# ntnu-yjyjames/nano-vectordb

Hardware: AMD Instinct MI355X
Metric: QPS + effective HBM GB/s, flat-scan top-10 d=768 (higher is better)
Workload: dtype f16

## Files before the change

include/nvdb_hip.h:

```cpp
#ifndef NVDB_HIP_H
#define NVDB_HIP_H

#include <stddef.h>
#include <stdint.h>

#ifdef __cplusplus
extern "C" {
#endif

#define NVDB_HIP_ABI_VERSION 3

enum { NVDB_DTYPE_F32 = 1, NVDB_DTYPE_F16 = 2, NVDB_DTYPE_I8 = 3 };

typedef enum nvdb_status {
  NVDB_OK = 0,
  NVDB_ERR_INVALID = 1,
  NVDB_ERR_HIP = 2,
  NVDB_ERR_UNSUPPORTED = 3,
  NVDB_ERR_NO_CORPUS = 4,
  NVDB_ERR_INTERNAL = 5
} nvdb_status;

#define NVDB_HIP_REFINE_KMAX 64

typedef struct nvdb_hip_ctx nvdb_hip_ctx;

typedef struct nvdb_hip_timing {
  float h2d_ms, kernel_ms, d2h_ms, total_ms;
  uint32_t threads;
  uint32_t nwarps;
  uint32_t K;
  uint32_t R;
  size_t shmem_bytes;
  uint32_t dbg_q;
  double dbg_dist_cycles_avg, dbg_write_cycles_avg, dbg_merge_cycles_avg;
  double dbg_dist_pct, dbg_write_pct, dbg_merge_pct;
} nvdb_hip_timing;

typedef struct nvdb_hip_scan_stats {
  uint32_t path;
  uint32_t chunks;
  uint64_t rows_scanned;
  uint64_t candidates;
  uint32_t overflow_queries;
  uint32_t bound_violations;
  float    filter_kernel_ms;
  float    other_kernel_ms;
  uint32_t i8_stage1_tiles;
  uint32_t i8_stage2_blocks;
  uint32_t sticky_overflow;
  uint32_t sticky_violations;
} nvdb_hip_scan_stats;

int nvdb_hip_abi_version(void);
int nvdb_hip_device_count(void);

nvdb_status nvdb_hip_create(int device_ordinal, nvdb_hip_ctx** out_ctx);
void nvdb_hip_destroy(nvdb_hip_ctx* ctx);
const char* nvdb_hip_last_error(const nvdb_hip_ctx* ctx);


nvdb_status nvdb_hip_upload_corpus(nvdb_hip_ctx* ctx, const void* rows, const float* scales,
                                   uint64_t n, uint32_t dim, uint32_t dtype, uint64_t global_row_base);

nvdb_status nvdb_hip_adopt_corpus(nvdb_hip_ctx* ctx, void* dev_rows, float* dev_scales,
                                  uint64_t n, uint32_t dim, uint32_t dtype, uint64_t global_row_base);

nvdb_status nvdb_hip_generate_corpus(nvdb_hip_ctx* ctx, uint64_t seed, uint64_t n, uint32_t dim,
                                     uint32_t dtype, uint64_t global_row_base);

nvdb_status nvdb_hip_corpus_info(const nvdb_hip_ctx* ctx, uint64_t* n, uint32_t* dim, uint32_t* dtype,
                                 uint64_t* global_row_base, float* max_row_norm);

nvdb_status nvdb_hip_download_rows(nvdb_hip_ctx* ctx, uint64_t row0, uint64_t nrows, void* rows_out,
                                   float* scales_out);


nvdb_status nvdb_hip_search_batch(nvdb_hip_ctx* ctx, const float* queries, uint32_t nq, uint32_t k,
                                  uint64_t* out_ids, float* out_scores, uint32_t* out_k_eff,
                                  nvdb_hip_timing* timing);

nvdb_status nvdb_hip_search_batch_dev(nvdb_hip_ctx* ctx, const float* dev_queries, uint32_t nq, uint32_t k,
                                      uint64_t* dev_out_ids, float* dev_out_scores, void* hip_stream);
nvdb_status nvdb_hip_search_check(nvdb_hip_ctx* ctx, nvdb_hip_scan_stats* stats);
nvdb_status nvdb_hip_get_stats(nvdb_hip_ctx* ctx, nvdb_hip_scan_stats* stats);


nvdb_status nvdb_hip_range_search(nvdb_hip_ctx* ctx, const float* queries, uint32_t nq,
                                  const float* radius , uint64_t* out_lims ,
                                  nvdb_hip_timing* timing );
nvdb_status nvdb_hip_range_results(nvdb_hip_ctx* ctx, uint64_t* out_ids, float* out_scores);

nvdb_status nvdb_hip_shadow_info(const nvdb_hip_ctx* ctx, uint64_t* out4);

nvdb_status nvdb_hip_merge_topk_dev(nvdb_hip_ctx* ctx, const uint64_t* dev_ids, const float* dev_scores,
                                    uint32_t nshards, uint32_t nq, uint32_t k, uint64_t* dev_out_ids,
                                    float* dev_out_scores, void* hip_stream);
nvdb_status nvdb_hip_merge_topk_strided_dev(nvdb_hip_ctx* ctx, const uint64_t* dev_ids, const float* dev_scores,
                                            size_t stride_ids_bytes, size_t stride_scores_bytes, uint32_t nshards,
                                            uint32_t nq, uint32_t k, uint64_t* dev_out_ids, float* dev_out_scores,
                                            void* hip_stream);
nvdb_status nvdb_merge_topk_host(const uint64_t* ids, const float* scores, uint32_t nshards, uint32_t nq,
                                 uint32_t k, uint64_t* out_ids, float* out_scores);

typedef struct nvdb_hip_group nvdb_hip_group;
typedef struct nvdb_hip_group_stats {
  uint32_t shards;
  uint32_t exchange;
  uint32_t host_merge_fallbacks;
  uint64_t bytes_per_rank;
} nvdb_hip_group_stats;

nvdb_status nvdb_hip_group_create(const int* devices, uint32_t n_devices, nvdb_hip_group** out_group);
void nvdb_hip_group_destroy(nvdb_hip_group* group);
const char* nvdb_hip_group_last_error(const nvdb_hip_group* group);
uint32_t nvdb_hip_group_size(const nvdb_hip_group* group);
nvdb_hip_ctx* nvdb_hip_group_ctx(nvdb_hip_group* group, uint32_t shard);
int nvdb_hip_group_exchange(const nvdb_hip_group* group, const char** why);
nvdb_status nvdb_hip_group_upload_corpus(nvdb_hip_group* group, const void* rows, const float* scales, uint64_t n,
                                         uint32_t dim, uint32_t dtype);
nvdb_status nvdb_hip_group_generate_corpus(nvdb_hip_group* group, uint64_t seed, uint64_t n, uint32_t dim, uint32_t dtype);
nvdb_status nvdb_hip_group_set_option(nvdb_hip_group* group, const char* key, int64_t value);
nvdb_status nvdb_hip_group_search_batch(nvdb_hip_group* group, const float* queries, uint32_t nq, uint32_t k,
                                        uint64_t* out_ids, float* out_scores, uint32_t* out_k_eff,
                                        nvdb_hip_group_stats* stats);


nvdb_status nvdb_hip_set_partitions(nvdb_hip_ctx* ctx, const uint64_t* offsets, uint32_t nparts);

nvdb_status nvdb_hip_set_centroids(nvdb_hip_ctx* ctx, const float* centroids);

nvdb_status nvdb_hip_search_partitions(nvdb_hip_ctx* ctx, const float* queries, uint32_t nq, uint32_t k,
                                       const uint32_t* probe, uint32_t nprobe,
                                       uint64_t* out_ids, float* out_scores, uint32_t* out_counts,
                                       nvdb_hip_timing* timing);

nvdb_status nvdb_hip_search_ivf(nvdb_hip_ctx* ctx, const float* queries, uint32_t nq, uint32_t k, uint32_t nprobe,
                                uint64_t* out_ids, float* out_scores, uint32_t* out_counts,
                                uint32_t* out_probe, nvdb_hip_timing* timing);


nvdb_status nvdb_hip_set_row_masks(nvdb_hip_ctx* ctx, const uint32_t* bits , uint32_t nmasks);

nvdb_status nvdb_hip_update_row_mask(nvdb_hip_ctx* ctx, uint32_t mask, const uint64_t* rows, uint64_t nrows, int live);

nvdb_status nvdb_hip_get_row_masks(nvdb_hip_ctx* ctx, uint32_t* nmasks, uint64_t* words_per_mask, uint32_t* bits_out );

nvdb_status nvdb_hip_search_partitions_masked(nvdb_hip_ctx* ctx, const float* queries, uint32_t nq, uint32_t k,
                                              const uint32_t* probe, uint32_t nprobe, const uint32_t* mask_of ,
                                              uint64_t* out_ids, float* out_scores, uint32_t* out_counts,
                                              nvdb_hip_timing* timing);
nvdb_status nvdb_hip_search_ivf_masked(nvdb_hip_ctx* ctx, const float* queries, uint32_t nq, uint32_t k, uint32_t nprobe,
                                       const uint32_t* mask_of ,
                                       uint64_t* out_ids, float* out_scores, uint32_t* out_counts,
                                       uint32_t* out_probe, nvdb_hip_timing* timing);
nvdb_status nvdb_hip_search_batch_masked(nvdb_hip_ctx* ctx, const float* queries, uint32_t nq, uint32_t k,
                                         const uint32_t* mask_of ,
                                         uint64_t* out_ids, float* out_scores, uint32_t* out_counts,
                                         nvdb_hip_timing* timing);


nvdb_status nvdb_hip_compact_rows(nvdb_hip_ctx* ctx, uint32_t mask, uint64_t* out_n ,
                                  uint32_t* out_old_rows );

struct nvdb_hip_ivf;
nvdb_status nvdb_hip_ivf_compact(struct nvdb_hip_ivf* ivf, uint32_t mask, uint64_t* out_n );


nvdb_status nvdb_hip_reserve_rows(nvdb_hip_ctx* ctx, uint64_t rows);

nvdb_status nvdb_hip_insert_rows(nvdb_hip_ctx* ctx, const void* rows, const float* scales , uint64_t m,
                                 const uint32_t* part_of ,
                                 uint64_t* out_new_rows , uint64_t* out_n );

nvdb_status nvdb_hip_ivf_add_rows(struct nvdb_hip_ivf* ivf, const void* rows, const float* scales , uint64_t m,
                                  uint64_t* out_first_id , uint32_t* out_assign );


nvdb_status nvdb_hip_range_search_partitions(nvdb_hip_ctx* ctx, const float* queries, uint32_t nq,
                                             const float* radius , const uint32_t* probe , uint32_t nprobe,
                                             const uint32_t* mask_of , int masked,
                                             uint64_t* out_lims , nvdb_hip_timing* timing );
nvdb_status nvdb_hip_range_search_ivf(nvdb_hip_ctx* ctx, const float* queries, uint32_t nq, const float* radius ,
                                      uint32_t nprobe, const uint32_t* mask_of , int masked,
                                      uint64_t* out_lims , uint32_t* out_probe ,
                                      nvdb_hip_timing* timing );
nvdb_status nvdb_hip_range_search_masked(nvdb_hip_ctx* ctx, const float* queries, uint32_t nq, const float* radius ,
                                         const uint32_t* mask_of , uint64_t* out_lims ,
                                         nvdb_hip_timing* timing );


nvdb_status nvdb_hip_search_partitions_anyk(nvdb_hip_ctx* ctx, const float* queries, uint32_t nq, uint32_t k,
                                            const uint32_t* probe , uint32_t nprobe,
                                            const uint32_t* mask_of , int masked,
                                            uint64_t* out_ids , float* out_scores ,
                                            uint32_t* out_counts , nvdb_hip_timing* timing );
nvdb_status nvdb_hip_search_ivf_anyk(nvdb_hip_ctx* ctx, const float* queries, uint32_t nq, uint32_t k, uint32_t nprobe,
                                     const uint32_t* mask_of , int masked,
                                     uint64_t* out_ids , float* out_scores ,
                                     uint32_t* out_counts , uint32_t* out_probe ,
                                     nvdb_hip_timing* timing );


nvdb_status nvdb_hip_assign_rows(nvdb_hip_ctx* ctx, const float* centroids, uint32_t nparts,
                                 uint64_t row0, uint64_t nrows, uint32_t* out_assign);

nvdb_status nvdb_hip_train_centroids(nvdb_hip_ctx* ctx, uint32_t nparts, uint32_t iters, uint64_t seed,
                                     uint64_t max_train_rows, const float* init, float* out_centroids);

nvdb_status nvdb_ivf_layout_host(const uint32_t* assign, uint64_t n, uint32_t nparts,
                                 uint64_t* out_offsets , uint32_t* out_perm );

typedef struct nvdb_hip_ivf nvdb_hip_ivf;
nvdb_status nvdb_hip_ivf_build(nvdb_hip_ctx* src, const float* centroids, uint32_t nparts, nvdb_hip_ivf** out);
void nvdb_hip_ivf_destroy(nvdb_hip_ivf* ivf);
const char* nvdb_hip_ivf_last_error(const nvdb_hip_ivf* ivf);
nvdb_hip_ctx* nvdb_hip_ivf_ctx(nvdb_hip_ivf* ivf);
nvdb_status nvdb_hip_ivf_info(const nvdb_hip_ivf* ivf, uint64_t* n, uint32_t* nparts,
                              uint64_t* offsets_out, uint32_t* perm_out);
nvdb_status nvdb_hip_ivf_search(nvdb_hip_ivf* ivf, const float* queries, uint32_t nq, uint32_t k, uint32_t nprobe,
                                uint64_t* out_ids, float* out_scores, uint32_t* out_counts,
                                uint32_t* out_probe, nvdb_hip_timing* timing);

nvdb_status nvdb_hip_ivf_set_row_masks(nvdb_hip_ivf* ivf, const uint32_t* bits, uint32_t nmasks);
nvdb_status nvdb_hip_ivf_update_row_mask(nvdb_hip_ivf* ivf, uint32_t mask, const uint64_t* rows, uint64_t nrows, int live);
nvdb_status nvdb_hip_ivf_search_masked(nvdb_hip_ivf* ivf, const float* queries, uint32_t nq, uint32_t k, uint32_t nprobe,
                                       const uint32_t* mask_of ,
                                       uint64_t* out_ids, float* out_scores, uint32_t* out_counts,
                                       uint32_t* out_probe, nvdb_hip_timing* timing);

nvdb_status nvdb_hip_ivf_search_anyk(nvdb_hip_ivf* ivf, const float* queries, uint32_t nq, uint32_t k, uint32_t nprobe,
                                     const uint32_t* mask_of , int masked,
                                     uint64_t* out_ids, float* out_scores, uint32_t* out_counts,
                                     uint32_t* out_probe, nvdb_hip_timing* timing);

nvdb_status nvdb_hip_ivf_range_search(nvdb_hip_ivf* ivf, const float* queries, uint32_t nq, const float* radius ,
                                      uint32_t nprobe, const uint32_t* mask_of , int masked,
                                      uint64_t* out_lims , uint32_t* out_probe ,
                                      nvdb_hip_timing* timing );
nvdb_status nvdb_hip_ivf_range_results(nvdb_hip_ivf* ivf, uint64_t* out_ids, float* out_scores);

nvdb_status nvdb_hip_set_option(nvdb_hip_ctx* ctx, const char* key, int64_t value);

nvdb_status nvdb_hip_collect_kernel_times(nvdb_hip_ctx* ctx, uint32_t* launches, double* total_ms,
                                          double* total_flops, double* total_bytes);


// ... 17 lines not shown
```

nano-vectordb_amd/csrc/kernels_corpus.h:

```cpp
#pragma once
#include <hip/hip_runtime.h>

#include "kernels_exact.h"
#include "nvdb_common.h"

namespace nvdbhip {

template <int DT>
__global__ __launch_bounds__(256) void gen_rows_kernel(uint64_t seed, uint64_t row_base, uint64_t n, uint32_t dim,
                                                       void* __restrict__ rows, float* __restrict__ scales) {
  const int lane = threadIdx.x & 63;
  const uint64_t r = static_cast<uint64_t>(blockIdx.x) * 4 + (threadIdx.x >> 6);
  if (r >= n) return;
  const uint32_t key = synth_row_key(seed, row_base + r);
  unsigned long long ss = 0;
  for (uint32_t c = lane; c < dim; c += 64) { const long long v = synth_raw(key, c); ss += static_cast<unsigned long long>(v * v); }
  for (int o = 32; o > 0; o >>= 1) ss += __shfl_xor(ss, o);
  const double inv = synth_inv_norm(ss);
  if constexpr (DT == DT_F32) {
    float* out = static_cast<float*>(rows) + r * dim;
    for (uint32_t c = lane; c < dim; c += 64) out[c] = synth_elem(synth_raw(key, c), inv);
  } else if constexpr (DT == DT_F16) {
    _Float16* out = static_cast<_Float16*>(rows) + r * dim;
    for (uint32_t c = lane; c < dim; c += 64) out[c] = static_cast<_Float16>(synth_elem(synth_raw(key, c), inv));
  } else {
    float mx = 0.f;
    for (uint32_t c = lane; c < dim; c += 64) mx = fmaxf(mx, fabsf(synth_elem(synth_raw(key, c), inv)));
    for (int o = 32; o > 0; o >>= 1) mx = fmaxf(mx, __shfl_xor(mx, o));
    const float scale = mx > 0.f ? mx / 127.f : 1.f;
    const float is = 1.0f / scale;
    signed char* out = static_cast<signed char*>(rows) + r * dim;
    for (uint32_t c = lane; c < dim; c += 64) {
      float qv = rintf(synth_elem(synth_raw(key, c), inv) * is);
      qv = fminf(fmaxf(qv, -127.f), 127.f);
      out[c] = static_cast<signed char>(static_cast<int>(qv));
    }
    if (lane == 0) scales[r] = scale;
  }
}

template <typename SrcT>
__global__ __launch_bounds__(256) void shadow_f16_kernel(const SrcT* __restrict__ src, _Float16* __restrict__ dst, size_t n,
                                                         uint32_t dim, uint32_t sdim, uint32_t* __restrict__ maxabs_bits) {
  float mx = 0.f;
  const size_t count = n * sdim;
  for (size_t i = static_cast<size_t>(blockIdx.x) * 256 + threadIdx.x; i < count; i += static_cast<size_t>(gridDim.x) * 256) {
    const size_t r = i / sdim;
    const uint32_t c = static_cast<uint32_t>(i - r * sdim);
    const float v = c < dim ? static_cast<float>(src[r * dim + c]) : 0.f;
    dst[i] = static_cast<_Float16>(v);
    mx = fmaxf(mx, fabsf(v));
  }
  for (int o = 32; o > 0; o >>= 1) mx = fmaxf(mx, __shfl_xor(mx, o));
  if ((threadIdx.x & 63) == 0 && mx > 0.f) atomicMax(maxabs_bits, __builtin_bit_cast(uint32_t, mx));
}

static __global__ __launch_bounds__(256) void shadow_i8_kernel(const signed char* __restrict__ src, signed char* __restrict__ dst, size_t n,
                                                        uint32_t dim, uint32_t sdim) {
  const size_t count = n * sdim;
  for (size_t i = static_cast<size_t>(blockIdx.x) * 256 + threadIdx.x; i < count; i += static_cast<size_t>(gridDim.x) * 256) {
    const size_t r = i / sdim;
    const uint32_t c = static_cast<uint32_t>(i - r * sdim);
    dst[i] = c < dim ? src[r * dim + c] : static_cast<signed char>(0);
  }
}

template <typename SrcT>
__global__ __launch_bounds__(256) void shadow_q8_kernel(const SrcT* __restrict__ src, signed char* __restrict__ dst, float* __restrict__ dst_scales,
                                                        uint64_t n, uint32_t dim, uint32_t sdim, uint32_t* __restrict__ out_bits) {
  const int lane = threadIdx.x & 63;
  float wres = 0.f;
  bool bad = false;
  for (uint64_t r = static_cast<uint64_t>(blockIdx.x) * 4 + (threadIdx.x >> 6); r < n; r += static_cast<uint64_t>(gridDim.x) * 4) {
    const SrcT* row = src + r * dim;
    float mx = 0.f;
    for (uint32_t c = lane; c < dim; c += 64) mx = fmaxf(mx, fabsf(static_cast<float>(row[c])));
    for (int o = 32; o > 0; o >>= 1) mx = fmaxf(mx, __shfl_xor(mx, o));
    if (!(mx < 3.0e38f)) bad = true;
    const float scale = mx > 0.f ? mx / 127.f : 1.f;
    const float inv = 1.0f / scale;
    float ss = 0.f;
    signed char* out = dst + r * sdim;
    for (uint32_t c = lane; c < sdim; c += 64) {
      float qv = 0.f, x = 0.f;
      if (c < dim) { x = static_cast<float>(row[c]); qv = fminf(fmaxf(rintf(x * inv), -127.f), 127.f); }
      out[c] = static_cast<signed char>(static_cast<int>(qv));
      const float d = x - qv * scale;
      ss = __builtin_fmaf(d, d, ss);
    }
    for (int o = 32; o > 0; o >>= 1) ss += __shfl_xor(ss, o);
    if (!(ss == ss)) bad = true;
    if (lane == 0) dst_scales[r] = scale;
    wres = fmaxf(wres, sqrtf(ss) * 1.0001f);
  }
  if (lane == 0 && wres > 0.f) atomicMax(out_bits, __builtin_bit_cast(uint32_t, wres));
  if (lane == 0 && (bad || !(wres < 3.0e38f))) out_bits[1] = 1u;
}

template <int DT>
__global__ __launch_bounds__(256) void row_norm_max_kernel(const void* __restrict__ rows, const float* __restrict__ scales,
                                                           uint64_t n, uint32_t dim, uint32_t* __restrict__ out_bits) {
  const int lane = threadIdx.x & 63;
  float wmax = 0.f;
  for (uint64_t r = static_cast<uint64_t>(blockIdx.x) * 4 + (threadIdx.x >> 6); r < n; r += static_cast<uint64_t>(gridDim.x) * 4) {
    const void* rp = row_ptr<DT>(rows, r, dim);
    float ss = 0.f;
    for (uint32_t c = lane; c < dim; c += 64) { const float v = load1<DT>(rp, c); ss = __builtin_fmaf(v, v, ss); }
    for (int o = 32; o > 0; o >>= 1) ss += __shfl_xor(ss, o);
    float nrm = sqrtf(ss) * 1.0001f;
    if constexpr (DT == DT_I8) {
      const float sc = scales[r];
      nrm *= fabsf(sc);
      if (!(sc >= 0.f && sc < 1e30f) && lane == 0) out_bits[1] = 1u;
    }
    wmax = fmaxf(wmax, nrm);
  }
  if (lane == 0 && wmax > 0.f) atomicMax(out_bits, __builtin_bit_cast(uint32_t, wmax));
}

}
```

nano-vectordb_amd/csrc/kernels_filter_i8s.h:

```cpp
#pragma once
#include "kernels_filter.h"

namespace nvdbhip {

typedef int intx4_t __attribute__((ext_vector_type(4)));

#define NVDB_MFMA_I8S_FROM(acc, a, b, c0) asm volatile("v_mfma_i32_16x16x64_i8 %0, %1, %2, %3" : "=&v"(acc) : "v"(a), "a"(b), "v"(c0))
#define NVDB_MFMA_I8S_ACC(acc, a, b) asm volatile("v_mfma_i32_16x16x64_i8 %0, %1, %2, %0" : "+v"(acc) : "v"(a), "a"(b))

template <int DIM, int WPB = 4> constexpr size_t filter_i8s_lds_bytes() { return static_cast<size_t>(3) * (2 * FILTER_ROWS * DIM + WPB * 256); }
template <int DIM, bool SYNC = false, bool STAMP = false, int RING = 6, int WPB = 4>
__global__ __launch_bounds__(64 * WPB, 1) void filter_i8s_kernel(
    const signed char* __restrict__ rows, const float* __restrict__ scales, uint32_t row_lo, uint32_t row_hi,
    const signed char* __restrict__ qhi, const signed char* __restrict__ qlo, uint32_t nq, uint32_t QT,
    const float* __restrict__ thr, const float* __restrict__ qscale, const float* __restrict__ qinv,
    const float* __restrict__ qdelta, Hit* __restrict__ hitlog, ScatterArgs sa, uint32_t* __restrict__ prog,
    uint32_t sync_mask, uint32_t sync_lead, uint32_t* __restrict__ stage_counts) {
  static_assert(WPB == 4 || WPB == 8, "4 waves x 64 queries or 8 waves x 32 queries");
  constexpr int NB = 16 / WPB, MB = 2;
  constexpr int NV = 8 * NB;
  constexpr int KS = DIM / 64;
  constexpr int ROW_BYTES = DIM;
  constexpr int TROWS = FILTER_ROWS * MB;
  constexpr int NSTAGE = 3;
  constexpr int DATA_BYTES = TROWS * ROW_BYTES;
  constexpr int STAGE_BYTES = DATA_BYTES + WPB * 256;
  constexpr int PIECES = DATA_BYTES / 1024, PPW = PIECES / WPB;
  constexpr int CHUNKS_PER_ROW = ROW_BYTES / 16;
  constexpr int NSLOT = 2 * NB * KS;
  constexpr int NFRAG = 2 * KS;
  static_assert(DIM % 128 == 0 && DIM <= 768, "row stride multiple of 128 bytes (swz_chunk); 64 queries x DIM bytes = 192 AGPRs at most");
  static_assert(PIECES % WPB == 0 && PPW % 2 == 0 && NSTAGE * STAGE_BYTES <= 160 * 1024 && PPW + 1 < 64 && NFRAG >= RING, "shape / LDS / vmcnt range");
  static_assert(NSTAGE * STAGE_BYTES == filter_i8s_lds_bytes<DIM, WPB>(), "the launchers size the dynamic LDS with filter_i8s_lds_bytes");

  extern __shared__ __attribute__((aligned(16))) char smem[];
  const int tid = threadIdx.x, lane = tid & 63, wave = __builtin_amdgcn_readfirstlane(tid >> 6);
  const int x15 = lane & 15, g4 = lane >> 4;
  const uint32_t wave_gid = blockIdx.x * WPB + wave;

  const uint32_t nwg = gridDim.x, b = blockIdx.x;
  const uint32_t S = nwg / QT;
  uint32_t stream, qt;
  if (xcd_aware_grid(QT, nwg)) { const uint32_t xcd = b & 7u, i = b >> 3; qt = i % QT; stream = (i / QT) * 8u + xcd; }
  else { qt = b % QT; stream = b / QT; }
  const uint32_t tiles_total = (row_hi - row_lo) / TROWS;
  const bool xcd_map = xcd_aware_grid(QT, nwg);
  uint32_t t_lo, t_hi;
  stream_tile_range(tiles_total, S, stream, xcd_map, sa.xcdw, t_lo, t_hi);
  const uint32_t NT = t_hi - t_lo;
  if (NT == 0) return;

  const uint32_t qbase = qt * 256u + wave * (16u * NB);
  float4_t bq[NB * KS];
#pragma unroll
  for (int f = 0; f < NB * KS; ++f) {
    const int nb = f / KS, s = f % KS;
    bq[f] = *reinterpret_cast<const float4_t*>(qhi + static_cast<uint64_t>(qbase + nb * 16 + x15) * DIM + 64 * s + 16 * g4);
  }
#pragma unroll
  for (int f = 0; f < NB * KS; ++f) asm volatile("" ::"a"(bq[f]));
  intx4_t bias0;
#pragma unroll
  for (int r = 0; r < 4; ++r) bias0[r] = I8_ACC_BIAS;
  asm volatile("" : "+v"(bias0));
  uint32_t qid[NB];
  float t1q[NB];
  const float lo_unit = __builtin_bit_cast(float, (127u - sa.lo_bits) << 23);
#pragma unroll
  for (int nb = 0; nb < NB; ++nb) {
    qid[nb] = qbase + nb * 16 + x15;
    const bool real = qid[nb] < nq;
    const float T = real ? thr[qid[nb]] * qscale[qid[nb]] : __builtin_huge_valf();
    t1q[nb] = real ? i8_stage1_bar(T, qdelta[qid[nb]], lo_unit) : __builtin_huge_valf();
    asm volatile("" ::"v"(t1q[nb]));
  }
  const bool wave_has_queries = qbase < nq;

  uint32_t src_off[PPW];
#pragma unroll
  for (int i = 0; i < PPW; ++i) {
    const uint32_t P = static_cast<uint32_t>((wave * PPW + i) * 64 + lane);
    const uint32_t r = P / CHUNKS_PER_ROW, cpos = P % CHUNKS_PER_ROW;
    src_off[i] = r * ROW_BYTES + (swz_chunk<ROW_BYTES>(cpos, r) << 4);
  }
  const uint32_t sc_off = (lane & (8 * MB - 1)) * 16;
  const uint32_t a16 = static_cast<uint32_t>(x15) * ROW_BYTES + (swz_chunk<ROW_BYTES>(static_cast<uint32_t>(g4), static_cast<uint32_t>(x15)) << 4);

  const char* gbase = reinterpret_cast<const char*>(rows);
  const uint32_t lds_base = static_cast<uint32_t>(reinterpret_cast<uintptr_t>(NVDB_LPTR(smem)));
  const uint32_t g_lo = row_lo / TROWS + t_lo;
  auto tile_row0 = [&](uint32_t t_rel) -> uint32_t { return perm_tile(g_lo + (t_rel < NT ? t_rel : NT - 1), sa) * TROWS; };
  auto issue_piece = [&](uint32_t row0, uint32_t buf, int i) {
    glds16(src_off[i], gbase + static_cast<uint64_t>(row0) * ROW_BYTES, lds_base + buf * STAGE_BYTES + (wave * PPW + i) * 1024);
  };
  auto issue_scales = [&](uint32_t row0, uint32_t buf) {
    if (lane < 8 * MB) glds16(sc_off, reinterpret_cast<const char*>(scales + row0), lds_base + buf * STAGE_BYTES + DATA_BYTES + wave * 256);
  };
#pragma unroll
  for (int st = 0; st < NSTAGE - 1; ++st) {
#pragma unroll
    for (int i = 0; i < PPW; ++i) issue_piece(tile_row0(st), st, i);
    issue_scales(tile_row0(st), st);
  }

  uint32_t wcnt = 0, n_stage1 = 0;
  Hit* mylog = hitlog + static_cast<uint64_t>(wave_gid) * FILTER_LOGCAP;

  intx4_t acc0[2][NB], acc1[2][NB];
  float scv[2][8], scc[2][8];
#pragma unroll
  for (int i = 0; i < 8; ++i) { scv[0][i] = scv[1][i] = 0.f; scc[0][i] = scc[1][i] = 0.f; }
#pragma unroll
  for (int h = 0; h < 2; ++h)
#pragma unroll
    for (int nb = 0; nb < NB; ++nb) acc1[h][nb] = bias0;
  float mx[NB][2];
  float4_t ar[RING];

  auto read_a = [&](const char* stage, int u, int mb) -> float4_t {
    const int s = u >> 1, h = u & 1;
    const uint32_t off = swz16<ROW_BYTES>() ? (a16 ^ ((s & 3) << 6)) + (s >> 2) * 256 : (a16 ^ ((s & 1) << 6)) + (s >> 1) * 128;
    return *reinterpret_cast<const float4_t*>(stage + off + (2 * mb + h) * 16 * ROW_BYTES);
  };
  constexpr int SW0 = NSLOT >= 64 ? 8 : 4;
  auto scale_step = [&](const char* stage, int mb, int set, int w) {
    if (w == 0) {
      const float* sc_lds = reinterpret_cast<const float*>(stage + DATA_BYTES + wave * 256);
#pragma unroll
      for (int h = 0; h < 2; ++h) {
        const float4 v = *reinterpret_cast<const float4*>(sc_lds + 32 * mb + 16 * h + 4 * g4);
        scv[set][4 * h] = v.x; scv[set][4 * h + 1] = v.y; scv[set][4 * h + 2] = v.z; scv[set][4 * h + 3] = v.w;
      }
    }
    const int i = w - SW0;
    if (i >= 0 && i < 8) scc[set][i] = scv[set][i] * -8388608.f;
  };
  float tm[NV];
  constexpr int W0 = SW0 + 10;
  constexpr int SPU = (NSLOT - W0 - 4) / NV >= 2 ? 2 : 1;
  static_assert(W0 + NV * SPU + 2 <= NSLOT, "the test ends before the half's last MFMA");
  auto test_step = [&](const intx4_t (&a)[2][NB], const float (&sc)[8], const float (&sccs)[8], int w) {
    const int rel = w - W0;
    if (rel < 0 || rel % SPU != 0) return;
    const int v = rel / SPU;
    if (v < NV) {
      const int nb = v >> 3, h = (v >> 2) & 1, j = v & 3;
      const int b0 = a[h][nb][j];
      tm[v] = __builtin_fmaf(__builtin_bit_cast(float, b0), sc[4 * h + j], sccs[4 * h + j]);
    }
    const int p = v - 1;
    if (p >= 0 && p < NV && (p & 1)) mx[p >> 3][(p >> 2) & 1] = vmax3(mx[p >> 3][(p >> 2) & 1], tm[p - 1], tm[p]);
  };
  auto reset_max = [&]() {
#pragma unroll
    for (int nb = 0; nb < NB; ++nb) { mx[nb][0] = -__builtin_huge_valf(); mx[nb][1] = -__builtin_huge_valf(); }
  };
  float flagv = -1.f;
  auto combine_flags = [&]() {
    float m[NB];
#pragma unroll
    for (int nb = 0; nb < NB; ++nb) m[nb] = vmax3(mx[nb][0], mx[nb][1], mx[nb][1]) - t1q[nb];
    flagv = NB == 4 ? vmax3(vmax3(m[0], m[1], m[NB / 2]), m[NB - 1], m[NB - 1]) : vmax3(m[0], m[NB - 1], m[NB - 1]);
  };
  auto any_flag = [&]() -> bool { return __builtin_amdgcn_ballot_w64(flagv >= 0.f) != 0; };
  auto rare_log = [&](const intx4_t (&a)[2][NB], const float (&sc)[8], uint32_t row0, int mb) {
    ++n_stage1;
#pragma unroll
    for (int nb = 0; nb < NB; ++nb)
#pragma unroll
      for (int h = 0; h < 2; ++h) {
        if (!__builtin_amdgcn_ballot_w64(mx[nb][h] >= t1q[nb])) continue;
#pragma unroll
        for (int j = 0; j < 4; ++j) {
          const int H = a[h][nb][j] - I8_ACC_BIAS;
          const bool hit = static_cast<float>(H) * sc[4 * h + j] >= t1q[nb];
          const unsigned long long m = __builtin_amdgcn_ballot_w64(hit);
          if (m) {
            const uint32_t idx = wcnt + static_cast<uint32_t>(__builtin_popcountll(m & ((1ull << lane) - 1ull)));
            if (hit && idx < FILTER_LOGCAP)
              mylog[idx] = Hit{sc[4 * h + j], row0 + 32u * mb + 16u * h + 4u * g4 + j, qid[nb], static_cast<uint32_t>(H)};
            wcnt += static_cast<uint32_t>(__builtin_popcountll(m));
          }
        }
      }
  };

  uint32_t sync_strikes = 0;
  uint64_t stamp_c = 0, stamp_r = 0;
  if constexpr (STAMP) { stamp_c = __builtin_amdgcn_s_memtime(); stamp_r = __builtin_amdgcn_s_memrealtime(); }
  const uint32_t xw_t0 = static_cast<uint32_t>(__builtin_amdgcn_s_memrealtime());
  constexpr int HP = PPW / 2, HP0 = HP < 3 ? HP : 3;
  constexpr int D1 = (HP - HP0) > 0 ? (HP - HP0) : 1;
  constexpr int EV1 = NFRAG / D1, EV2 = NFRAG / (PPW - HP);
  static_assert((HP == HP0 || NFRAG % (HP - HP0) == 0) && NFRAG % (PPW - HP) == 0, "pieces spread evenly over the A fragments of both halves");
  for (uint32_t t = 0; t < NT; ++t) {
    if constexpr (SYNC) {
      if (wave == 0 && (t & sync_mask) == 0) sibling_rendezvous(prog + static_cast<uint64_t>(stream) * 8, qt, t, sync_lead, sync_strikes, lane);
    }
    asm volatile("s_waitcnt vmcnt(%0)" ::"n"(PPW + 1) : "memory");
    __builtin_amdgcn_s_barrier();
    const uint32_t next_row0 = tile_row0(t + 2), next_buf = (t + 2) % NSTAGE;
    const char* stage = smem + (t % NSTAGE) * STAGE_BYTES;
    if (!wave_has_queries) {
#pragma unroll
      for (int i = 0; i < PPW; ++i) issue_piece(next_row0, next_buf, i);
      issue_scales(next_row0, next_buf);
      continue;
    }
    reset_max();
#pragma unroll
    for (int u = 0; u < RING - 1; ++u) ar[u] = read_a(stage, u, 0);
#pragma unroll
    for (int i = 0; i < HP0; ++i) issue_piece(next_row0, next_buf, i);
    __builtin_amdgcn_sched_barrier(0);
#pragma unroll
    for (int u = 0; u < NFRAG; ++u) {
      if (u + RING - 1 < NFRAG) ar[(u + RING - 1) % RING] = read_a(stage, u + RING - 1, 0);
      else ar[(u + RING - 1) % RING] = read_a(stage, u + RING - 1 - NFRAG, 1);
      const float4_t av = ar[u % RING];
      const int s = u >> 1, h = u & 1;
#pragma unroll
      for (int nb = 0; nb < NB; ++nb) {
        if (s == 0) NVDB_MFMA_I8S_FROM(acc0[h][nb], av, bq[nb * KS], bias0);
        else NVDB_MFMA_I8S_ACC(acc0[h][nb], av, bq[nb * KS + s]);
        const int w = NB * u + nb;
        scale_step(stage, 0, 0, w);
        test_step(acc1, scv[1], scc[1], w);
        if (w == NSLOT - 1) combine_flags();
        __builtin_amdgcn_sched_barrier(0);
      }
      if constexpr (HP > HP0) {
        if (u % EV1 == EV1 - 1) issue_piece(next_row0, next_buf, HP0 + u / EV1);
        __builtin_amdgcn_sched_barrier(0);
      }
    }
    if (t > 0 && any_flag()) rare_log(acc1, scv[1], tile_row0(t - 1), 1);
    reset_max();
    constexpr int R0 = NFRAG % RING;
#pragma unroll
    for (int u = 0; u < NFRAG; ++u) {
      if (u + RING - 1 < NFRAG) ar[(R0 + u + RING - 1) % RING] = read_a(stage, u + RING - 1, 1);
      const float4_t av = ar[(R0 + u) % RING];
      const int s = u >> 1, h = u & 1;
#pragma unroll
      for (int nb = 0; nb < NB; ++nb) {
        if (s == 0) NVDB_MFMA_I8S_FROM(acc1[h][nb], av, bq[nb * KS], bias0);
        else NVDB_MFMA_I8S_ACC(acc1[h][nb], av, bq[nb * KS + s]);
        const int w = NB * u + nb;
        scale_step(stage, 1, 1, w);
        test_step(acc0, scv[0], scc[0], w);
        if (w == NSLOT - 1) combine_flags();
        __builtin_amdgcn_sched_barrier(0);
      }
      if (u % EV2 == EV2 - 1) issue_piece(next_row0, next_buf, HP + u / EV2);
      if (u == 0) issue_scales(next_row0, next_buf);
      __builtin_amdgcn_sched_barrier(0);
    }
    if (any_flag()) rare_log(acc0, scv[0], tile_row0(t), 0);
  }
  if (wave_has_queries) {
    asm volatile("s_nop 15\n\ts_nop 15" ::: "memory");
    reset_max();
#pragma unroll
    for (int w = W0; w < W0 + (NV + 1) * SPU; ++w) test_step(acc1, scv[1], scc[1], w);
    combine_flags();
    if (any_flag()) rare_log(acc1, scv[1], tile_row0(NT - 1), 1);
  }
  if constexpr (STAMP) {
    const uint64_t dc = __builtin_amdgcn_s_memtime() - stamp_c, dr = __builtin_amdgcn_s_memrealtime() - stamp_r;
    if (wave == 0 && lane == 0) {
      uint64_t* out = reinterpret_cast<uint64_t*>(prog + static_cast<uint64_t>(gridDim.x) * 8) + static_cast<uint64_t>(blockIdx.x) * 2;
      out[0] = dc; out[1] = dr;
    }
  }
  if constexpr (SYNC) { if (wave == 0 && lane == 0) __hip_atomic_store(prog + static_cast<uint64_t>(stream) * 8 + qt, 0xFFFFFFFFu, __ATOMIC_RELAXED, __HIP_MEMORY_SCOPE_AGENT); }
  if (stage_counts && lane == 0 && n_stage1) atomicAdd(stage_counts, n_stage1);
  if (wave == 0 && lane == 0) record_xcd_speed(sa.xcdw, xcd_map, stream & 7u, NT, static_cast<uint32_t>(__builtin_amdgcn_s_memrealtime()) - xw_t0);
  verify_and_scatter_i8<DIM>(mylog, wcnt, sa, lane, rows, qlo, thr, qscale, qinv);
}

}
```

nano-vectordb_amd/csrc/nvdb_corpus.cpp:

```cpp
#include "nvdb_ctx.h"
#include "compact_plan.h"
#include "insert_plan.h"
#include "kernels_corpus.h"

namespace {

std::string g_create_err;

void free_corpus(nvdb_hip_ctx* c) {
  if (c->owned) {
    if (c->rows) (void)hipFree(c->rows);
    if (c->scales) (void)hipFree(c->scales);
  }
  if (c->shadow16) { (void)hipFree(c->shadow16); c->shadow16 = nullptr; }
  if (c->shadow8) { (void)hipFree(c->shadow8); c->shadow8 = nullptr; }
  if (c->shadow8_scales) { (void)hipFree(c->shadow8_scales); c->shadow8_scales = nullptr; }
  c->rows = nullptr; c->scales = nullptr; c->owned = false; c->n = 0; c->cap_rows = 0; c->dim = 0; c->fdim = 0; c->dtype = 0; c->max_norm = 0.f;
  c->cap_hint = 0;
  c->q8shadow = false; c->resid_max = 0.f; c->filter_max_norm = 0.f;
  c->shadow_demoted = false; c->last_filter_kind = FILTER_NONE;
  c->range_valid = false; c->range_total = 0;
  parts_drop(c);
  c->nmasks = 0;
}

nvdb_status compute_max_norm(nvdb_hip_ctx* c) {
  nvdb_status st = ensure(c, c->misc, 64);
  if (st) return st;
  if (c->cap_rows < c->n) c->cap_rows = c->n;
  const size_t cap = static_cast<size_t>(c->cap_rows);
  HIPCHK(c, hipMemsetAsync(c->misc.p, 0, 64, c->stream));
  uint32_t* bits = static_cast<uint32_t*>(c->misc.p) + 8;
  const unsigned grid = static_cast<unsigned>(std::min<uint64_t>((c->n + 3) / 4, 4096));
  if (c->dtype == NVDB_DTYPE_F32) row_norm_max_kernel<DT_F32><<<grid, 256, 0, c->stream>>>(c->rows, c->scales, c->n, c->dim, bits);
  else if (c->dtype == NVDB_DTYPE_F16) row_norm_max_kernel<DT_F16><<<grid, 256, 0, c->stream>>>(c->rows, c->scales, c->n, c->dim, bits);
  else row_norm_max_kernel<DT_I8><<<grid, 256, 0, c->stream>>>(c->rows, c->scales, c->n, c->dim, bits);
  HIPCHK(c, hipGetLastError());
  uint32_t h = 0, hb[2] = {0, 0};
  HIPCHK(c, hipMemcpyAsync(hb, bits, 8, hipMemcpyDeviceToHost, c->stream));
  HIPCHK(c, hipStreamSynchronize(c->stream));
  h = hb[0];
  std::memcpy(&c->max_norm, &h, 4);
  c->i8_scales_signed = hb[1] != 0;
  c->fdim = c->dim;
  c->filter_max_norm = c->max_norm;
  c->q8shadow = false; c->resid_max = 0.f;
  size_t free_hbm = 0, total_hbm = 0;
  const bool automatic = c->opt_q8_shadow < 0;
  if (automatic && hipMemGetInfo(&free_hbm, &total_hbm) != hipSuccess) { (void)hipGetLastError(); free_hbm = 0; }
  if (q8_shadow_wanted(c, free_hbm)) {
    const uint32_t sdim = c->dim;
    const size_t pad = static_cast<size_t>(PAD_ROWS) * sdim + 4096;
    const size_t cap_pad = (cap + PAD_ROWS - 1) / PAD_ROWS * PAD_ROWS + PAD_ROWS;
    hipError_t e = hipMalloc(reinterpret_cast<void**>(&c->shadow8), cap * sdim + pad);
    if (e == hipSuccess) e = hipMalloc(reinterpret_cast<void**>(&c->shadow8_scales), cap_pad * 4);
    if (e != hipSuccess) {
      if (c->shadow8) (void)hipFree(c->shadow8);
      c->shadow8 = nullptr; c->shadow8_scales = nullptr;
      (void)hipGetLastError();
      if (!automatic) return fail(c, NVDB_ERR_HIP, std::string("q8_shadow allocation: ") + hipGetErrorString(e));
    }
  }
  if (c->shadow8) {
    const uint32_t sdim = c->dim;
    const size_t count = static_cast<size_t>(c->n) * sdim, pad = static_cast<size_t>(PAD_ROWS) * sdim + 4096;
    const size_t n_pad = (static_cast<size_t>(c->n) + PAD_ROWS - 1) / PAD_ROWS * PAD_ROWS + PAD_ROWS;
    HIPCHK(c, hipMemsetAsync(c->shadow8 + count, 0, pad, c->stream));
    HIPCHK(c, hipMemsetAsync(c->shadow8_scales, 0, n_pad * 4, c->stream));
    HIPCHK(c, hipMemsetAsync(bits, 0, 8, c->stream));
    if (c->dtype == NVDB_DTYPE_F32) shadow_q8_kernel<float><<<grid, 256, 0, c->stream>>>(static_cast<const float*>(c->rows), c->shadow8, c->shadow8_scales, c->n, c->dim, sdim, bits);
    else shadow_q8_kernel<_Float16><<<grid, 256, 0, c->stream>>>(static_cast<const _Float16*>(c->rows), c->shadow8, c->shadow8_scales, c->n, c->dim, sdim, bits);
    HIPCHK(c, hipGetLastError());
    HIPCHK(c, hipMemcpyAsync(hb, bits, 8, hipMemcpyDeviceToHost, c->stream));
    HIPCHK(c, hipStreamSynchronize(c->stream));
    if (hb[1] == 0) {
      std::memcpy(&c->resid_max, &hb[0], 4);
      HIPCHK(c, hipMemsetAsync(bits, 0, 8, c->stream));
      row_norm_max_kernel<DT_I8><<<grid, 256, 0, c->stream>>>(c->shadow8, c->shadow8_scales, c->n, sdim, bits);
      HIPCHK(c, hipGetLastError());
      HIPCHK(c, hipMemcpyAsync(hb, bits, 8, hipMemcpyDeviceToHost, c->stream));
      HIPCHK(c, hipStreamSynchronize(c->stream));
      std::memcpy(&c->filter_max_norm, &hb[0], 4);
      c->q8shadow = true;
      c->i8_scales_signed = false;
      return NVDB_OK;
    }
    (void)hipFree(c->shadow8); c->shadow8 = nullptr;
    (void)hipFree(c->shadow8_scales); c->shadow8_scales = nullptr;
  }
  if (c->dtype != NVDB_DTYPE_I8 && c->dim <= F16_FILTER_MAX_DIM && !(c->dtype == NVDB_DTYPE_F16 && f16_filter_dim(c->dim)) && c->opt_f32_shadow) {
    uint32_t sdim = 128;
    while (!f16_filter_dim(sdim) || sdim < c->dim) sdim += 128;
    const size_t count = static_cast<size_t>(c->n) * sdim;
    const size_t pad = static_cast<size_t>(PAD_ROWS) * sdim * 2 + 4096;
    HIPCHK(c, hipMalloc(reinterpret_cast<void**>(&c->shadow16), cap * sdim * 2 + pad));
    HIPCHK(c, hipMemsetAsync(reinterpret_cast<char*>(c->shadow16) + count * 2, 0, pad, c->stream));
    HIPCHK(c, hipMemsetAsync(bits, 0, 4, c->stream));
    if (c->dtype == NVDB_DTYPE_F32) shadow_f16_kernel<float><<<4096, 256, 0, c->stream>>>(static_cast<const float*>(c->rows), c->shadow16, c->n, c->dim, sdim, bits);
    else shadow_f16_kernel<_Float16><<<4096, 256, 0, c->stream>>>(static_cast<const _Float16*>(c->rows), c->shadow16, c->n, c->dim, sdim, bits);
    HIPCHK(c, hipGetLastError());
    HIPCHK(c, hipMemcpyAsync(&h, bits, 4, hipMemcpyDeviceToHost, c->stream));
    HIPCHK(c, hipStreamSynchronize(c->stream));
    float maxabs; std::memcpy(&maxabs, &h, 4);
    if (!(maxabs < 60000.f)) { (void)hipFree(c->shadow16); c->shadow16 = nullptr; }
    else c->fdim = sdim;
  }
  if (c->dtype == NVDB_DTYPE_I8 && c->dim <= I8_FILTER_MAX_DIM && !i8_filter_dim(c->dim) && c->opt_f32_shadow) {
    uint32_t sdim = 256;
    while (!i8_filter_dim(sdim) || sdim < c->dim) sdim += 128;
    const size_t count = static_cast<size_t>(c->n) * sdim, pad = static_cast<size_t>(PAD_ROWS) * sdim + 4096;
    const size_t n_pad = (static_cast<size_t>(c->n) + PAD_ROWS - 1) / PAD_ROWS * PAD_ROWS + PAD_ROWS;
    const size_t cap_pad = (cap + PAD_ROWS - 1) / PAD_ROWS * PAD_ROWS + PAD_ROWS;
    HIPCHK(c, hipMalloc(reinterpret_cast<void**>(&c->shadow8), cap * sdim + pad));
    HIPCHK(c, hipMalloc(reinterpret_cast<void**>(&c->shadow8_scales), cap_pad * 4));
    HIPCHK(c, hipMemsetAsync(c->shadow8 + count, 0, pad, c->stream));
    HIPCHK(c, hipMemsetAsync(c->shadow8_scales, 0, n_pad * 4, c->stream));
    HIPCHK(c, hipMemcpyAsync(c->shadow8_scales, c->scales, static_cast<size_t>(c->n) * 4, hipMemcpyDeviceToDevice, c->stream));
    shadow_i8_kernel<<<4096, 256, 0, c->stream>>>(static_cast<const signed char*>(c->rows), c->shadow8, c->n, c->dim, sdim);
    HIPCHK(c, hipGetLastError());
    HIPCHK(c, hipStreamSynchronize(c->stream));
    c->fdim = sdim;
  }
  return NVDB_OK;
}

nvdb_status upload_rows(nvdb_hip_ctx* c, void* dst, const void* src, size_t bytes) {
  unsigned T = std::min(6u, std::max(2u, std::thread::hardware_concurrency() / 2));
  if (const char* e = std::getenv("NVDB_UPLOAD_THREADS")) T = static_cast<unsigned>(std::max(1, std::atoi(e)));
  constexpr size_t CH = size_t(8) << 20;
  const size_t nch = (bytes + CH - 1) / CH;
  if (T <= 1 || nch < 4 * static_cast<size_t>(T)) {
    const size_t chunk = size_t(256) << 20;
    for (size_t off = 0; off < bytes; off += chunk) {
      const size_t take = std::min(chunk, bytes - off);
      HIPCHK(c, hipMemcpy(static_cast<char*>(dst) + off, static_cast<const char*>(src) + off, take, hipMemcpyHostToDevice));
    }
    return NVDB_OK;
  }
  std::vector<std::string> errs(T);
  std::atomic<size_t> next{0};
  auto worker = [&](unsigned t) {
    hipStream_t st = nullptr;
    void* pin[2] = {nullptr, nullptr};
    hipEvent_t ev[2] = {nullptr, nullptr};
    bool used[2] = {false, false};
    auto chk = [&](hipError_t e, const char* what) { if (e != hipSuccess && errs[t].empty()) errs[t] = std::string(what) + ": " + hipGetErrorString(e); return e == hipSuccess; };
    bool ok = chk(hipSetDevice(c->device), "hipSetDevice") && chk(hipStreamCreateWithFlags(&st, hipStreamNonBlocking), "hipStreamCreate");
    const auto tp0 = std::chrono::steady_clock::now();
    for (int b = 0; b < 2 && ok; ++b)
      ok = chk(hipHostMalloc(&pin[b], CH, hipHostMallocDefault), "hipHostMalloc") && chk(hipEventCreateWithFlags(&ev[b], hipEventDisableTiming), "hipEventCreate");
    if (t == 0 && std::getenv("NVDB_UPLOAD_DEBUG")) std::fprintf(stderr, "[nvdb upload] thread 0: stream + 2 pinned buffers of %zu MB in %.1f ms\n", CH >> 20, std::chrono::duration<double, std::milli>(std::chrono::steady_clock::now() - tp0).count());
    for (int b = 0; ok; b ^= 1) {
      const size_t i = next.fetch_add(1);
      if (i >= nch) break;
      const size_t off = i * CH, take = std::min(CH, bytes - off);
      if (used[b]) ok = chk(hipEventSynchronize(ev[b]), "hipEventSynchronize");
      if (!ok) break;
      std::memcpy(pin[b], static_cast<const char*>(src) + off, take);
      ok = chk(hipMemcpyAsync(static_cast<char*>(dst) + off, pin[b], take, hipMemcpyHostToDevice, st), "hipMemcpyAsync") && chk(hipEventRecord(ev[b], st), "hipEventRecord");
      used[b] = true;
    }
    if (st) (void)hipStreamSynchronize(st);
    for (int b = 0; b < 2; ++b) { if (ev[b]) (void)hipEventDestroy(ev[b]); if (pin[b]) (void)hipHostFree(pin[b]); }
    if (st) (void)hipStreamDestroy(st);
  };
  std::vector<std::thread> th;
  for (unsigned t = 0; t < T; ++t) th.emplace_back(worker, t);
  for (auto& x : th) x.join();
  for (const auto& e : errs) if (!e.empty()) return fail(c, NVDB_ERR_HIP, "upload: " + e);
  return NVDB_OK;
}

nvdb_status check_corpus_args(nvdb_hip_ctx* c, uint64_t n, uint32_t dim, uint32_t dtype) {
  if (!c) return NVDB_ERR_INVALID;
  if (n == 0 || dim == 0) return fail(c, NVDB_ERR_INVALID, "corpus: count and dim must be > 0");
  if (bpe_of(dtype) == 0) return fail(c, NVDB_ERR_INVALID, "Unsupported base dtype (Float32/Float16/Int8 only)");
  if (n >= 0xFFFFFFF0ull) return fail(c, NVDB_ERR_UNSUPPORTED, "corpus shard must hold fewer than 2^32-16 rows (shard it)");
  return NVDB_OK;
}

}

namespace nvdbhip {

nvdb_status corpus_alloc_padded(nvdb_hip_ctx* c, uint64_t n, uint32_t dim, uint32_t dtype, void** rows, float** scales) {
  *rows = nullptr; *scales = nullptr;
  const size_t bytes = static_cast<size_t>(n) * dim * bpe_of(dtype);
  const size_t pad = static_cast<size_t>(PAD_ROWS) * dim * bpe_of(dtype) + 4096;
  HIPCHK(c, hipMalloc(rows, bytes + pad));
  hipError_t e = hipMemset(static_cast<char*>(*rows) + bytes, 0, pad);
  if (e == hipSuccess && dtype == NVDB_DTYPE_I8) {
    e = hipMalloc(reinterpret_cast<void**>(scales), (n + PAD_ROWS) * sizeof(float));
    if (e == hipSuccess) e = hipMemset(*scales + n, 0, PAD_ROWS * sizeof(float));
  }
  if (e != hipSuccess) {
    (void)hipFree(*rows); *rows = nullptr;
    if (*scales) { (void)hipFree(*scales); *scales = nullptr; }
    return fail(c, NVDB_ERR_HIP, std::string("corpus allocation: ") + hipGetErrorString(e));
  }
  return NVDB_OK;
}

nvdb_status corpus_take_ownership(nvdb_hip_ctx* c, void* dev_rows, float* dev_scales, uint64_t n, uint32_t dim, uint32_t dtype,
                                  uint64_t global_row_base) {
  free_corpus(c);
  c->rows = dev_rows; c->scales = dev_scales; c->owned = true;
  nvdb_status st = check_corpus_args(c, n, dim, dtype);
  if (!st && (!dev_rows || (dtype == NVDB_DTYPE_I8 && !dev_scales))) st = fail(c, NVDB_ERR_INVALID, "take_ownership: null buffer");
  if (st) { free_corpus(c); return st; }
  HIPCHK(c, hipSetDevice(c->device));
  c->n = n; c->dim = dim; c->dtype = dtype; c->row_base = global_row_base;
  return compute_max_norm(c);
}

void corpus_drop(nvdb_hip_ctx* c) { free_corpus(c); }

nvdb_status corpus_rederive(nvdb_hip_ctx* c) {
  if (c->shadow16) { (void)hipFree(c->shadow16); c->shadow16 = nullptr; }
  if (c->shadow8) { (void)hipFree(c->shadow8); c->shadow8 = nullptr; }
  if (c->shadow8_scales) { (void)hipFree(c->shadow8_scales); c->shadow8_scales = nullptr; }
  return compute_max_norm(c);
}

}

extern "C" {

int nvdb_hip_abi_version(void) { return NVDB_HIP_ABI_VERSION; }

// ... 6 lines not shown
nvdb_status nvdb_hip_create(int device_ordinal, nvdb_hip_ctx** out_ctx) {
  if (!out_ctx) return NVDB_ERR_INVALID;
  *out_ctx = nullptr;
  int ndev = 0;
  hipError_t e = hipGetDeviceCount(&ndev);
  if (e != hipSuccess || ndev <= 0) {
    g_create_err = std::string("no HIP device available: ") + (e != hipSuccess ? hipGetErrorString(e) : "device count is 0");
    return NVDB_ERR_HIP;
  }
  if (device_ordinal < 0 || device_ordinal >= ndev) { g_create_err = "device ordinal out of range"; return NVDB_ERR_INVALID; }
  if ((e = hipSetDevice(device_ordinal)) != hipSuccess) { g_create_err = hipGetErrorString(e); return NVDB_ERR_HIP; }
  auto* c = new nvdb_hip_ctx();
  c->device = device_ordinal;
  hipDeviceProp_t prop;
  if (hipGetDeviceProperties(&prop, device_ordinal) == hipSuccess) c->num_cu = prop.multiProcessorCount;
  if ((e = hipStreamCreateWithFlags(&c->stream, hipStreamNonBlocking)) != hipSuccess) {
    g_create_err = hipGetErrorString(e);
    delete c;
    return NVDB_ERR_HIP;
  }
  {
    float w0[24];
    for (int i = 0; i < 24; ++i) w0[i] = i < 8 ? 1.f : 0.f;
    if ((e = hipMalloc(&c->xcdw.p, sizeof(w0))) != hipSuccess || (e = hipMemcpy(c->xcdw.p, w0, sizeof(w0), hipMemcpyHostToDevice)) != hipSuccess) {
      g_create_err = hipGetErrorString(e);
      if (c->xcdw.p) (void)hipFree(c->xcdw.p);
      (void)hipStreamDestroy(c->stream);
      delete c;
      return NVDB_ERR_HIP;
    }
    c->xcdw.bytes = sizeof(w0);
  }
  *out_ctx = c;
  return NVDB_OK;
}

void nvdb_hip_destroy(nvdb_hip_ctx* c) {
  if (!c) return;
  (void)hipSetDevice(c->device);
  (void)hipStreamSynchronize(c->stream);
  free_corpus(c);
  parts_destroy(c);
  if (c->hostblock.p) c->misc.p = nullptr;
  for (DevBuf* b : {&c->q32, &c->q16, &c->qscale, &c->qinv, &c->ebound, &c->slack, &c->thr, &c->cnt, &c->overflow, &c->cand,
                    &c->out_ids, &c->out_scores, &c->misc, &c->hostblock, &c->hitlog, &c->prog, &c->qdelta, &c->rq, &c->rcand, &c->rout_ids, &c->rout_dist, &c->rdbg, &c->lk_scores, &c->lk_sel, &c->lk_hist, &c->lk_state, &c->xcdw, &c->tickets,
                    &c->rg_radius, &c->rg_kept, &c->rg_off, &c->rg_idx, &c->rg_q, &c->rg_desc, &c->rg_taken, &c->rg_slab, &c->rg_pcnt, &c->rg_maskof, &c->rg_ids, &c->rg_scores, &c->row_masks, &c->mask_rows,
                    &c->cp_rank, &c->cp_sums, &c->cp_bounce, &c->cp_map, &c->cp_live, &c->row_masks_alt, &c->ins_meta, &c->ins_pos})
    if (b->p) (void)hipFree(b->p);
  for (hipEvent_t e : c->ev_pool) (void)hipEventDestroy(e);
  for (auto& k : c->klaunch) { (void)hipEventDestroy(k.e0); (void)hipEventDestroy(k.e1); }
  for (hipEvent_t e : c->kl_pool) (void)hipEventDestroy(e);
  if (c->pinned) (void)hipHostFree(c->pinned);
  if (c->rpinned) (void)hipHostFree(c->rpinned);
  (void)hipStreamDestroy(c->stream);
  delete c;
}

const char* nvdb_hip_last_error(const nvdb_hip_ctx* c) { return c ? c->err.c_str() : g_create_err.c_str(); }

nvdb_status nvdb_hip_upload_corpus(nvdb_hip_ctx* c, const void* rows, const float* scales, uint64_t n, uint32_t dim,
                                   uint32_t dtype, uint64_t global_row_base) {
  nvdb_status st = check_corpus_args(c, n, dim, dtype);
  if (st) return st;
  if (!rows) return fail(c, NVDB_ERR_INVALID, "upload_corpus: null rows");
  if (dtype == NVDB_DTYPE_I8 && !scales) return fail(c, NVDB_ERR_INVALID, "upload_corpus: int8 corpus needs per-row scales");
  HIPCHK(c, hipSetDevice(c->device));
  free_corpus(c);
  const size_t bytes = static_cast<size_t>(n) * dim * bpe_of(dtype);
  const bool dbg = std::getenv("NVDB_UPLOAD_DEBUG") != nullptr;
  const auto t0 = std::chrono::steady_clock::now();
  auto since = [&]() { return std::chrono::duration<double, std::milli>(std::chrono::steady_clock::now() - t0).count(); };
  if ((st = corpus_alloc_padded(c, n, dim, dtype, &c->rows, &c->scales))) return st;
  c->owned = true;
  const double t_alloc = since();
  if ((st = upload_rows(c, c->rows, rows, bytes))) return st;
  const double t_rows = since();
  if (dtype == NVDB_DTYPE_I8) HIPCHK(c, hipMemcpy(c->scales, scales, n * sizeof(float), hipMemcpyHostToDevice));
  c->n = n; c->dim = dim; c->dtype = dtype; c->row_base = global_row_base;
  st = compute_max_norm(c);
  if (dbg) std::fprintf(stderr, "[nvdb upload] %.2f GB: device allocation %.1f ms, rows %.1f ms (%.1f GB/s), scales + row-norm pass (+ shadow copy) %.1f ms\n",
                        bytes / 1e9, t_alloc, t_rows - t_alloc, bytes / 1e6 / (t_rows - t_alloc), since() - t_rows);
  return st;
}

nvdb_status nvdb_hip_adopt_corpus(nvdb_hip_ctx* c, void* dev_rows, float* dev_scales, uint64_t n, uint32_t dim, uint32_t dtype,
                                  uint64_t global_row_base) {
  nvdb_status st = check_corpus_args(c, n, dim, dtype);
  if (st) return st;
  if (!dev_rows) return fail(c, NVDB_ERR_INVALID, "adopt_corpus: null rows");
  if (dtype == NVDB_DTYPE_I8 && !dev_scales) return fail(c, NVDB_ERR_INVALID, "adopt_corpus: int8 corpus needs per-row scales");
  HIPCHK(c, hipSetDevice(c->device));
  free_corpus(c);
  c->rows = dev_rows; c->scales = dev_scales; c->owned = false;
  c->n = n; c->dim = dim; c->dtype = dtype; c->row_base = global_row_base;
  return compute_max_norm(c);
}

nvdb_status nvdb_hip_generate_corpus(nvdb_hip_ctx* c, uint64_t seed, uint64_t n, uint32_t dim, uint32_t dtype,
                                     uint64_t global_row_base) {
  nvdb_status st = check_corpus_args(c, n, dim, dtype);
  if (st) return st;
  HIPCHK(c, hipSetDevice(c->device));
  free_corpus(c);
  if ((st = corpus_alloc_padded(c, n, dim, dtype, &c->rows, &c->scales))) return st;
  c->owned = true;
  c->n = n; c->dim = dim; c->dtype = dtype; c->row_base = global_row_base;
  const uint64_t slab = 1ull << 24;
  for (uint64_t r0 = 0; r0 < n; r0 += slab) {
    const uint64_t cntr = std::min(slab, n - r0);
    const unsigned grid = static_cast<unsigned>((cntr + 3) / 4);
    char* rp = static_cast<char*>(c->rows) + r0 * dim * bpe_of(dtype);
    if (dtype == NVDB_DTYPE_F32) gen_rows_kernel<DT_F32><<<grid, 256, 0, c->stream>>>(seed, global_row_base + r0, cntr, dim, rp, nullptr);
    else if (dtype == NVDB_DTYPE_F16) gen_rows_kernel<DT_F16><<<grid, 256, 0, c->stream>>>(seed, global_row_base + r0, cntr, dim, rp, nullptr);
    else gen_rows_kernel<DT_I8><<<grid, 256, 0, c->stream>>>(seed, global_row_base + r0, cntr, dim, rp, c->scales + r0);
    HIPCHK(c, hipGetLastError());
  }
  return compute_max_norm(c);
}

nvdb_status nvdb_hip_corpus_info(const nvdb_hip_ctx* c, uint64_t* n, uint32_t* dim, uint32_t* dtype, uint64_t* base, float* mx) {
  if (!c) return NVDB_ERR_INVALID;
  if (n) *n = c->n;
  if (dim) *dim = c->dim;
  if (dtype) *dtype = c->dtype;
  if (base) *base = c->row_base;
  if (mx) *mx = c->max_norm;
  return c->rows ? NVDB_OK : NVDB_ERR_NO_CORPUS;
}

nvdb_status nvdb_hip_download_rows(nvdb_hip_ctx* c, uint64_t row0, uint64_t nrows, void* rows_out, float* scales_out) {
  if (!c) return NVDB_ERR_INVALID;
  if (!c->rows) return fail(c, NVDB_ERR_NO_CORPUS, "Empty base");
  if (row0 + nrows > c->n || !rows_out) return fail(c, NVDB_ERR_INVALID, "download_rows: range out of bounds");
  HIPCHK(c, hipSetDevice(c->device));
  HIPCHK(c, hipStreamSynchronize(c->stream));
  const size_t rb = static_cast<size_t>(c->dim) * bpe_of(c->dtype);
  HIPCHK(c, hipMemcpy(rows_out, static_cast<const char*>(c->rows) + row0 * rb, nrows * rb, hipMemcpyDeviceToHost));
  if (scales_out && c->scales) HIPCHK(c, hipMemcpy(scales_out, c->scales + row0, nrows * sizeof(float), hipMemcpyDeviceToHost));
  return NVDB_OK;
}

nvdb_status nvdb_hip_set_option(nvdb_hip_ctx* c, const char* key, int64_t value) {
  if (!c || !key) return NVDB_ERR_INVALID;
  const std::string k(key);
  if (k == "path") { if (value < 0 || value > 2) return fail(c, NVDB_ERR_INVALID, "path must be 0,1,2"); c->opt_path = value; }
  else if (k == "chunk0_rows") { if (value < 256) return fail(c, NVDB_ERR_INVALID, "chunk0_rows must be >= 256"); c->opt_chunk0 = value; }
  else if (k == "cand_cap") { if (value < 0 || value > SELECT_MAX_CAP) return fail(c, NVDB_ERR_INVALID, "cand_cap out of range"); c->opt_cap = value; }
  else if (k == "time_kernels") { c->opt_time_kernels = value ? 1 : 0; }
  else if (k == "sync_every") { if (value < 1 || (value & (value - 1))) return fail(c, NVDB_ERR_INVALID, "sync_every must be a power of two"); c->opt_sync_every = value; }
  else if (k == "sync_lead") { if (value < 1) return fail(c, NVDB_ERR_INVALID, "sync_lead must be >= 1"); c->opt_sync_lead = value; }
  else if (k == "sibling_sync") { c->opt_sibling_sync = value ? 1 : 0; }
  else if (k == "f32_shadow") { c->opt_f32_shadow = value ? 1 : 0; }
  else if (k == "q8_shadow") { c->opt_q8_shadow = value < 0 ? -1 : value ? 1 : 0; }
  else if (k == "q8_auto_min_rows") { if (value < 1) return fail(c, NVDB_ERR_INVALID, "q8_auto_min_rows must be >= 1"); c->opt_q8_auto_min_rows = value; }
  else if (k == "q8_auto_max_mb") { if (value < 0 || value > (int64_t(1) << 30)) return fail(c, NVDB_ERR_INVALID, "q8_auto_max_mb out of range"); c->opt_q8_auto_max_mb = value; }
#ifdef NVDB_HIP_DEV
  else if (k == "mfma16") { c->opt_mfma16 = value ? 1 : 0; }
  else if (k == "i8_wide") { c->opt_i8_wide = value ? 1 : 0; }
  else if (k == "i8_pipe") { c->opt_i8_pipe = value ? 1 : 0; }
  else if (k == "i8_waves8") { c->opt_i8_waves8 = value ? 1 : 0; }
  else if (k == "i8_mfma16") { c->opt_i8_mfma16 = value ? 1 : 0; }
  else if (k == "i8_small8") { c->opt_i8_small8 = value ? 1 : 0; }
#else
  else if (k == "mfma16" || k == "i8_wide" || k == "i8_pipe" || k == "i8_mfma16" || k == "i8_small8") { if (!value) return fail(c, NVDB_ERR_UNSUPPORTED, k + " = 0 selects a developer-build kernel variant (libnvdb_hip_dev.so)"); }
  else if (k == "i8_waves8") { if (value) return fail(c, NVDB_ERR_UNSUPPORTED, "i8_waves8 = 1 selects a developer-build kernel variant (libnvdb_hip_dev.so)"); }
#endif

  else if (k == "i8_dense8") { c->opt_i8_dense8 = value ? 1 : 0; }
  else if (k == "i8_defer") { c->opt_i8_defer = value ? 1 : 0; }
  else if (k == "xcd_balance") { c->opt_xcd_balance = value ? 1 : 0; }
  else if (k == "i8_lo_bits") { if (value < 2 || value > 7) return fail(c, NVDB_ERR_INVALID, "i8_lo_bits must be in [2,7]"); c->opt_i8_lo_bits = value; }
  else if (k == "boot_tiles") { if (value < 0 || value > SELECT_MAX_CAP) return fail(c, NVDB_ERR_INVALID, "boot_tiles out of range"); c->opt_boot_tiles = value; }
#ifdef NVDB_HIP_DEV
  else if (k == "debug_rows") { c->dbg_rows = value < 0 ? 0 : value; }
  else if (k == "debug_bound_pct") { if (value < 1 || value > 100) return fail(c, NVDB_ERR_INVALID, "debug_bound_pct must be in [1,100]"); c->dbg_bound_pct = value; }
#endif
  else if (k == "waves8") { c->opt_waves8 = value ? 1 : 0; }
  else if (k == "fuse") { c->opt_fuse = value ? 1 : 0; }
  else if (k == "zero_copy") { c->opt_zero_copy = value ? 1 : 0; }
  else if (k == "shadow_exact_thr") { c->opt_shadow_exact_thr = value ? 1 : 0; }
  else if (k == "exact_mfma") { c->opt_exact_mfma = value ? 1 : 0; }
  else if (k == "exact_img") { c->opt_exact_img = value ? 1 : 0; }
  else if (k == "exact_prescan") { c->opt_exact_prescan = value ? 1 : 0; }
  else if (k == "exact_wgs") { if (value < 1 || value > 16) return fail(c, NVDB_ERR_INVALID, "exact_wgs must be in [1,16]"); c->opt_exact_wgs = value; }
  else if (k == "exact_lds") { if (value < 0 || value > 2) return fail(c, NVDB_ERR_INVALID, "exact_lds must be 0, 1 or 2"); c->opt_exact_lds = value; }
  else if (k == "time_launches") { c->opt_time_launches = value ? 1 : 0; }
  else if (k == "tile_permute") { c->opt_tile_permute = value ? 1 : 0; }
  else if (k == "rescore8") { c->opt_rescore8 = value < 0 ? 0 : (value > 2 ? 2 : value); }
  else if (k == "mfma_boot") { c->opt_mfma_boot = value ? 1 : 0; }
  else if (k == "refine_v2") { c->opt_refine_v2 = value < 0 ? 0 : (value > 2 ? 2 : value); }
  else if (k == "refine_pinned") { c->opt_refine_pinned = value ? 1 : 0; }
  else if (k == "refine_dbg_q") { if (value < 0) return fail(c, NVDB_ERR_INVALID, "refine_dbg_q must be >= 0"); c->opt_refine_dbg_q = value; }
  else if (k == "largek_budget_mb") { if (value < 1) return fail(c, NVDB_ERR_INVALID, "largek_budget_mb must be >= 1"); c->opt_largek_budget_mb = value; }
  else if (k == "range_max_mb") { if (value < 1) return fail(c, NVDB_ERR_INVALID, "range_max_mb must be >= 1"); c->opt_range_max_mb = value; }
  else if (k == "compact_slab_rows") { if (!cp_slab_rows_valid(value)) return fail(c, NVDB_ERR_INVALID, "compact_slab_rows must be a multiple of 64 in [64, 2^24]"); c->opt_compact_slab_rows = value; }
  else if (k == "insert_growth_pct") { if (!ins_growth_pct_valid(value)) return fail(c, NVDB_ERR_INVALID, "insert_growth_pct must be in [0, 400]"); c->opt_insert_growth_pct = value; }
  else if (k == "chunk_growth") { if (value != 0 && (value < 2 || value > 64)) return fail(c, NVDB_ERR_INVALID, "chunk_growth must be 0 (automatic) or in [2,64]"); c->opt_growth = value; }
  else if (k == "min_filter_batch") { if (value < 1) return fail(c, NVDB_ERR_INVALID, "min_filter_batch must be >= 1"); c->opt_min_filter_batch = value; }
  else return fail(c, NVDB_ERR_INVALID, "unknown option: " + k);
  return NVDB_OK;
}

nvdb_status nvdb_hip_shadow_info(const nvdb_hip_ctx* c, uint64_t* out4) {
  if (!c || !out4) return NVDB_ERR_INVALID;
  out4[0] = c->q8shadow ? 1u : 0u;
  out4[1] = c->q8shadow ? q8_shadow_bytes(c->n, c->dim) : 0u;
  out4[2] = c->shadow_demoted ? 1u : 0u;
  out4[3] = c->last_filter_kind;
  return NVDB_OK;
}

nvdb_status nvdb_hip_get_stats(nvdb_hip_ctx* c, nvdb_hip_scan_stats* stats) {
  if (!c || !stats) return NVDB_ERR_INVALID;
  if (c->stats_lazy) {
    c->stats_lazy = false;
    unsigned long long tot = 0;
    HIPCHK(c, hipSetDevice(c->device));
    if (nvdb_status st = sum_candidates(c, &tot)) return st;
    c->stats.candidates = tot;
  }
  *stats = c->stats;
  return NVDB_OK;
}

#ifdef NVDB_HIP_DEV
uint32_t nvdb_permuted_tile(uint32_t g, uint32_t n_tiles) {
  uint32_t mul, mask;
  perm_params(n_tiles, mul, mask);
  return perm_tile_raw(g, mul, mask, n_tiles);
}
#endif

void nvdb_synth_rows_f32(uint64_t seed, uint64_t row0, uint64_t nrows, uint32_t dim, float* out) {
  std::vector<int32_t> raw(dim);
  for (uint64_t r = 0; r < nrows; ++r) {
    const uint32_t key = synth_row_key(seed, row0 + r);
    uint64_t ss = 0;
    for (uint32_t c = 0; c < dim; ++c) { raw[c] = synth_raw(key, c); ss += static_cast<uint64_t>(static_cast<int64_t>(raw[c]) * raw[c]); }
    const double inv = synth_inv_norm(ss);
    for (uint32_t c = 0; c < dim; ++c) out[r * dim + c] = synth_elem(raw[c], inv);
  }
}

void nvdb_f32_to_f16(const float* src, uint16_t* dst, uint64_t n) {
  for (uint64_t i = 0; i < n; ++i) dst[i] = f32_to_f16_rne(src[i]);
}

void nvdb_quantize_i8_rows(const float* rows, uint64_t nrows, uint32_t dim, int8_t* out, float* scales) {
  for (uint64_t r = 0; r < nrows; ++r) scales[r] = quantize_i8_row(rows + r * dim, dim, out + r * dim);
}

}
```

nano-vectordb_amd/csrc/nvdb_ctx.h:

```cpp
#pragma once
#pragma GCC visibility push(default)
#include "../../include/nvdb_hip.h"
#ifdef NVDB_HIP_DEV
#include "../../include/nvdb_hip_dev.h"
#endif
#pragma GCC visibility pop

#include <hip/hip_runtime.h>
#include <hip/hip_ext.h>

#include <algorithm>
#include <atomic>
#include <chrono>
#include <cmath>
#include <cstdio>
#include <cstdlib>
#include <cstring>
#include <set>
#include <string>
#include <thread>
#include <type_traits>
#include <vector>

#include "kernels_exact.h"
#include "kernels_filter.h"
#include "nvdb_common.h"

using namespace nvdbhip;

namespace nvdbhip {

constexpr uint32_t SELECT_MAX_CAP = 8192;
constexpr uint32_t WAVE_KMAX = 64;
constexpr uint32_t FILTER_KMAX = 1024;
constexpr float FILTER_REL_F16 = 7.5e-4f;
constexpr uint32_t PROG_SLOTS = 16;
constexpr uint32_t F16_FILTER_MAX_DIM = 3072;
constexpr uint32_t I8W_TILE_ROWS = 64;
constexpr uint32_t PAD_ROWS = 64;
constexpr uint32_t I8_FILTER_MAX_DIM = 1536;

enum FilterKind : uint32_t { FILTER_NONE = 0, FILTER_F16 = 1, FILTER_SHADOW8 = 2, FILTER_I8 = 3 };
struct DevBuf {
  void* p = nullptr;
  size_t bytes = 0;
};

struct PartState;

}

struct nvdb_hip_ctx {
  int device = 0;
  int num_cu = 256;
  hipStream_t stream = nullptr;
  std::string err;

  void* rows = nullptr;
  float* scales = nullptr;
  bool owned = false;
  uint64_t n = 0;
  uint64_t cap_rows = 0;
  uint32_t dim = 0, dtype = 0;
  uint64_t row_base = 0;
  float max_norm = 0.f;
  bool i8_scales_signed = false;
  signed char* shadow8 = nullptr;
  bool q8shadow = false;
  bool shadow_demoted = false;
  float filter_max_norm = 0.f;
  float resid_max = 0.f;
  int64_t opt_q8_shadow = -1;
  int64_t opt_q8_auto_min_rows = 1 << 20;
  int64_t opt_q8_auto_max_mb = 16384;
  float* shadow8_scales = nullptr;
  _Float16* shadow16 = nullptr;
  uint32_t fdim = 0;
  DevBuf qdelta;
  int64_t opt_i8_wide = 1;
  int64_t opt_i8_waves8 = 0;
  int64_t opt_i8_dense8 = 1;
  int64_t opt_i8_defer = 0;
  int64_t opt_i8_mfma16 = 1;
  int64_t opt_i8_pipe = 1;
  int64_t opt_waves8 = 1;
  void* pinned = nullptr;
  void* pinned_dev = nullptr;
  size_t pinned_bytes = 0;
  int64_t opt_tile_permute = 1;
  uint32_t cap_hint = 0;
  bool stats_lazy = false;
  std::vector<hipEvent_t> kl_pool;
  int64_t opt_time_launches = 0;
  int64_t opt_exact_lds = 1;
  int64_t opt_exact_img = 1;
  int64_t opt_exact_wgs = 1;
  int64_t opt_exact_prescan = 1;
  int64_t opt_exact_mfma = 1;
  int64_t opt_rescore8 = 2;

  DevBuf q32, q16, qscale, qinv, ebound, slack, thr, cnt, overflow, cand, out_ids, out_scores, misc, hitlog, prog;
  DevBuf hostblock;
  DevBuf tickets;
  int64_t opt_fuse = 1;
  int64_t opt_shadow_exact_thr = 1;
  int64_t opt_zero_copy = 1;
  bool status_by_kernel = false;
  size_t q32_dirty = 0;
  DevBuf rq, rcand, rout_ids, rout_dist;
  DevBuf rdbg;
  DevBuf xcdw;
  int64_t opt_xcd_balance = 1;
  int64_t opt_i8_lo_bits = 7;
  int64_t opt_boot_tiles = 0;
  int64_t opt_i8_small8 = 1;
  int64_t dbg_rows = 0;
  int64_t dbg_bound_pct = 100;
  DevBuf lk_scores, lk_sel, lk_hist, lk_state;
  int64_t opt_refine_pinned = 0;
  int64_t opt_refine_dbg_q = 0;
  void* rpinned = nullptr;
  size_t rpinned_bytes = 0;
  int64_t opt_largek_budget_mb = 8192;
  DevBuf rg_radius, rg_kept, rg_off, rg_idx, rg_q, rg_desc, rg_taken, rg_slab;
  DevBuf rg_pcnt, rg_maskof;
  DevBuf rg_ids, rg_scores;
  uint64_t range_total = 0;
  bool range_valid = false;
  int64_t opt_range_max_mb = 4096;

  int64_t opt_path = 0, opt_chunk0 = 512, opt_cap = 0, opt_min_filter_batch = 1, opt_growth = 0;

  nvdb_hip_scan_stats stats{};
  uint32_t last_nq = 0, last_cap = 0;
  bool last_filter = false;
  FilterKind last_filter_kind = FILTER_NONE;
  bool last_perm = false;
  std::vector<hipEvent_t> ev_pool;
  std::vector<std::pair<int, int>> ev_filter;
  struct KLaunch { hipEvent_t e0, e1; double flops, bytes; };
  std::vector<KLaunch> klaunch;
  int64_t opt_time_kernels = 0;
  int64_t opt_sync_every = 4, opt_sync_lead = 4;
  int64_t opt_sibling_sync = 1;
  int64_t opt_f32_shadow = 1;
  int64_t opt_mfma_boot = 1;
  int64_t opt_refine_v2 = 2;
  int64_t opt_mfma16 = 1;
  std::set<const void*> lds_attr_set;
  nvdbhip::PartState* parts = nullptr;
  DevBuf row_masks, mask_rows;
  uint32_t nmasks = 0;
  std::vector<uint64_t> mask_live;
  DevBuf cp_rank, cp_sums, cp_bounce, cp_map, cp_live, row_masks_alt;
  int64_t opt_compact_slab_rows = 65536;
  DevBuf ins_meta, ins_pos;
  int64_t opt_insert_growth_pct = 50;
};

#define HIPCHK(ctx, call)                                                                        \
  do {                                                                                           \
    hipError_t e_ = (call);                                                                      \
    if (e_ != hipSuccess) {                                                                      \
      (ctx)->err = std::string(#call) + ": " + hipGetErrorString(e_);                            \
      return NVDB_ERR_HIP;                                                                       \
    }                                                                                            \
  } while (0)

namespace nvdbhip {

inline nvdb_status fail(nvdb_hip_ctx* c, nvdb_status s, const std::string& msg) {
  c->err = msg;
  return s;
}

inline nvdb_status ensure(nvdb_hip_ctx* c, DevBuf& b, size_t bytes) {
  if (b.bytes >= bytes && b.p) return NVDB_OK;
  if (b.p) { HIPCHK(c, hipFree(b.p)); b.p = nullptr; b.bytes = 0; }
  size_t want = std::max<size_t>(bytes, 256);
  HIPCHK(c, hipMalloc(&b.p, want));
  b.bytes = want;
  return NVDB_OK;
}

inline size_t bpe_of(uint32_t dtype) { return dtype == NVDB_DTYPE_F32 ? 4 : (dtype == NVDB_DTYPE_F16 ? 2 : (dtype == NVDB_DTYPE_I8 ? 1 : 0)); }

inline bool aligned_rows(uint32_t dtype, uint32_t dim) {
  if (dtype == NVDB_DTYPE_F32) return dim % 4 == 0;
  return dim % 8 == 0;
}

template <int... D> struct DimList {};
using F16Dims = DimList<768, 640, 512, 384, 256, 128>;
using F16Dims16 = DimList<896, 1024, 1152, 1280, 1408, 1536>;
using F16DimsK2 = DimList<2048, 2560, 3072>;
using I8Dims = DimList<768, 640, 512, 384, 256>;
using I8DimsBig = DimList<896, 1024, 1152, 1280, 1408, 1536>;
using ExactMfmaDims = DimList<768, 640, 512, 384, 256, 128>;
using Refine3Dims = DimList<768, 512, 384, 256>;

template <int... D, typename F>
bool dispatch_dim(DimList<D...>, uint32_t dim, nvdb_status& st, F&& f) {
  return ((dim == static_cast<uint32_t>(D) && ((st = f(std::integral_constant<int, D>{})), true)) || ...);
}
template <int... D> bool has_dim(DimList<D...>, uint32_t dim) { return ((dim == static_cast<uint32_t>(D)) || ...); }
template <typename F>
void dispatch_dtype(uint32_t dtype, nvdb_status& st, F&& f) {
  if (dtype == NVDB_DTYPE_F32) st = f(std::integral_constant<int, DT_F32>{});
  else if (dtype == NVDB_DTYPE_F16) st = f(std::integral_constant<int, DT_F16>{});
  else st = f(std::integral_constant<int, DT_I8>{});
}

inline bool f16_filter_dim(uint32_t dim) { return has_dim(F16Dims{}, dim) || has_dim(F16Dims16{}, dim) || has_dim(F16DimsK2{}, dim); }
inline bool i8_filter_dim(uint32_t dim) { return has_dim(I8Dims{}, dim) || has_dim(I8DimsBig{}, dim); }

inline const signed char* filter_rows_i8(const nvdb_hip_ctx* c) { return c->shadow8 ? c->shadow8 : static_cast<const signed char*>(c->rows); }
inline const float* filter_scales_i8(const nvdb_hip_ctx* c) { return c->shadow8 ? c->shadow8_scales : c->scales; }
inline const _Float16* filter_rows_f16(const nvdb_hip_ctx* c) {
  return c->shadow16 ? c->shadow16 : static_cast<const _Float16*>(c->rows);
}

inline bool f16_beside_shadow(const nvdb_hip_ctx* c) { return c->q8shadow && c->dtype == NVDB_DTYPE_F16 && f16_filter_dim(c->dim); }
inline bool shadow_preferred(const nvdb_hip_ctx* c) { return c->q8shadow && !(f16_beside_shadow(c) && (c->opt_q8_shadow == 0 || c->shadow_demoted)); }
inline FilterKind filter_kind(const nvdb_hip_ctx* c) { return c->dtype == NVDB_DTYPE_I8 ? FILTER_I8 : shadow_preferred(c) ? FILTER_SHADOW8 : FILTER_F16; }
// ... 161 lines not shown
```

nano-vectordb_amd/csrc/nvdb_insert.cpp:

```cpp
#include "nvdb_insert.h"
#include "nvdb_parts.h"
#include "insert_plan.h"
#include "kernels_corpus.h"
#include "kernels_insert.h"

namespace nvdbhip {
namespace {

enum ArrKind { ARR_ROWS, ARR_SCALES, ARR_SH8, ARR_SH8S, ARR_SH16 };

struct InsArray { ArrKind kind; void* p; size_t row_bytes; const void* staged; void* fresh; };

inline size_t pad_rows_up(size_t n) { return (n + PAD_ROWS - 1) / PAD_ROWS * PAD_ROWS + PAD_ROWS; }

size_t arr_bytes(const InsArray& a, size_t cap) {
  if (a.kind == ARR_SCALES) return (cap + PAD_ROWS) * 4;
  if (a.kind == ARR_SH8S) return pad_rows_up(cap) * 4;
  return cap * a.row_bytes + static_cast<size_t>(PAD_ROWS) * a.row_bytes + 4096;
}
size_t arr_tail(const InsArray& a, size_t n) {
  if (a.kind == ARR_SCALES) return static_cast<size_t>(PAD_ROWS) * 4;
  if (a.kind == ARR_SH8S) return (pad_rows_up(n) - n) * 4;
  return static_cast<size_t>(PAD_ROWS) * a.row_bytes + 4096;
}
// ... 32 lines not shown
    (void)hipFree(a.p);
    switch (a.kind) {
      case ARR_ROWS: c->rows = a.fresh; break;
      case ARR_SCALES: c->scales = static_cast<float*>(a.fresh); break;
      case ARR_SH8: c->shadow8 = static_cast<signed char*>(a.fresh); break;
      case ARR_SH8S: c->shadow8_scales = static_cast<float*>(a.fresh); break;
      case ARR_SH16: c->shadow16 = static_cast<_Float16*>(a.fresh); break;
    }
    a.p = a.fresh; a.fresh = nullptr;
  }
  c->cap_rows = cap;
}

template <class F>
void with_lane(size_t row_bytes, F&& f) {
  if (row_bytes % 16 == 0) f(CompactLane16{});
  else if (row_bytes % 8 == 0) f(CompactLane8{});
  else if (row_bytes % 4 == 0) f(uint32_t{});
  else if (row_bytes % 2 == 0) f(uint16_t{});
  else f(uint8_t{});
}

struct PlanImage { const uint64_t *off_old, *shift, *off_new; uint32_t nparts; };

nvdb_status launch_spread(nvdb_hip_ctx* c, hipStream_t s, const InsArray& a, const void* src, uint64_t src_row0, void* dst, const PlanImage& im, const InsSlab& sl) {
  const uint32_t nt = static_cast<uint32_t>((sl.s1 - sl.s0 + INS_TILE_ROWS - 1) / INS_TILE_ROWS);
  with_lane(a.row_bytes, [&](auto lane) {
    using LaneT = decltype(lane);
    insert_spread_kernel<LaneT><<<nt, INSERT_MOVE_THREADS, 0, s>>>(static_cast<const LaneT*>(src), src_row0, static_cast<LaneT*>(dst), im.off_old, im.shift, im.nparts,
                                                                    sl.s0, sl.s1, static_cast<uint32_t>(a.row_bytes / sizeof(LaneT)));
  });
  HIPCHK(c, hipGetLastError());
  return NVDB_OK;
}

nvdb_status launch_scatter(nvdb_hip_ctx* c, hipStream_t s, const InsArray& a, void* dst, const uint32_t* pos, uint64_t m) {
  const uint32_t nt = static_cast<uint32_t>((m + INS_TILE_ROWS - 1) / INS_TILE_ROWS);
  with_lane(a.row_bytes, [&](auto lane) {
    using LaneT = decltype(lane);
    insert_scatter_kernel<LaneT><<<nt, INSERT_MOVE_THREADS, 0, s>>>(static_cast<const LaneT*>(a.staged), static_cast<LaneT*>(dst), pos, m,
                                                                     static_cast<uint32_t>(a.row_bytes / sizeof(LaneT)));
  });
  HIPCHK(c, hipGetLastError());
  return NVDB_OK;
}

nvdb_status move_array(nvdb_hip_ctx* c, hipStream_t s, const InsArray& a, bool grow, const InsPlan& pl, const std::vector<InsSlab>& slabs, const PlanImage& im,
                       const uint32_t* pos) {
  char* dst = static_cast<char*>(grow ? a.fresh : a.p);
  if (grow && pl.lo) HIPCHK(c, hipMemcpyAsync(dst, a.p, pl.lo * a.row_bytes, hipMemcpyDeviceToDevice, s));
  for (const InsSlab& sl : slabs) {
    if (grow || sl.direct) {
      if (nvdb_status st = launch_spread(c, s, a, a.p, 0, dst, im, sl)) return st;
      continue;
    }
    HIPCHK(c, hipMemcpyAsync(c->cp_bounce.p, static_cast<const char*>(a.p) + sl.s0 * a.row_bytes, (sl.s1 - sl.s0) * a.row_bytes, hipMemcpyDeviceToDevice, s));
    if (nvdb_status st = launch_spread(c, s, a, c->cp_bounce.p, sl.s0, dst, im, sl)) return st;
  }
  if (nvdb_status st = launch_scatter(c, s, a, dst, pos, pl.m)) return st;
  const size_t n_new = static_cast<size_t>(pl.n + pl.m);
  HIPCHK(c, hipMemsetAsync(dst + n_new * a.row_bytes, 0, arr_tail(a, n_new), s));
  return NVDB_OK;
}

struct DevTmp {
  void* p = nullptr;
  DevTmp() = default;
  DevTmp(const DevTmp&) = delete;
  DevTmp& operator=(const DevTmp&) = delete;
  ~DevTmp() { if (p) (void)hipFree(p); }
};
nvdb_status tmp_alloc(nvdb_hip_ctx* c, DevTmp& t, size_t bytes) {
  HIPCHK(c, hipMalloc(&t.p, std::max<size_t>(bytes, 256)));
  return NVDB_OK;
}

nvdb_status read_bits(nvdb_hip_ctx* c, hipStream_t s, const uint32_t* bits, uint32_t hb[2]) {
  HIPCHK(c, hipMemcpyAsync(hb, bits, 8, hipMemcpyDeviceToHost, s));
  HIPCHK(c, hipStreamSynchronize(s));
  return NVDB_OK;
}
inline float as_float(uint32_t b) { float f; std::memcpy(&f, &b, 4); return f; }

template <int DT>
nvdb_status launch_norm(nvdb_hip_ctx* c, hipStream_t s, const void* rows, const float* scales, uint64_t m, uint32_t dim, uint32_t* bits) {
  HIPCHK(c, hipMemsetAsync(bits, 0, 8, s));
  const unsigned grid = static_cast<unsigned>(std::min<uint64_t>((m + 3) / 4, 4096));
  row_norm_max_kernel<DT><<<grid, 256, 0, s>>>(rows, scales, m, dim, bits);
  HIPCHK(c, hipGetLastError());
  return NVDB_OK;
}

}

nvdb_status insert_stage(nvdb_hip_ctx* c, const char* who, const void* rows, const float* scales, uint64_t m, bool needs_table, const uint32_t* part_of,
                         InsertStage& stage, bool* done) {
  *done = true;
  const std::string w(who);
  if (!c->rows || c->n == 0) return fail(c, NVDB_ERR_NO_CORPUS, "Empty base");
  if (!c->owned) return fail(c, NVDB_ERR_UNSUPPORTED, w + ": an adopted corpus is the caller's memory (unpadded, not moved)");
  if (m == 0) return NVDB_OK;
  if (!rows) return fail(c, NVDB_ERR_INVALID, w + ": null rows");
  if (c->dtype == NVDB_DTYPE_I8 && !scales) return fail(c, NVDB_ERR_INVALID, w + ": int8 corpus needs per-row scales");
  const bool table = c->parts && !c->parts->offsets.empty();
  if ((needs_table || part_of) && !table) return fail(c, NVDB_ERR_INVALID, w + ": part_of without a partition table (nvdb_hip_set_partitions)");
  if (part_of) {
    const uint64_t nparts = c->parts->offsets.size() - 1;
    for (uint64_t i = 0; i < m; ++i)
      if (part_of[i] >= nparts) return fail(c, NVDB_ERR_INVALID, w + ": an entry of part_of is >= the number of partitions");
  }
  if (m >= 0xFFFFFFF0ull - c->n) return fail(c, NVDB_ERR_UNSUPPORTED, w + ": corpus shard must hold fewer than 2^32-16 rows (shard it)");
  if ((table || c->nmasks) && c->n + m > ROW_MASK_MAX_ROWS) return fail(c, NVDB_ERR_UNSUPPORTED, w + ": too many rows for the resident partition table / row masks");
  HIPCHK(c, hipSetDevice(c->device));
  const size_t rb = static_cast<size_t>(c->dim) * bpe_of(c->dtype);
  HIPCHK(c, hipMalloc(&stage.rows, std::max<size_t>(m * rb, 256)));
  if (c->dtype == NVDB_DTYPE_I8) HIPCHK(c, hipMalloc(reinterpret_cast<void**>(&stage.scales), std::max<size_t>(m * 4, 256)));
  HIPCHK(c, hipMemcpyAsync(stage.rows, rows, m * rb, hipMemcpyHostToDevice, c->stream));
  if (stage.scales) HIPCHK(c, hipMemcpyAsync(stage.scales, scales, m * 4, hipMemcpyHostToDevice, c->stream));
  HIPCHK(c, hipStreamSynchronize(c->stream));
  *done = false;
  return NVDB_OK;
}

nvdb_status insert_staged(nvdb_hip_ctx* c, const char* who, const InsertStage& stage, uint64_t m, const uint32_t* part_of, uint64_t* out_new_rows, uint64_t* out_n,
                          InsPlan* out_plan) {
  const std::string w(who);
  hipStream_t s = c->stream;
  nvdb_status st;
  const uint64_t n = c->n, n_new = n + m;
  const bool table = c->parts && !c->parts->offsets.empty();

  const uint64_t whole[2] = {0, n};
  const uint64_t* offsets = table ? c->parts->offsets.data() : whole;
  const uint32_t nparts = table ? static_cast<uint32_t>(c->parts->offsets.size() - 1) : 1u;
  InsPlan pl;
  std::vector<uint64_t> new_rows(m);
  if (!ins_plan(offsets, nparts, part_of, m, pl, new_rows.data())) return fail(c, NVDB_ERR_INVALID, w + ": an entry of part_of is >= the number of partitions");
  const bool grow = n_new > c->cap_rows;
  const uint64_t new_cap = grow ? ins_capacity(n, m, c->cap_rows, static_cast<uint64_t>(c->opt_insert_growth_pct)) : c->cap_rows;

  HIPCHK(c, hipSetDevice(c->device));
  if ((st = ensure(c, c->misc, 64))) return st;
  uint32_t* bits = static_cast<uint32_t*>(c->misc.p) + 8;
  uint32_t hb[2] = {0, 0};
  if (c->dtype == NVDB_DTYPE_F32) st = launch_norm<DT_F32>(c, s, stage.rows, stage.scales, m, c->dim, bits);
  else if (c->dtype == NVDB_DTYPE_F16) st = launch_norm<DT_F16>(c, s, stage.rows, stage.scales, m, c->dim, bits);
  else st = launch_norm<DT_I8>(c, s, stage.rows, stage.scales, m, c->dim, bits);
  if (st || (st = read_bits(c, s, bits, hb))) return st;
  const float new_max_norm = as_float(hb[0]);
  const bool new_signed = hb[1] != 0;
  float new_filter_norm = 0.f, new_resid = 0.f;
  bool shadow_bad = false;
  DevTmp sh8, sh8s, sh16;
  const void* staged_sh8s = nullptr;
  if (c->q8shadow) {
    if ((st = tmp_alloc(c, sh8, m * c->dim)) || (st = tmp_alloc(c, sh8s, m * 4))) return st;
    HIPCHK(c, hipMemsetAsync(bits, 0, 8, s));
    const unsigned grid = static_cast<unsigned>(std::min<uint64_t>((m + 3) / 4, 4096));
    if (c->dtype == NVDB_DTYPE_F32) shadow_q8_kernel<float><<<grid, 256, 0, s>>>(static_cast<const float*>(stage.rows), static_cast<signed char*>(sh8.p), static_cast<float*>(sh8s.p), m, c->dim, c->dim, bits);
    else shadow_q8_kernel<_Float16><<<grid, 256, 0, s>>>(static_cast<const _Float16*>(stage.rows), static_cast<signed char*>(sh8.p), static_cast<float*>(sh8s.p), m, c->dim, c->dim, bits);
    HIPCHK(c, hipGetLastError());
    if ((st = read_bits(c, s, bits, hb))) return st;
    new_resid = as_float(hb[0]);
    shadow_bad = hb[1] != 0;
    if (!shadow_bad) {
      if ((st = launch_norm<DT_I8>(c, s, sh8.p, static_cast<const float*>(sh8s.p), m, c->dim, bits)) || (st = read_bits(c, s, bits, hb))) return st;
      new_filter_norm = as_float(hb[0]);
    }
    staged_sh8s = sh8s.p;
  } else if (c->shadow8) {
    if ((st = tmp_alloc(c, sh8, m * c->fdim))) return st;
    const unsigned grid = static_cast<unsigned>(std::min<uint64_t>((m * c->fdim + 255) / 256, 4096));
    shadow_i8_kernel<<<grid, 256, 0, s>>>(static_cast<const signed char*>(stage.rows), static_cast<signed char*>(sh8.p), m, c->dim, c->fdim);
    HIPCHK(c, hipGetLastError());
    staged_sh8s = stage.scales;
  }
  if (c->shadow16) {
    if ((st = tmp_alloc(c, sh16, m * c->fdim * 2))) return st;
    HIPCHK(c, hipMemsetAsync(bits, 0, 8, s));
    const unsigned grid = static_cast<unsigned>(std::min<uint64_t>((m * c->fdim + 255) / 256, 4096));
    if (c->dtype == NVDB_DTYPE_F32) shadow_f16_kernel<float><<<grid, 256, 0, s>>>(static_cast<const float*>(stage.rows), static_cast<_Float16*>(sh16.p), m, c->dim, c->fdim, bits);
    else shadow_f16_kernel<_Float16><<<grid, 256, 0, s>>>(static_cast<const _Float16*>(stage.rows), static_cast<_Float16*>(sh16.p), m, c->dim, c->fdim, bits);
    HIPCHK(c, hipGetLastError());
    if ((st = read_bits(c, s, bits, hb))) return st;
    if (!(as_float(hb[0]) < 60000.f)) shadow_bad = true;
  }

  std::vector<InsArray> arrays = corpus_arrays(c, !shadow_bad);
  for (InsArray& a : arrays)
    a.staged = a.kind == ARR_ROWS ? stage.rows : a.kind == ARR_SCALES ? static_cast<const void*>(stage.scales) : a.kind == ARR_SH8 ? sh8.p : a.kind == ARR_SH8S ? staged_sh8s : sh16.p;
  std::vector<uint64_t> meta;
  meta.insert(meta.end(), pl.off_old.begin(), pl.off_old.end());
  meta.insert(meta.end(), pl.shift.begin(), pl.shift.end());
  meta.insert(meta.end(), pl.off_new.begin(), pl.off_new.end());
  std::vector<uint32_t> pos32(new_rows.begin(), new_rows.end());
  if ((st = ensure(c, c->ins_meta, meta.size() * 8)) || (st = ensure(c, c->ins_pos, m * 4))) return st;
  HIPCHK(c, hipMemcpyAsync(c->ins_meta.p, meta.data(), meta.size() * 8, hipMemcpyHostToDevice, s));
  HIPCHK(c, hipMemcpyAsync(c->ins_pos.p, pos32.data(), m * 4, hipMemcpyHostToDevice, s));
  const uint64_t* d_meta = static_cast<const uint64_t*>(c->ins_meta.p);
  const PlanImage im{d_meta, d_meta + nparts + 1, d_meta + 2 * static_cast<size_t>(nparts) + 1, nparts};
  std::vector<InsSlab> slabs;
  ins_slabs(pl, static_cast<uint64_t>(c->opt_compact_slab_rows), slabs);
  if (!grow) {
    size_t bounce = 0;
    for (const InsSlab& sl : slabs)
      if (!sl.direct)
        for (const InsArray& a : arrays) bounce = std::max(bounce, static_cast<size_t>(sl.s1 - sl.s0) * a.row_bytes);
    if (bounce && (st = ensure(c, c->cp_bounce, bounce))) return st;
  }

  const uint32_t W = static_cast<uint32_t>(rm_words(n)), W2 = static_cast<uint32_t>(rm_words(n_new));
  if (c->nmasks) {
    if ((st = ensure(c, c->row_masks_alt, static_cast<size_t>(c->nmasks) * W2 * 4))) return st;
    insert_planes_kernel<<<dim3((W2 + 255) / 256, c->nmasks), 256, 0, s>>>(static_cast<const uint32_t*>(c->row_masks.p), W, static_cast<uint32_t*>(c->row_masks_alt.p), W2,
                                                                           im.off_old, im.off_new, nparts, n_new);
    HIPCHK(c, hipGetLastError());
  }
  if (grow && (st = alloc_fresh(c, arrays, new_cap, who))) return st;
  if (hipStreamSynchronize(s) != hipSuccess) {
    free_fresh(arrays);
    return fail(c, NVDB_ERR_HIP, w + ": staging failed on the device");
  }

  for (const InsArray& a : arrays)
    if ((st = move_array(c, s, a, grow, pl, slabs, im, static_cast<const uint32_t*>(c->ins_pos.p)))) break;
  if (!st && hipStreamSynchronize(s) != hipSuccess) st = fail(c, NVDB_ERR_HIP, w + ": the move failed on the device");
  if (!st) {
    if (grow) adopt_fresh(c, arrays, new_cap);
    c->n = n_new;
    if (shadow_bad) st = corpus_rederive(c);
  }
  if (st) {
    const std::string why = c->err;
    (void)hipGetLastError();
    free_fresh(arrays);
    corpus_drop(c);
    return fail(c, NVDB_ERR_HIP, why + " (the corpus was dropped: load it again)");
  }
  if (!shadow_bad) {
    c->max_norm = std::max(c->max_norm, new_max_norm);
    if (c->q8shadow) {
      c->filter_max_norm = std::max(c->filter_max_norm, new_filter_norm);
      c->resid_max = std::max(c->resid_max, new_resid);
    } else {
      c->filter_max_norm = c->max_norm;
      c->i8_scales_signed = c->i8_scales_signed || new_signed;
    }
  }
  if (table) c->parts->offsets = pl.off_new;
  if (c->nmasks) {
    std::swap(c->row_masks, c->row_masks_alt);
    for (uint64_t& live : c->mask_live) live += m;
  }
  c->range_valid = false; c->range_total = 0;
  if (out_new_rows) std::copy(new_rows.begin(), new_rows.end(), out_new_rows);
  if (out_n) *out_n = n_new;
  if (out_plan) *out_plan = std::move(pl);
  return NVDB_OK;
}

}

extern "C" {

nvdb_status nvdb_hip_reserve_rows(nvdb_hip_ctx* c, uint64_t rows) {
  if (!c) return NVDB_ERR_INVALID;
  if (!c->rows || c->n == 0) return fail(c, NVDB_ERR_NO_CORPUS, "Empty base");
  if (!c->owned) return fail(c, NVDB_ERR_UNSUPPORTED, "reserve_rows: an adopted corpus is the caller's memory");
  if (rows <= c->cap_rows) return NVDB_OK;
  if (rows >= 0xFFFFFFF0ull) return fail(c, NVDB_ERR_UNSUPPORTED, "reserve_rows: corpus shard must hold fewer than 2^32-16 rows (shard it)");
  HIPCHK(c, hipSetDevice(c->device));
  hipStream_t s = c->stream;
  std::vector<InsArray> arrays = corpus_arrays(c, true);
  if (nvdb_status st = alloc_fresh(c, arrays, rows, "reserve_rows")) return st;
  hipError_t e = hipSuccess;
  for (const InsArray& a : arrays) {
    const size_t used = static_cast<size_t>(c->n) * a.row_bytes;
    if (e == hipSuccess) e = hipMemcpyAsync(a.fresh, a.p, used, hipMemcpyDeviceToDevice, s);
    if (e == hipSuccess) e = hipMemsetAsync(static_cast<char*>(a.fresh) + used, 0, arr_tail(a, c->n), s);
  }
  if (e == hipSuccess) e = hipStreamSynchronize(s);
  if (e != hipSuccess) {
    free_fresh(arrays);
    (void)hipGetLastError();
    return fail(c, NVDB_ERR_HIP, std::string("reserve_rows: ") + hipGetErrorString(e));
  }
  adopt_fresh(c, arrays, rows);
  return NVDB_OK;
}

nvdb_status nvdb_hip_insert_rows(nvdb_hip_ctx* c, const void* rows, const float* scales, uint64_t m, const uint32_t* part_of, uint64_t* out_new_rows, uint64_t* out_n) {
  if (!c) return NVDB_ERR_INVALID;
  InsertStage stage;
  bool done = false;
  if (nvdb_status st = insert_stage(c, "insert_rows", rows, scales, m, false, part_of, stage, &done)) return st;
  if (done) {
    if (out_n) *out_n = c->n;
    return NVDB_OK;
  }
  return insert_staged(c, "insert_rows", stage, m, part_of, out_new_rows, out_n);
}

}
```

nano-vectordb_amd/csrc/nvdb_ivf.cpp:

```cpp
#include "nvdb_ctx.h"
#include "compact_plan.h"
#include "insert_plan.h"
#include "nvdb_insert.h"
#include "nvdb_parts.h"
#include "ivf_layout.h"
#include "row_mask.h"
#include "kernels_ivf.h"

namespace nvdbhip {
namespace {

constexpr uint32_t ASSIGN_BATCH = 1024;

std::string g_ivf_build_err;

struct DevMem {
  void* p = nullptr;
  DevMem() = default;
  DevMem(const DevMem&) = delete;
  DevMem& operator=(const DevMem&) = delete;
  ~DevMem() { if (p) (void)hipFree(p); }
  template <typename T> T* as() const { return static_cast<T*>(p); }
};
nvdb_status dev_alloc(nvdb_hip_ctx* c, DevMem& m, size_t bytes) {
// ... 170 lines not shown

nvdb_status nvdb_hip_assign_rows(nvdb_hip_ctx* c, const float* centroids, uint32_t nparts, uint64_t row0, uint64_t nrows, uint32_t* out_assign) {
  nvdb_status st = ivf_args(c, nparts, "assign_rows");
  if (st) return st;
  if (!centroids) return fail(c, NVDB_ERR_INVALID, "assign_rows: null centroids");
  if (row0 > c->n || nrows > c->n - row0) return fail(c, NVDB_ERR_INVALID, "assign_rows: row range out of bounds");
  if (nrows == 0) return NVDB_OK;
  if (!out_assign) return fail(c, NVDB_ERR_INVALID, "assign_rows: null output");
  Coarse co;
  if ((st = coarse_load(c, co, centroids, nparts, "assign_rows"))) return st;
  return assign_core(c, co.ctx, nparts, RowSel{row0, nullptr, nrows}, out_assign, "assign_rows");
}

nvdb_status nvdb_hip_train_centroids(nvdb_hip_ctx* c, uint32_t nparts, uint32_t iters, uint64_t seed, uint64_t max_train_rows,
                                     const float* init, float* out_centroids) {
  nvdb_status st = ivf_args(c, nparts, "train_centroids");
  if (st) return st;
  if (!out_centroids) return fail(c, NVDB_ERR_INVALID, "train_centroids: null output");
  const uint64_t n = c->n, m = (max_train_rows == 0 || max_train_rows >= n) ? n : max_train_rows;
  if (nparts > m) return fail(c, NVDB_ERR_INVALID, "train_centroids: more centroids than training rows");
  if (m > IVF_MAX_ROWS) return fail(c, NVDB_ERR_UNSUPPORTED, "train_centroids: training set too large (max_train_rows)");
  HIPCHK(c, hipSetDevice(c->device));
  hipStream_t s = c->stream;
  const uint32_t dim = c->dim;
  const size_t cen_count = static_cast<size_t>(nparts) * dim;

  std::vector<uint32_t> train_rows;
  DevMem d_train;
  if (m < n) {
    train_rows.resize(m);
    for (uint64_t i = 0; i < m; ++i) train_rows[i] = static_cast<uint32_t>(i * n / m);
    if ((st = dev_alloc(c, d_train, m * 4))) return st;
    HIPCHK(c, hipMemcpy(d_train.p, train_rows.data(), m * 4, hipMemcpyHostToDevice));
  }
  const RowSel train{0, m < n ? d_train.as<uint32_t>() : nullptr, m};
  auto corpus_row = [&](uint64_t t) { return m < n ? train_rows[t] : static_cast<uint32_t>(t); };

  std::vector<float> cen(cen_count);
  DevMem d_cen;
  if ((st = dev_alloc(c, d_cen, cen_count * 4))) return st;
  if (init) std::memcpy(cen.data(), init, cen_count * 4);
  else {
    std::vector<bool> taken(m, false);
    std::vector<uint32_t> pick(nparts);
    for (uint32_t j = 0; j < nparts; ++j) {
      uint64_t t = train_draw(seed, j, 0, m);
      for (uint32_t a = 1; taken[t] && a < 64; ++a) t = train_draw(seed, j, a, m);
      while (taken[t]) t = t + 1 < m ? t + 1 : 0;
      taken[t] = true;
      pick[j] = corpus_row(t);
    }
    DevMem d_pick;
    if ((st = dev_alloc(c, d_pick, static_cast<size_t>(nparts) * 4))) return st;
    HIPCHK(c, hipMemcpyAsync(d_pick.p, pick.data(), static_cast<size_t>(nparts) * 4, hipMemcpyHostToDevice, s));
    if ((st = launch_rows_to_f32(c, s, RowSel{0, d_pick.as<uint32_t>(), nparts}, 0, nparts, d_cen.as<float>()))) return st;
    HIPCHK(c, hipMemcpyAsync(cen.data(), d_cen.p, cen_count * 4, hipMemcpyDeviceToHost, s));
    HIPCHK(c, hipStreamSynchronize(s));
    for (uint32_t j = 0; j < nparts; ++j) {
      float* v = cen.data() + static_cast<size_t>(j) * dim;
      double ss = 0.0;
      for (uint32_t k = 0; k < dim; ++k) ss += static_cast<double>(v[k]) * v[k];
      const double norm = std::sqrt(ss);
      if (!(norm > 0.0) || !std::isfinite(norm)) continue;
      for (uint32_t k = 0; k < dim; ++k) v[k] = static_cast<float>(static_cast<double>(v[k]) / norm);
    }
  }

  if (iters) {
    Coarse co;
    std::vector<uint32_t> assign(m), perm(m), members, chunk_first(static_cast<size_t>(nparts) + 1);
    std::vector<uint64_t> offsets(static_cast<size_t>(nparts) + 1);
    std::vector<uint2> chunks;
    const size_t max_chunks = m / IVF_SUM_CHUNK_ROWS + nparts;
    DevMem d_members, d_chunks, d_first, d_partial;
    if ((st = dev_alloc(c, d_members, m * 4))) return st;
    if ((st = dev_alloc(c, d_chunks, max_chunks * sizeof(uint2)))) return st;
    if ((st = dev_alloc(c, d_first, chunk_first.size() * 4))) return st;
    if ((st = dev_alloc(c, d_partial, max_chunks * dim * sizeof(double)))) return st;
    const bool dbg = ivf_debug();
    StreamTimer t_assign(dbg, s), t_update(dbg, s);
    float ms_assign = 0.f, ms_update = 0.f;
    for (uint32_t it = 0; it < iters; ++it) {
      if ((st = coarse_load(c, co, cen.data(), nparts, "train_centroids"))) return st;
      t_assign.start();
      if ((st = assign_core(c, co.ctx, nparts, train, assign.data(), "train_centroids"))) return st;
      ms_assign += t_assign.stop();
      if (!ivf_layout(assign.data(), m, nparts, offsets.data(), perm.data())) return fail(c, NVDB_ERR_INTERNAL, "train_centroids: assignment out of range");
      const uint32_t* mem = perm.data();
      if (m < n) {
        members.resize(m);
        for (uint64_t j = 0; j < m; ++j) members[j] = train_rows[perm[j]];
        mem = members.data();
      }
      chunks.clear();
      for (uint32_t p = 0; p < nparts; ++p) {
        chunk_first[p] = static_cast<uint32_t>(chunks.size());
        for (uint64_t b = offsets[p]; b < offsets[p + 1]; b += IVF_SUM_CHUNK_ROWS)
          chunks.push_back(make_uint2(static_cast<uint32_t>(b), static_cast<uint32_t>(std::min<uint64_t>(b + IVF_SUM_CHUNK_ROWS, offsets[p + 1]))));
      }
      chunk_first[nparts] = static_cast<uint32_t>(chunks.size());
      HIPCHK(c, hipMemcpyAsync(d_members.p, mem, m * 4, hipMemcpyHostToDevice, s));
      HIPCHK(c, hipMemcpyAsync(d_chunks.p, chunks.data(), chunks.size() * sizeof(uint2), hipMemcpyHostToDevice, s));
      HIPCHK(c, hipMemcpyAsync(d_first.p, chunk_first.data(), chunk_first.size() * 4, hipMemcpyHostToDevice, s));
      HIPCHK(c, hipMemcpyAsync(d_cen.p, cen.data(), cen_count * 4, hipMemcpyHostToDevice, s));
      t_update.start();
      if ((st = launch_centroid_sum(c, s, d_members.as<uint32_t>(), d_chunks.as<uint2>(), static_cast<uint32_t>(chunks.size()), d_partial.as<double>()))) return st;
      centroid_finish_kernel<<<nparts, 256, 0, s>>>(d_partial.as<double>(), d_first.as<uint32_t>(), dim, d_cen.as<float>());
      HIPCHK(c, hipGetLastError());
      ms_update += t_update.stop();
      HIPCHK(c, hipMemcpyAsync(cen.data(), d_cen.p, cen_count * 4, hipMemcpyDeviceToHost, s));
      HIPCHK(c, hipStreamSynchronize(s));
    }
    if (dbg) std::fprintf(stderr, "[nvdb ivf] train: %u iterations over %llu rows, %u centroids: assignment %.1f ms, member sums + normalisation %.2f ms (hipEvents)\n",
                          iters, static_cast<unsigned long long>(m), nparts, ms_assign, ms_update);
  }
  std::memcpy(out_centroids, cen.data(), cen_count * 4);
  return NVDB_OK;
}

nvdb_status nvdb_hip_ivf_build(nvdb_hip_ctx* src, const float* centroids, uint32_t nparts, nvdb_hip_ivf** out) {
  if (!out) return NVDB_ERR_INVALID;
  *out = nullptr;
  if (!src) { g_ivf_build_err = "ivf_build: null source context"; return NVDB_ERR_INVALID; }
  auto src_fail = [&](nvdb_status st) { g_ivf_build_err = src->err; return st; };
  nvdb_status st = ivf_args(src, nparts, "ivf_build");
  if (st) return src_fail(st);
  if (!centroids) return src_fail(fail(src, NVDB_ERR_INVALID, "ivf_build: null centroids"));
  if (src->n > IVF_MAX_ROWS) return src_fail(fail(src, NVDB_ERR_UNSUPPORTED, "ivf_build: corpus shard too large"));
  const uint64_t n = src->n;
  const bool dbg = ivf_debug();

  auto ix = new nvdb_hip_ivf();
  auto bail = [&](nvdb_status s_, const std::string& msg) { g_ivf_build_err = msg; nvdb_hip_ivf_destroy(ix); return s_; };
  std::vector<uint32_t> assign(n);
  float ms_assign = 0.f, ms_gather = 0.f;
  {
    Coarse co;
    if ((st = coarse_load(src, co, centroids, nparts, "ivf_build"))) return bail(st, src->err);
    StreamTimer t(dbg, src->stream);
    t.start();
    if ((st = assign_core(src, co.ctx, nparts, RowSel{0, nullptr, n}, assign.data(), "ivf_build"))) return bail(st, src->err);
    ms_assign = t.stop();
  }
  ix->perm.resize(n);
  ix->offsets.resize(static_cast<size_t>(nparts) + 1);
  ix->src_row_base = src->row_base;
  ix->src_n = n;
  if (!ivf_layout(assign.data(), n, nparts, ix->offsets.data(), ix->perm.data())) return bail(NVDB_ERR_INTERNAL, "ivf_build: assignment out of range");

  if ((st = nvdb_hip_create(src->device, &ix->ctx))) return bail(st, std::string("ivf_build: ") + nvdb_hip_last_error(nullptr));
  nvdb_hip_ctx* c = ix->ctx;
  auto ctx_fail = [&](nvdb_status s_) { return bail(s_, "ivf_build: " + c->err); };
  c->opt_f32_shadow = src->opt_f32_shadow;
  c->opt_q8_shadow = src->opt_q8_shadow > 0 ? 1 : 0;
  void* rows = nullptr;
  float* scales = nullptr;
  {
    DevMem d_perm;
    if ((st = dev_alloc(c, d_perm, n * 4))) return ctx_fail(st);
    if ((st = corpus_alloc_padded(c, n, src->dim, src->dtype, &rows, &scales))) return ctx_fail(st);
    auto gather = [&]() -> nvdb_status {
      HIPCHK(c, hipStreamSynchronize(src->stream));
      HIPCHK(c, hipMemcpyAsync(d_perm.p, ix->perm.data(), n * 4, hipMemcpyHostToDevice, c->stream));
      StreamTimer t(dbg, c->stream);
      t.start();
      if (nvdb_status g = launch_gather_rows(c, c->stream, src, d_perm.as<uint32_t>(), rows, scales)) return g;
      ms_gather = t.stop();
      HIPCHK(c, hipStreamSynchronize(c->stream));
      return NVDB_OK;
    };
    if ((st = gather())) { (void)hipFree(rows); if (scales) (void)hipFree(scales); return ctx_fail(st); }
  }
  if ((st = corpus_take_ownership(c, rows, scales, n, src->dim, src->dtype, 0))) return ctx_fail(st);
  if ((st = nvdb_hip_set_partitions(c, ix->offsets.data(), nparts))) return ctx_fail(st);
  if ((st = nvdb_hip_set_centroids(c, centroids))) return ctx_fail(st);
  if (dbg) {
    const double bytes = 2.0 * static_cast<double>(n) * src->dim * bpe_of(src->dtype);
    std::fprintf(stderr, "[nvdb ivf] build: %llu rows, %u lists: assignment %.1f ms, gather %.3f ms (%.2f TB/s read + written) (hipEvents)\n",
                 static_cast<unsigned long long>(n), nparts, ms_assign, ms_gather, ms_gather > 0.f ? bytes / (ms_gather * 1e9) : 0.0);
  }
  *out = ix;
  return NVDB_OK;
}

void nvdb_hip_ivf_destroy(nvdb_hip_ivf* ix) {
  if (!ix) return;
  if (ix->ctx) nvdb_hip_destroy(ix->ctx);
  delete ix;
}

const char* nvdb_hip_ivf_last_error(const nvdb_hip_ivf* ix) { return ix ? ix->err.c_str() : g_ivf_build_err.c_str(); }

nvdb_hip_ctx* nvdb_hip_ivf_ctx(nvdb_hip_ivf* ix) { return ix ? ix->ctx : nullptr; }

nvdb_status nvdb_hip_ivf_info(const nvdb_hip_ivf* ix, uint64_t* n, uint32_t* nparts, uint64_t* offsets_out, uint32_t* perm_out) {
  if (!ix) return NVDB_ERR_INVALID;
  if (n) *n = ix->perm.size();
  if (nparts) *nparts = static_cast<uint32_t>(ix->offsets.size() - 1);
  if (offsets_out) std::memcpy(offsets_out, ix->offsets.data(), ix->offsets.size() * sizeof(uint64_t));
  if (perm_out && !ix->perm.empty()) std::memcpy(perm_out, ix->perm.data(), ix->perm.size() * sizeof(uint32_t));
  return NVDB_OK;
}

nvdb_status nvdb_hip_ivf_search(nvdb_hip_ivf* ix, const float* queries, uint32_t nq, uint32_t k, uint32_t nprobe, uint64_t* out_ids,
                                float* out_scores, uint32_t* out_counts, uint32_t* out_probe, nvdb_hip_timing* timing) {
  if (!ix) return NVDB_ERR_INVALID;
  if (nvdb_status st = ivf_forward(ix, nvdb_hip_search_ivf(ix->ctx, queries, nq, k, nprobe, out_ids, out_scores, out_counts, out_probe, timing))) return st;
  if (nq && k) ivf_map_ids(ix, out_ids, static_cast<uint64_t>(nq) * k);
  return NVDB_OK;
}

nvdb_status nvdb_hip_ivf_set_row_masks(nvdb_hip_ivf* ix, const uint32_t* bits, uint32_t nmasks) {
  if (!ix) return NVDB_ERR_INVALID;
  nvdb_status st;
  if (!bits || nmasks == 0 || nmasks == 0xFFFFFFFFu) st = nvdb_hip_set_row_masks(ix->ctx, nullptr, nmasks);
  else {
    const uint64_t n = ix->perm.size(), W = rm_words(n), Wsrc = rm_words(ix->src_n);
    std::vector<uint32_t> planes(static_cast<size_t>(nmasks) * W);
    for (uint32_t m = 0; m < nmasks; ++m) rm_permute(bits + static_cast<size_t>(m) * Wsrc, ix->perm.data(), n, planes.data() + static_cast<size_t>(m) * W);
    st = nvdb_hip_set_row_masks(ix->ctx, planes.data(), nmasks);
  }
  if (st) ix->err = nvdb_hip_last_error(ix->ctx);
  return st;
}

nvdb_status nvdb_hip_ivf_update_row_mask(nvdb_hip_ivf* ix, uint32_t mask, const uint64_t* rows, uint64_t nrows, int live) {
  if (!ix) return NVDB_ERR_INVALID;
  const uint64_t n = ix->src_n;
  if (nrows && !rows) { ix->err = "ivf_update_row_mask: null row list"; return NVDB_ERR_INVALID; }
  if (!rm_rows_valid(rows, nrows, n)) { ix->err = "ivf_update_row_mask: a listed row is >= the row count"; return NVDB_ERR_INVALID; }
  if (ix->inv.empty() && nrows) {
    ix->inv.resize(n);
    if (!cp_inverse(ix->perm.data(), ix->perm.size(), n, ix->inv.data())) { ix->inv.clear(); ix->err = "ivf_update_row_mask: the index's permutation is damaged"; return NVDB_ERR_INTERNAL; }
  }
  std::vector<uint64_t> pos;
  pos.reserve(nrows);
  for (uint64_t i = 0; i < nrows; ++i)
    if (ix->inv[rows[i]] != 0xFFFFFFFFu) pos.push_back(ix->inv[rows[i]]);
  const nvdb_status st = nvdb_hip_update_row_mask(ix->ctx, mask, pos.data(), pos.size(), live);
  if (st) ix->err = nvdb_hip_last_error(ix->ctx);
  return st;
}

nvdb_status nvdb_hip_ivf_compact(nvdb_hip_ivf* ix, uint32_t mask, uint64_t* out_n) {
  if (!ix) return NVDB_ERR_INVALID;
  std::vector<uint32_t> old_rows(ix->perm.size());
  uint64_t n_new = 0;
  const nvdb_status st = nvdb_hip_compact_rows(ix->ctx, mask, &n_new, old_rows.data());
  if (st) {
    ix->err = nvdb_hip_last_error(ix->ctx);
    if (!ix->ctx->rows) {
      ix->perm.clear(); ix->inv.clear();
      std::fill(ix->offsets.begin(), ix->offsets.end(), 0);
    }
    return st;
  }
  if (n_new == ix->perm.size()) {
    if (out_n) *out_n = n_new;
    return NVDB_OK;
  }
  cp_offsets_from_map(old_rows.data(), n_new, ix->offsets.data(), ix->offsets.size(), ix->offsets.data());
  cp_perm(ix->perm.data(), old_rows.data(), n_new);
  ix->perm.resize(n_new);
  ix->inv.clear();
  if (out_n) *out_n = n_new;
  return NVDB_OK;
}

nvdb_status nvdb_hip_ivf_add_rows(nvdb_hip_ivf* ix, const void* rows, const float* scales, uint64_t m, uint64_t* out_first_id, uint32_t* out_assign) {
  if (!ix) return NVDB_ERR_INVALID;
  nvdb_hip_ctx* c = ix->ctx;
  auto ctx_fail = [&](nvdb_status st) {
    ix->err = c->err;
    if (!c->rows) {
      ix->perm.clear(); ix->inv.clear();
      std::fill(ix->offsets.begin(), ix->offsets.end(), 0);
    }
    return st;
  };
  if (m > IVF_MAX_ROWS || ix->src_n + m > IVF_MAX_ROWS) { ix->err = "ivf_add_rows: too many rows for one index"; return NVDB_ERR_UNSUPPORTED; }
  InsertStage stage;
  bool done = false;
  nvdb_status st = insert_stage(c, "ivf_add_rows", rows, scales, m, true, nullptr, stage, &done);
  if (st) return ctx_fail(st);
  if (done) {
    if (out_first_id) *out_first_id = ix->src_n;
    return NVDB_OK;
  }
  PartState* ps = c->parts;
  if (!ps || !ps->have_centroids || !ps->coarse) return ctx_fail(fail(c, NVDB_ERR_INVALID, "ivf_add_rows: the index has no centroids"));
  const uint32_t nparts = static_cast<uint32_t>(ix->offsets.size() - 1);
  std::vector<uint32_t> assign(m);
  if ((st = assign_core(c, ps->coarse, nparts, RowSel{0, nullptr, m, stage.rows, stage.scales}, assign.data(), "ivf_add_rows"))) return ctx_fail(st);
  InsPlan pl;
  std::vector<uint64_t> new_rows(m);
  if ((st = insert_staged(c, "ivf_add_rows", stage, m, assign.data(), new_rows.data(), nullptr, &pl))) return ctx_fail(st);
  ins_perm(ix->perm, ix->inv, pl, new_rows.data(), ix->src_n);
  ix->offsets = pl.off_new;
  if (out_first_id) *out_first_id = ix->src_n;
  if (out_assign) std::copy(assign.begin(), assign.end(), out_assign);
  ix->src_n += m;
  return NVDB_OK;
}

nvdb_status nvdb_hip_ivf_search_masked(nvdb_hip_ivf* ix, const float* queries, uint32_t nq, uint32_t k, uint32_t nprobe, const uint32_t* mask_of,
                                       uint64_t* out_ids, float* out_scores, uint32_t* out_counts, uint32_t* out_probe, nvdb_hip_timing* timing) {
// ... 29 lines not shown
```

nano-vectordb_amd/csrc/nvdb_launch_i8.cpp:

```cpp
#include "nvdb_ctx.h"
#include "kernels_filter_i8s.h"

namespace nvdbhip {

nvdb_status launch_prep_q8(nvdb_hip_ctx* c, hipStream_t s, const float* dev_q, uint32_t nq, uint32_t nq_pad, const PrepInit& pinit) {
  prep_q8_kernel<<<nq_pad, 256, 0, s>>>(dev_q, nq, c->dim, c->fdim, prep_norm(c, c->filter_max_norm), c->q8shadow ? prep_norm(c, c->resid_max) : 0.f, static_cast<signed char*>(c->q16.p),
                                        static_cast<signed char*>(c->q16.p) + static_cast<size_t>(nq_pad) * c->fdim,
                                        static_cast<float*>(c->qscale.p), static_cast<float*>(c->qinv.p),
                                        static_cast<float*>(c->ebound.p), static_cast<float*>(c->slack.p), static_cast<float*>(c->qdelta.p),
                                        static_cast<uint32_t*>(c->overflow.p), static_cast<uint32_t>(c->opt_i8_lo_bits), pinit);
  HIPCHK(c, hipGetLastError());
  return NVDB_OK;
}

#ifdef NVDB_HIP_DEV
template <int DIM>
nvdb_status launch_filter_i8_dim(nvdb_hip_ctx* c, FilterRun& run, RowRange rows) {
  const uint32_t nwg = filter_grid(c, run.QT);
  nvdb_status st;
  SyncArgs sy;
  if ((st = sibling_sync_args(c, run, nwg, sy))) return st;
  return launch_filter_i8_kernel(c, run, rows, run.QT, sy.prog ? filter_i8_kernel<DIM, false, 6, true> : filter_i8_kernel<DIM>, nwg, FilterGeom{256, filter_i8_lds_bytes<DIM>(), 4, true},
                                 static_cast<size_t>(run.nq_pad) * DIM, &c->hitlog, scatter_args(c, run, FILTER_ROWS), 0u, sy.prog, sy.mask, sy.lead);
}
#endif

template <int DIM, int NB, int MB> auto i8w_build(bool sync) { return sync ? filter_i8w_kernel<DIM, NB, 6, true, MB> : filter_i8w_kernel<DIM, NB, 6, false, MB>; }
template <int DIM, int WPB, bool DEFER> auto i8p_build(bool sync) { return sync ? filter_i8p_kernel<DIM, true, false, 6, WPB, DEFER> : filter_i8p_kernel<DIM, false, false, 6, WPB, DEFER>; }
template <int DIM, int WPB> auto i8s_build(bool sync) { return sync ? filter_i8s_kernel<DIM, true, false, 6, WPB> : filter_i8s_kernel<DIM, false, false, 6, WPB>; }

template <int DIM, int NB>
nvdb_status launch_filter_i8w_dim(nvdb_hip_ctx* c, FilterRun& run, RowRange rows) {
  constexpr uint32_t TROWS = i8w_tile_rows(DIM);
  static_assert(TROWS == I8W_TILE_ROWS, "the builds of dims <= 768 stream two 32-row blocks per tile");
  if ((rows.hi - rows.lo) % TROWS) return fail(c, NVDB_ERR_INTERNAL, "int8 two-stage kernel: row range is not a multiple of its 64-row tile");
  const bool pipe = i8_pipelined(c, run.kind, NB);
  const bool defer = i8_stage2_in_loop(c), logs = i8_logs_survivors(c, run.kind, NB);
#ifdef NVDB_HIP_DEV
  const bool w8 = pipe && c->opt_i8_waves8 && DIM != 384;
  constexpr bool HAS_I8W = true, HAS_I8P32 = true, DEV_I8S8_512 = true;
#else
  constexpr bool DEV_I8S8_512 = false;
  constexpr bool w8 = false;
  constexpr bool HAS_I8W = (NB == 1);
  constexpr bool HAS_I8P32 = (DIM < 384);
#endif
  const uint32_t nwg = filter_grid(c, run.QT);
  nvdb_status st;
  SyncArgs sy;
  if ((st = sibling_sync_args(c, run, nwg, sy))) return st;
  const bool sync = sy.prog != nullptr;
  auto launch = [&](auto kern, uint32_t waves, size_t lds) {
    return launch_filter_i8w_kernel(c, run, rows, kern, nwg, FilterGeom{64 * waves, lds, 8, true}, static_cast<size_t>(run.nq_pad) * DIM, TROWS, sy);
  };
  if constexpr (NB == 1 && (DIM == 768 || DIM == 512))
    if (c->opt_i8_small8 && !defer && run.QT == 1 && run.nq > 8)
      return launch(filter_i8s_kernel<DIM, false, false, 6, 8>, 8, filter_i8s_lds_bytes<DIM, 8>());
  if constexpr (NB == 1 && DIM == 384)
    if (c->opt_i8_small8 && !defer && run.QT == 1 && run.nq > 64)
      return launch(filter_i8s_kernel<DIM, false, false, 6, 4>, 4, filter_i8s_lds_bytes<DIM, 4>());
  if (logs && c->opt_i8_mfma16) {
    if constexpr (DIM == 768 || (DEV_I8S8_512 && DIM == 512))
      if ((w8 || c->opt_i8_dense8) && DIM == 768) return launch(i8s_build<DIM, 8>(sync), 8, filter_i8s_lds_bytes<DIM, 8>());
    if constexpr (DIM >= 384)
      if (!w8) return launch(i8s_build<DIM, 4>(sync), 4, filter_i8s_lds_bytes<DIM, 4>());
  }
#ifdef NVDB_HIP_DEV
  if constexpr (DIM != 384)
    if (w8) return launch(i8p_build<DIM, 8, true>(sync), 8, filter_i8p_lds_bytes<DIM, 8, true>());
#endif
  if (pipe && defer) return launch(i8p_build<DIM, 4, true>(sync), 4, filter_i8p_lds_bytes<DIM, 4, true>());
  if constexpr (HAS_I8P32)
    if (pipe) return launch(i8p_build<DIM, 4, false>(sync), 4, filter_i8p_lds_bytes<DIM, 4, false>());
  if constexpr (HAS_I8W)
    if (!pipe) return launch(i8w_build<DIM, NB, 2>(sync), 4, filter_i8w_lds_bytes<DIM, 2>());
  return fail(c, NVDB_ERR_INTERNAL, "int8 two-stage kernel: no build for this batch");
}

template <int DIM>
nvdb_status launch_filter_i8w_big_dim(nvdb_hip_ctx* c, FilterRun& run, RowRange rows) {
  constexpr uint32_t TROWS = i8w_tile_rows(DIM);
  static_assert(TROWS == FILTER_ROWS, "the builds of dims > 768 stream one 32-row block per tile");
  if ((rows.hi - rows.lo) % TROWS) return fail(c, NVDB_ERR_INTERNAL, "int8 kernel: row range is not a multiple of its 32-row tile");
  const uint32_t nwg = filter_grid(c, run.QT);
  nvdb_status st;
  SyncArgs sy;
  if ((st = sibling_sync_args(c, run, nwg, sy))) return st;
  return launch_filter_i8w_kernel(c, run, rows, i8w_build<DIM, 1, 1>(sy.prog != nullptr), nwg, FilterGeom{256, filter_i8w_lds_bytes<DIM, 1>(), 4, true},
                                  static_cast<size_t>(run.nq_pad) * DIM, TROWS, sy);
}

template <int DIM>
nvdb_status launch_boot_i8_dim(nvdb_hip_ctx* c, FilterRun& run, RowRange rows) {
  const uint32_t QT = run.nq_pad / 128u;
  return launch_filter_i8_kernel(c, run, rows, QT, filter_i8_kernel<DIM, true>, filter_grid(c, QT), FilterGeom{256, filter_i8_lds_bytes<DIM>(), 0, false},
                                 static_cast<size_t>(run.nq_pad) * DIM, &c->cand, scatter_args(c, run, FILTER_ROWS), run.cap, static_cast<uint32_t*>(nullptr), 0u, 0u);
}

nvdb_status launch_boot_i8(nvdb_hip_ctx* c, FilterRun& run, uint32_t n0) {
  nvdb_status st;
  if (dispatch_dim(I8Dims{}, c->fdim, st, [&](auto D) { return launch_boot_i8_dim<decltype(D)::value>(c, run, RowRange{0, n0}); })) return st;
  return fail(c, NVDB_ERR_UNSUPPORTED, "int8 boot kernel: unsupported dim");
}

nvdb_status launch_filter_i8(nvdb_hip_ctx* c, FilterRun& run, RowRange rows) {
  const uint32_t nb = filter_nb(c, run.kind, run.nq);
  nvdb_status st;
  if (dispatch_dim(I8DimsBig{}, c->fdim, st, [&](auto D) { return launch_filter_i8w_big_dim<decltype(D)::value>(c, run, rows); })) return st;
  if (i8_two_stage(c, run.kind) && dispatch_dim(I8Dims{}, c->fdim, st, [&](auto D) {
        return nb == 2 ? launch_filter_i8w_dim<decltype(D)::value, 2>(c, run, rows) : launch_filter_i8w_dim<decltype(D)::value, 1>(c, run, rows);
      })) return st;
#ifdef NVDB_HIP_DEV
  if (dispatch_dim(I8Dims{}, c->fdim, st, [&](auto D) { return launch_filter_i8_dim<decltype(D)::value>(c, run, rows); })) return st;
#endif
  return fail(c, NVDB_ERR_UNSUPPORTED, "int8 filter kernel: unsupported dim");
}

}
```

nano-vectordb_amd/nvdb_amd/__init__.py:

```python
import ctypes as C
import os

import numpy as np

_HERE = os.path.dirname(os.path.abspath(__file__))
LIB_PATH = os.path.join(os.path.dirname(_HERE), "lib", "libnvdb_hip.so")
DEV_LIB_PATH = os.path.join(os.path.dirname(_HERE), "lib", "libnvdb_hip_dev.so")

DT_F32, DT_F16, DT_I8 = 1, 2, 3
REFINE_KMAX = 64
_NP_OF = {DT_F32: np.float32, DT_F16: np.uint16, DT_I8: np.int8}

EXPORTS = [
    "nvdb_hip_abi_version", "nvdb_hip_device_count", "nvdb_hip_create", "nvdb_hip_destroy", "nvdb_hip_last_error",
    "nvdb_hip_upload_corpus", "nvdb_hip_adopt_corpus", "nvdb_hip_generate_corpus", "nvdb_hip_corpus_info",
    "nvdb_hip_download_rows", "nvdb_hip_search_batch", "nvdb_hip_search_batch_dev", "nvdb_hip_search_check",
    "nvdb_hip_get_stats", "nvdb_hip_range_search", "nvdb_hip_range_results", "nvdb_hip_shadow_info", "nvdb_hip_collect_kernel_times", "nvdb_hip_merge_topk_dev", "nvdb_hip_merge_topk_strided_dev", "nvdb_merge_topk_host", "nvdb_hip_set_option",
    "nvdb_hip_refine_l2_topk", "nvdb_hip_refine_l2_topk_dev", "nvdb_synth_rows_f32", "nvdb_f32_to_f16",
    "nvdb_quantize_i8_rows",
    "nvdb_hip_group_create", "nvdb_hip_group_destroy", "nvdb_hip_group_last_error", "nvdb_hip_group_size", "nvdb_hip_group_ctx",
    "nvdb_hip_group_exchange", "nvdb_hip_group_upload_corpus", "nvdb_hip_group_generate_corpus", "nvdb_hip_group_set_option",
    "nvdb_hip_group_search_batch",
    "nvdb_hip_set_partitions", "nvdb_hip_set_centroids", "nvdb_hip_search_partitions", "nvdb_hip_search_ivf",
    "nvdb_hip_assign_rows", "nvdb_hip_train_centroids", "nvdb_ivf_layout_host",
    "nvdb_hip_ivf_build", "nvdb_hip_ivf_destroy", "nvdb_hip_ivf_last_error", "nvdb_hip_ivf_ctx", "nvdb_hip_ivf_info", "nvdb_hip_ivf_search",
    "nvdb_hip_set_row_masks", "nvdb_hip_update_row_mask", "nvdb_hip_get_row_masks", "nvdb_hip_search_partitions_masked",
    "nvdb_hip_search_ivf_masked", "nvdb_hip_search_batch_masked",
    "nvdb_hip_ivf_set_row_masks", "nvdb_hip_ivf_update_row_mask", "nvdb_hip_ivf_search_masked",
    "nvdb_hip_range_search_partitions", "nvdb_hip_range_search_ivf", "nvdb_hip_range_search_masked",
    "nvdb_hip_ivf_range_search", "nvdb_hip_ivf_range_results",
    "nvdb_hip_search_partitions_anyk", "nvdb_hip_search_ivf_anyk", "nvdb_hip_ivf_search_anyk",
    "nvdb_hip_compact_rows", "nvdb_hip_ivf_compact",
    "nvdb_hip_reserve_rows", "nvdb_hip_insert_rows", "nvdb_hip_ivf_add_rows",
]
DEV_EXPORTS = ["nvdb_hip_debug_clock", "nvdb_hip_debug_clock_i8", "nvdb_permuted_tile", "nvdb_hip_debug_tile_ranges",
               "nvdb_hip_debug_plan"]


class NvdbError(RuntimeError):
    def __init__(self, status, msg):
        super().__init__(f"nvdb_hip status {status}: {msg}")
        self.status = status


class Timing(C.Structure):
    _fields_ = [("h2d_ms", C.c_float), ("kernel_ms", C.c_float), ("d2h_ms", C.c_float), ("total_ms", C.c_float),
                ("threads", C.c_uint32), ("nwarps", C.c_uint32), ("K", C.c_uint32), ("R", C.c_uint32),
                ("shmem_bytes", C.c_size_t), ("dbg_q", C.c_uint32),
                ("dbg_dist_cycles_avg", C.c_double), ("dbg_write_cycles_avg", C.c_double),
                ("dbg_merge_cycles_avg", C.c_double), ("dbg_dist_pct", C.c_double), ("dbg_write_pct", C.c_double),
                ("dbg_merge_pct", C.c_double)]


class ScanStats(C.Structure):
    _fields_ = [("path", C.c_uint32), ("chunks", C.c_uint32), ("rows_scanned", C.c_uint64), ("candidates", C.c_uint64),
                ("overflow_queries", C.c_uint32), ("bound_violations", C.c_uint32), ("filter_kernel_ms", C.c_float),
                ("other_kernel_ms", C.c_float), ("i8_stage1_tiles", C.c_uint32), ("i8_stage2_blocks", C.c_uint32),
                ("sticky_overflow", C.c_uint32), ("sticky_violations", C.c_uint32)]

    def as_dict(self):
        return {f: getattr(self, f) for f, _ in self._fields_}


class PlanShape(C.Structure):
    _fields_ = [("n", C.c_uint64), ("dim", C.c_uint32), ("fdim", C.c_uint32), ("dtype", C.c_uint32), ("owned", C.c_uint32),
                ("has_shadow16", C.c_uint32), ("has_shadow8", C.c_uint32), ("q8shadow", C.c_uint32), ("i8_scales_signed", C.c_uint32),
                ("num_cu", C.c_uint32), ("cap_hint", C.c_uint32), ("shadow_demoted", C.c_uint32), ("load_rule", C.c_uint32),
                ("free_hbm", C.c_uint64)]


class PlanOption(C.Structure):
    _fields_ = [("key", C.c_char_p), ("value", C.c_int64)]


PLAN_MAX_CHUNKS = 64


class Plan(C.Structure):
    _fields_ = [(f, C.c_uint32) for f in ("route", "prep", "prep_inits", "k_wide", "k_eff", "cap", "QPB", "QT", "nq_pad", "prog_words", "head",
                                          "padded", "perm_on", "boot", "tile_rows", "n_al", "growth", "boot_tiles", "boot_rows", "r0",
                                          "tail_exact", "helper_tile_rows", "n_chunks")] + \
               [("chunk_lo", C.c_uint32 * PLAN_MAX_CHUNKS), ("chunk_hi", C.c_uint32 * PLAN_MAX_CHUNKS), ("stat_chunks", C.c_uint32),
                ("stat_rows_scanned", C.c_uint64), ("filter_shadow", C.c_uint32)]


class GroupStats(C.Structure):
    _fields_ = [("shards", C.c_uint32), ("exchange", C.c_uint32), ("host_merge_fallbacks", C.c_uint32), ("bytes_per_rank", C.c_uint64)]

    def as_dict(self):
        return {f: getattr(self, f) for f, _ in self._fields_}


_lib = None
_dev_lib = None


def _share_hip_runtime_with_torch():
    import importlib.util
    spec = importlib.util.find_spec("torch")
    if spec is None or not spec.submodule_search_locations:
        return
    cand = os.path.join(list(spec.submodule_search_locations)[0], "lib", "libamdhip64.so")
    if os.path.exists(cand):
        C.CDLL(cand, mode=C.RTLD_GLOBAL)


def _share_rccl_with_torch():
    import importlib.util
    if importlib.util.find_spec("torch") is None:
        return
    import torch


def _bind(L, dev):
    vp, u32, u64, i64, f32p = C.c_void_p, C.c_uint32, C.c_uint64, C.c_int64, C.POINTER(C.c_float)
    L.nvdb_hip_abi_version.restype = C.c_int
    L.nvdb_hip_device_count.restype = C.c_int
    L.nvdb_hip_create.argtypes = [C.c_int, C.POINTER(vp)]
    L.nvdb_hip_destroy.argtypes = [vp]
    L.nvdb_hip_destroy.restype = None
    L.nvdb_hip_last_error.argtypes = [vp]
    L.nvdb_hip_last_error.restype = C.c_char_p
    L.nvdb_hip_upload_corpus.argtypes = [vp, vp, vp, u64, u32, u32, u64]
    L.nvdb_hip_adopt_corpus.argtypes = [vp, vp, vp, u64, u32, u32, u64]
    L.nvdb_hip_generate_corpus.argtypes = [vp, u64, u64, u32, u32, u64]
    L.nvdb_hip_corpus_info.argtypes = [vp, C.POINTER(u64), C.POINTER(u32), C.POINTER(u32), C.POINTER(u64), f32p]
    L.nvdb_hip_download_rows.argtypes = [vp, u64, u64, vp, vp]
    L.nvdb_hip_search_batch.argtypes = [vp, vp, u32, u32, vp, vp, C.POINTER(u32), C.POINTER(Timing)]
    L.nvdb_hip_search_batch_dev.argtypes = [vp, vp, u32, u32, vp, vp, vp]
    L.nvdb_hip_search_check.argtypes = [vp, C.POINTER(ScanStats)]
    L.nvdb_hip_get_stats.argtypes = [vp, C.POINTER(ScanStats)]
    L.nvdb_hip_range_search.argtypes = [vp, vp, u32, vp, vp, C.POINTER(Timing)]
    L.nvdb_hip_range_results.argtypes = [vp, vp, vp]
    L.nvdb_hip_shadow_info.argtypes = [vp, C.POINTER(u64)]
    L.nvdb_hip_collect_kernel_times.argtypes = [vp, C.POINTER(u32), C.POINTER(C.c_double), C.POINTER(C.c_double),
                                                C.POINTER(C.c_double)]
    L.nvdb_hip_merge_topk_dev.argtypes = [vp, vp, vp, u32, u32, u32, vp, vp, vp]
    L.nvdb_hip_merge_topk_strided_dev.argtypes = [vp, vp, vp, C.c_size_t, C.c_size_t, u32, u32, u32, vp, vp, vp]
    L.nvdb_merge_topk_host.argtypes = [vp, vp, u32, u32, u32, vp, vp]
    L.nvdb_hip_set_option.argtypes = [vp, C.c_char_p, i64]
    L.nvdb_hip_refine_l2_topk.argtypes = [vp, vp, vp, u32, u32, u32, vp, vp, C.POINTER(Timing)]
    L.nvdb_hip_refine_l2_topk_dev.argtypes = [vp, vp, vp, u32, u32, u32, vp, vp, vp]
    L.nvdb_synth_rows_f32.argtypes = [u64, u64, u64, u32, vp]
    L.nvdb_synth_rows_f32.restype = None
    L.nvdb_f32_to_f16.argtypes = [vp, vp, u64]
    L.nvdb_f32_to_f16.restype = None
    L.nvdb_quantize_i8_rows.argtypes = [vp, u64, u32, vp, vp]
    L.nvdb_quantize_i8_rows.restype = None
    L.nvdb_hip_group_create.argtypes = [C.POINTER(C.c_int), u32, C.POINTER(vp)]
    L.nvdb_hip_group_destroy.argtypes = [vp]
    L.nvdb_hip_group_destroy.restype = None
    L.nvdb_hip_group_last_error.argtypes = [vp]
    L.nvdb_hip_group_last_error.restype = C.c_char_p
    L.nvdb_hip_group_size.argtypes = [vp]
    L.nvdb_hip_group_size.restype = u32
    L.nvdb_hip_group_ctx.argtypes = [vp, u32]
    L.nvdb_hip_group_ctx.restype = vp
    L.nvdb_hip_group_exchange.argtypes = [vp, C.POINTER(C.c_char_p)]
    L.nvdb_hip_group_exchange.restype = C.c_int
    L.nvdb_hip_group_upload_corpus.argtypes = [vp, vp, vp, u64, u32, u32]
    L.nvdb_hip_group_generate_corpus.argtypes = [vp, u64, u64, u32, u32]
    L.nvdb_hip_group_set_option.argtypes = [vp, C.c_char_p, i64]
    L.nvdb_hip_group_search_batch.argtypes = [vp, vp, u32, u32, vp, vp, C.POINTER(u32), C.POINTER(GroupStats)]
    L.nvdb_hip_set_partitions.argtypes = [vp, vp, u32]
    L.nvdb_hip_set_centroids.argtypes = [vp, vp]
    L.nvdb_hip_search_partitions.argtypes = [vp, vp, u32, u32, vp, u32, vp, vp, vp, C.POINTER(Timing)]
    L.nvdb_hip_search_ivf.argtypes = [vp, vp, u32, u32, u32, vp, vp, vp, vp, C.POINTER(Timing)]
    L.nvdb_hip_assign_rows.argtypes = [vp, vp, u32, u64, u64, vp]
    L.nvdb_hip_train_centroids.argtypes = [vp, u32, u32, u64, u64, vp, vp]
    L.nvdb_ivf_layout_host.argtypes = [vp, u64, u32, vp, vp]
    L.nvdb_hip_ivf_build.argtypes = [vp, vp, u32, C.POINTER(vp)]
    L.nvdb_hip_ivf_destroy.argtypes = [vp]
    L.nvdb_hip_ivf_destroy.restype = None
    L.nvdb_hip_ivf_last_error.argtypes = [vp]
    L.nvdb_hip_ivf_last_error.restype = C.c_char_p
    L.nvdb_hip_ivf_ctx.argtypes = [vp]
    L.nvdb_hip_ivf_ctx.restype = vp
    L.nvdb_hip_ivf_info.argtypes = [vp, C.POINTER(u64), C.POINTER(u32), vp, vp]
    L.nvdb_hip_ivf_search.argtypes = [vp, vp, u32, u32, u32, vp, vp, vp, vp, C.POINTER(Timing)]
    L.nvdb_hip_set_row_masks.argtypes = [vp, vp, u32]
    L.nvdb_hip_update_row_mask.argtypes = [vp, u32, vp, u64, C.c_int]
    L.nvdb_hip_get_row_masks.argtypes = [vp, C.POINTER(u32), C.POINTER(u64), vp]
    L.nvdb_hip_search_partitions_masked.argtypes = [vp, vp, u32, u32, vp, u32, vp, vp, vp, vp, C.POINTER(Timing)]
    L.nvdb_hip_search_ivf_masked.argtypes = [vp, vp, u32, u32, u32, vp, vp, vp, vp, vp, C.POINTER(Timing)]
    L.nvdb_hip_search_batch_masked.argtypes = [vp, vp, u32, u32, vp, vp, vp, vp, C.POINTER(Timing)]
    L.nvdb_hip_ivf_set_row_masks.argtypes = [vp, vp, u32]
    L.nvdb_hip_ivf_update_row_mask.argtypes = [vp, u32, vp, u64, C.c_int]
    L.nvdb_hip_ivf_search_masked.argtypes = [vp, vp, u32, u32, u32, vp, vp, vp, vp, vp, C.POINTER(Timing)]
    L.nvdb_hip_range_search_partitions.argtypes = [vp, vp, u32, vp, vp, u32, vp, C.c_int, vp, C.POINTER(Timing)]
    L.nvdb_hip_range_search_ivf.argtypes = [vp, vp, u32, vp, u32, vp, C.c_int, vp, vp, C.POINTER(Timing)]
    L.nvdb_hip_range_search_masked.argtypes = [vp, vp, u32, vp, vp, vp, C.POINTER(Timing)]
    L.nvdb_hip_ivf_range_search.argtypes = [vp, vp, u32, vp, u32, vp, C.c_int, vp, vp, C.POINTER(Timing)]
    L.nvdb_hip_ivf_range_results.argtypes = [vp, vp, vp]
    L.nvdb_hip_search_partitions_anyk.argtypes = [vp, vp, u32, u32, vp, u32, vp, C.c_int, vp, vp, vp, C.POINTER(Timing)]
    L.nvdb_hip_search_ivf_anyk.argtypes = [vp, vp, u32, u32, u32, vp, C.c_int, vp, vp, vp, vp, C.POINTER(Timing)]
    L.nvdb_hip_ivf_search_anyk.argtypes = [vp, vp, u32, u32, u32, vp, C.c_int, vp, vp, vp, vp, C.POINTER(Timing)]
    L.nvdb_hip_compact_rows.argtypes = [vp, u32, C.POINTER(u64), vp]
    L.nvdb_hip_ivf_compact.argtypes = [vp, u32, C.POINTER(u64)]
    L.nvdb_hip_reserve_rows.argtypes = [vp, u64]
    L.nvdb_hip_insert_rows.argtypes = [vp, vp, vp, u64, vp, vp, C.POINTER(u64)]
    L.nvdb_hip_ivf_add_rows.argtypes = [vp, vp, vp, u64, C.POINTER(u64), vp]
    for name in EXPORTS:
        getattr(L, name)
    if dev:
        L.nvdb_hip_debug_clock.argtypes = [vp, C.c_int, u32, C.c_float, f32p]
        L.nvdb_hip_debug_clock_i8.argtypes = [vp, C.c_int, u32, C.c_float, f32p]
        L.nvdb_permuted_tile.argtypes = [u32, u32]
        L.nvdb_hip_debug_tile_ranges.argtypes = [vp, u32, u32, f32p, C.POINTER(u32), C.POINTER(u32), f32p]
        L.nvdb_permuted_tile.restype = u32
        L.nvdb_hip_debug_plan.argtypes = [C.POINTER(PlanShape), C.POINTER(PlanOption), u32, u32, u32, C.c_int, u32, C.POINTER(Plan), C.c_char_p, C.c_size_t]
    return L


def load_library():
    global _lib
    if _lib is not None:
        return _lib
    if not os.path.exists(LIB_PATH):
        raise ImportError(f"{LIB_PATH} is missing: build it with `make -C nano-vectordb_amd` "
                          "(python -c 'import __graft_entry__ as g; g.build()')")
    _share_hip_runtime_with_torch()
    _lib = _bind(C.CDLL(LIB_PATH), dev=False)
    return _lib


def load_dev_library():
    global _dev_lib
    if _dev_lib is not None:
        return _dev_lib
    if not os.path.exists(DEV_LIB_PATH):
        raise ImportError(f"{DEV_LIB_PATH} is missing: build it with `make -C nano-vectordb_amd`")
    _share_hip_runtime_with_torch()
    _dev_lib = _bind(C.CDLL(DEV_LIB_PATH), dev=True)
    return _dev_lib


def synth_rows_f32(seed, row0, nrows, dim):
    out = np.empty((nrows, dim), dtype=np.float32)
    load_library().nvdb_synth_rows_f32(seed, row0, nrows, dim, out.ctypes.data)
    return out


def f32_to_f16(x):
    x = np.ascontiguousarray(x, dtype=np.float32)
    out = np.empty(x.shape, dtype=np.uint16)
    load_library().nvdb_f32_to_f16(x.ctypes.data, out.ctypes.data, x.size)
    return out


def quantize_i8(rows):
    rows = np.ascontiguousarray(rows, dtype=np.float32)
    out = np.empty(rows.shape, dtype=np.int8)
    scales = np.empty(rows.shape[0], dtype=np.float32)
    load_library().nvdb_quantize_i8_rows(rows.ctypes.data, rows.shape[0], rows.shape[1], out.ctypes.data,
                                         scales.ctypes.data)
    return out, scales


def synth_corpus(seed, row0, nrows, dim, dtype):
    f = synth_rows_f32(seed, row0, nrows, dim)
    if dtype == DT_F32:
        return f, None
    if dtype == DT_F16:
        return f32_to_f16(f), None
    return quantize_i8(f)


def debug_plan(shape, nq, k, options=None, force_path=0, cap_override=0):
    sh = PlanShape(**{"fdim": shape["dim"], **shape})
    items = list((options or {}).items())
    opts = (PlanOption * max(len(items), 1))(*[PlanOption(key.encode(), int(v)) for key, v in items])
    out, err = Plan(), C.create_string_buffer(256)
    st = load_dev_library().nvdb_hip_debug_plan(C.byref(sh), opts, len(items), nq, k, force_path, cap_override, C.byref(out), err, len(err))
    if st:
        raise NvdbError(st, err.value.decode())
    p = {f: getattr(out, f) for f, _ in Plan._fields_}
    p["chunk_lo"], p["chunk_hi"] = list(out.chunk_lo[:out.n_chunks]), list(out.chunk_hi[:out.n_chunks])
    return p


def merge_topk_host(ids, scores):
    ids = np.ascontiguousarray(ids, dtype=np.uint64)
    scores = np.ascontiguousarray(scores, dtype=np.float32)
    s, nq, k = ids.shape
    oi = np.empty((nq, k), dtype=np.uint64)
    os_ = np.empty((nq, k), dtype=np.float32)
    st = load_library().nvdb_merge_topk_host(ids.ctypes.data, scores.ctypes.data, s, nq, k, oi.ctypes.data,
# ... 19 lines not shown
    words = (n + 31) // 32
    if masks.dtype == np.uint32:
        return np.ascontiguousarray(masks).reshape(-1, words)
    if masks.dtype != np.bool_:
        raise TypeError("row masks are bool [nmasks, n] or packed uint32 [nmasks, ceil(n / 32)]")
    masks = masks.reshape(-1, n)
    packed = np.zeros((masks.shape[0], words * 4), dtype=np.uint8)
    packed[:, :(n + 7) // 8] = np.packbits(masks, axis=1, bitorder="little")
    return np.ascontiguousarray(packed).view("<u4")


def unpack_row_masks(packed, n):
    packed = np.ascontiguousarray(packed, dtype="<u4")
    return np.unpackbits(packed.view(np.uint8), axis=1, bitorder="little")[:, :n].astype(bool)


def _mask_of_arg(mask_of, nq):
    if mask_of is None:
        return None
    return np.ascontiguousarray(np.broadcast_to(np.asarray(mask_of, dtype=np.uint32), (nq,)))


def _range_call(owner, last_error, results, call, queries, radius, mask_of, masked):
    queries = np.ascontiguousarray(queries, dtype=np.float32)
    if queries.ndim == 1:
        queries = queries[None, :]
    nq = queries.shape[0]
    radius = np.ascontiguousarray(np.broadcast_to(np.asarray(radius, dtype=np.float32), (nq,)))
    mo = _mask_of_arg(mask_of, nq)
    masked = (mo is not None) if masked is None else bool(masked)
    lims = np.zeros(nq + 1, dtype=np.uint64)
    st = call(queries, nq, radius, mo.ctypes.data if mo is not None else None, 1 if masked else 0, lims)
    if st:
        err = NvdbError(st, last_error())
        err.lims = lims
        raise err
    total = int(lims[nq])
    ids = np.empty(max(total, 1), dtype=np.uint64)
    scores = np.empty(max(total, 1), dtype=np.float32)
    owner._chk(results(ids.ctypes.data, scores.ctypes.data))
    return lims, ids[:total], scores[:total]


class HipContext:

    def __init__(self, device=0, dev=False):
        self.lib = load_dev_library() if dev else load_library()
        h = C.c_void_p()
        st = self.lib.nvdb_hip_create(device, C.byref(h))
        if st:
            raise NvdbError(st, self.lib.nvdb_hip_last_error(None).decode())
        self.h = h
        self.device = device

    def close(self):
        if getattr(self, "h", None):
            self.lib.nvdb_hip_destroy(self.h)
            self.h = None

    def __del__(self):
        try:
            self.close()
        except Exception:
            pass

    def _chk(self, st):
        if st:
            raise NvdbError(st, self.lib.nvdb_hip_last_error(self.h).decode())

    def upload_corpus(self, rows, dtype, scales=None, row_base=0):
        if dtype == DT_F16 and getattr(rows, "dtype", None) == np.float16:
            rows = rows.view(np.uint16)
        rows = np.ascontiguousarray(rows, dtype=_NP_OF[dtype])
        sc = np.ascontiguousarray(scales, dtype=np.float32) if scales is not None else None
        self._chk(self.lib.nvdb_hip_upload_corpus(self.h, rows.ctypes.data, sc.ctypes.data if sc is not None else None,
                                                  rows.shape[0], rows.shape[1], dtype, row_base))

    def adopt_corpus(self, dev_ptr, n, dim, dtype, dev_scales_ptr=None, row_base=0):
        self._chk(self.lib.nvdb_hip_adopt_corpus(self.h, dev_ptr, dev_scales_ptr, n, dim, dtype, row_base))

    def generate_corpus(self, seed, n, dim, dtype, row_base=0):
        self._chk(self.lib.nvdb_hip_generate_corpus(self.h, seed, n, dim, dtype, row_base))

    def corpus_info(self):
        n, dim, dt, base, mx = C.c_uint64(), C.c_uint32(), C.c_uint32(), C.c_uint64(), C.c_float()
        self._chk(self.lib.nvdb_hip_corpus_info(self.h, C.byref(n), C.byref(dim), C.byref(dt), C.byref(base), C.byref(mx)))
        return dict(n=n.value, dim=dim.value, dtype=dt.value, row_base=base.value, max_row_norm=mx.value)

    def download_rows(self, row0, nrows):
        info = self.corpus_info()
        out = np.empty((nrows, info["dim"]), dtype=_NP_OF[info["dtype"]])
        sc = np.empty(nrows, dtype=np.float32) if info["dtype"] == DT_I8 else None
        self._chk(self.lib.nvdb_hip_download_rows(self.h, row0, nrows, out.ctypes.data,
                                                  sc.ctypes.data if sc is not None else None))
        return out, sc

    def set_option(self, key, value):
        self._chk(self.lib.nvdb_hip_set_option(self.h, key.encode(), int(value)))

    def search_batch(self, queries, k, want_timing=False):
        queries = np.ascontiguousarray(queries, dtype=np.float32)
        if queries.ndim == 1:
            queries = queries[None, :]
        nq = queries.shape[0]
        ids = np.full((nq, max(k, 1)), np.iinfo(np.uint64).max, dtype=np.uint64)
        scores = np.full((nq, max(k, 1)), -np.inf, dtype=np.float32)
        keff = C.c_uint32(0)
        t = Timing()
        self._chk(self.lib.nvdb_hip_search_batch(self.h, queries.ctypes.data, nq, k, ids.ctypes.data, scores.ctypes.data,
                                                 C.byref(keff), C.byref(t) if want_timing else None))
        ke = keff.value if k > 0 else 0
        if want_timing:
            return ids[:, :ke], scores[:, :ke], t
        return ids[:, :ke], scores[:, :ke]

    def search_batch_dev(self, dev_q, nq, k, dev_out_ids, dev_out_scores, stream=None):
        self._chk(self.lib.nvdb_hip_search_batch_dev(self.h, dev_q, nq, k, dev_out_ids, dev_out_scores, stream))

    def search_check(self):
        s = ScanStats()
        self._chk(self.lib.nvdb_hip_search_check(self.h, C.byref(s)))
        return s.as_dict()

    def stats(self):
        s = ScanStats()
        self._chk(self.lib.nvdb_hip_get_stats(self.h, C.byref(s)))
        return s.as_dict()

    def range_search(self, queries, radius, want_timing=False):
        queries = np.ascontiguousarray(queries, dtype=np.float32)
        if queries.ndim == 1:
            queries = queries[None, :]
        nq = queries.shape[0]
        radius = np.ascontiguousarray(np.broadcast_to(np.asarray(radius, dtype=np.float32), (nq,)))
        lims = np.zeros(nq + 1, dtype=np.uint64)
        t = Timing()
        st = self.lib.nvdb_hip_range_search(self.h, queries.ctypes.data, nq, radius.ctypes.data, lims.ctypes.data,
                                            C.byref(t) if want_timing else None)
        if st:
            err = NvdbError(st, self.lib.nvdb_hip_last_error(self.h).decode())
            err.lims = lims
            raise err
        total = int(lims[nq])
        ids = np.empty(max(total, 1), dtype=np.uint64)
        scores = np.empty(max(total, 1), dtype=np.float32)
        self._chk(self.lib.nvdb_hip_range_results(self.h, ids.ctypes.data, scores.ctypes.data))
        return (lims, ids[:total], scores[:total], t) if want_timing else (lims, ids[:total], scores[:total])

    def shadow_info(self):
        out = (C.c_uint64 * 4)()
        self._chk(self.lib.nvdb_hip_shadow_info(self.h, out))
        return dict(resident=bool(out[0]), bytes=int(out[1]), demoted=bool(out[2]), last_filter=(None, "f16", "shadow", "i8")[out[3]])

    def collect_kernel_times(self):
        n, ms, fl, by = C.c_uint32(), C.c_double(), C.c_double(), C.c_double()
        self._chk(self.lib.nvdb_hip_collect_kernel_times(self.h, C.byref(n), C.byref(ms), C.byref(fl), C.byref(by)))
        return dict(launches=n.value, ms=ms.value, flops=fl.value, bytes=by.value)

    def merge_topk_dev(self, dev_ids, dev_scores, nshards, nq, k, dev_out_ids, dev_out_scores, stream=None):
        self._chk(self.lib.nvdb_hip_merge_topk_dev(self.h, dev_ids, dev_scores, nshards, nq, k, dev_out_ids,
                                                   dev_out_scores, stream))

    def merge_topk_strided_dev(self, dev_ids, dev_scores, stride_ids, stride_scores, nshards, nq, k, dev_out_ids, dev_out_scores,
                               stream=None):
        self._chk(self.lib.nvdb_hip_merge_topk_strided_dev(self.h, dev_ids, dev_scores, stride_ids, stride_scores, nshards, nq, k,
                                                           dev_out_ids, dev_out_scores, stream))

    def set_partitions(self, offsets):
        offsets = np.ascontiguousarray(offsets, dtype=np.uint64)
        self._chk(self.lib.nvdb_hip_set_partitions(self.h, offsets.ctypes.data, max(offsets.size, 1) - 1))

    def set_centroids(self, centroids):
        centroids = np.ascontiguousarray(centroids, dtype=np.float32)
        self._chk(self.lib.nvdb_hip_set_centroids(self.h, centroids.ctypes.data))

    def _probe_outputs(self, queries, k):
        queries = np.ascontiguousarray(queries, dtype=np.float32)
        if queries.ndim == 1:
            queries = queries[None, :]
        nq = queries.shape[0]
        ids = np.full((nq, k), np.iinfo(np.uint64).max, dtype=np.uint64)
        scores = np.full((nq, k), -np.inf, dtype=np.float32)
        return queries, nq, ids, scores, np.zeros(nq, dtype=np.uint32)

    def search_partitions(self, queries, k, probe, want_timing=False):
        queries, nq, ids, scores, counts = self._probe_outputs(queries, k)
        probe = np.ascontiguousarray(probe, dtype=np.uint32).reshape(nq, -1)
        t = Timing()
        self._chk(self.lib.nvdb_hip_search_partitions(self.h, queries.ctypes.data, nq, k, probe.ctypes.data, probe.shape[1],
                                                      ids.ctypes.data, scores.ctypes.data, counts.ctypes.data,
                                                      C.byref(t) if want_timing else None))
        return (ids, scores, counts, t) if want_timing else (ids, scores, counts)

    def search_ivf(self, queries, k, nprobe, want_probe=False):
        queries, nq, ids, scores, counts = self._probe_outputs(queries, k)
        probe = np.full((nq, nprobe), 0xFFFFFFFF, dtype=np.uint32)
        self._chk(self.lib.nvdb_hip_search_ivf(self.h, queries.ctypes.data, nq, k, nprobe, ids.ctypes.data, scores.ctypes.data,
                                               counts.ctypes.data, probe.ctypes.data if want_probe else None, None))
        return (ids, scores, counts, probe) if want_probe else (ids, scores, counts)

    def set_row_masks(self, masks):
        if masks is None or (isinstance(masks, (int, np.integer)) and not isinstance(masks, (bool, np.bool_))):
            self._chk(self.lib.nvdb_hip_set_row_masks(self.h, None, int(masks or 0)))
            return
        packed = pack_row_masks(masks, self.corpus_info()["n"])
        self._chk(self.lib.nvdb_hip_set_row_masks(self.h, packed.ctypes.data, packed.shape[0]))

    def update_row_mask(self, mask, rows, live):
        rows = np.ascontiguousarray(rows, dtype=np.uint64).ravel()
        self._chk(self.lib.nvdb_hip_update_row_mask(self.h, mask, rows.ctypes.data if rows.size else None, rows.size, 1 if live else 0))

    def get_row_masks(self):
        nm, w = C.c_uint32(), C.c_uint64()
        self._chk(self.lib.nvdb_hip_get_row_masks(self.h, C.byref(nm), C.byref(w), None))
        out = np.zeros((nm.value, w.value), dtype=np.uint32)
        if out.size:
            self._chk(self.lib.nvdb_hip_get_row_masks(self.h, None, None, out.ctypes.data))
        return out

    def compact_rows(self, mask=0):
        n_old = self.corpus_info()["n"]
        old = np.zeros(max(n_old, 1), dtype=np.uint32)
        n_new = C.c_uint64(0)
        self._chk(self.lib.nvdb_hip_compact_rows(self.h, mask, C.byref(n_new), old.ctypes.data))
        return n_new.value, old[:n_new.value].copy()

    def reserve_rows(self, rows):
        self._chk(self.lib.nvdb_hip_reserve_rows(self.h, int(rows)))

    def insert_rows(self, rows, scales=None, part_of=None):
        info = self.corpus_info()
        if info["dtype"] == DT_F16 and getattr(rows, "dtype", None) == np.float16:
            rows = rows.view(np.uint16)
        rows = np.ascontiguousarray(rows, dtype=_NP_OF[info["dtype"]]).reshape(-1, info["dim"])
        m = rows.shape[0]
        sc = np.ascontiguousarray(scales, dtype=np.float32) if scales is not None else None
        po = np.ascontiguousarray(part_of, dtype=np.uint32).ravel() if part_of is not None else None
        if po is not None and po.size != m:
            raise ValueError("part_of must have one entry per row")
        new_rows = np.zeros(max(m, 1), dtype=np.uint64)
        n_new = C.c_uint64(0)
        self._chk(self.lib.nvdb_hip_insert_rows(self.h, rows.ctypes.data if m else None, sc.ctypes.data if sc is not None else None, m,
                                                po.ctypes.data if po is not None else None, new_rows.ctypes.data, C.byref(n_new)))
        return n_new.value, new_rows[:m].copy()

    def search_partitions_masked(self, queries, k, probe, mask_of=None, want_timing=False):
        queries, nq, ids, scores, counts = self._probe_outputs(queries, k)
        probe = np.ascontiguousarray(probe, dtype=np.uint32).reshape(nq, -1)
        mo = _mask_of_arg(mask_of, nq)
        t = Timing()
        self._chk(self.lib.nvdb_hip_search_partitions_masked(self.h, queries.ctypes.data, nq, k, probe.ctypes.data, probe.shape[1],
                                                             mo.ctypes.data if mo is not None else None, ids.ctypes.data,
                                                             scores.ctypes.data, counts.ctypes.data, C.byref(t) if want_timing else None))
        return (ids, scores, counts, t) if want_timing else (ids, scores, counts)

    def search_ivf_masked(self, queries, k, nprobe, mask_of=None, want_probe=False):
        queries, nq, ids, scores, counts = self._probe_outputs(queries, k)
        probe = np.full((nq, nprobe), 0xFFFFFFFF, dtype=np.uint32)
        mo = _mask_of_arg(mask_of, nq)
        self._chk(self.lib.nvdb_hip_search_ivf_masked(self.h, queries.ctypes.data, nq, k, nprobe, mo.ctypes.data if mo is not None else None,
                                                      ids.ctypes.data, scores.ctypes.data, counts.ctypes.data,
                                                      probe.ctypes.data if want_probe else None, None))
        return (ids, scores, counts, probe) if want_probe else (ids, scores, counts)

    def search_masked(self, queries, k, mask_of=None, want_timing=False):
        queries, nq, ids, scores, counts = self._probe_outputs(queries, k)
        mo = _mask_of_arg(mask_of, nq)
        t = Timing()
        self._chk(self.lib.nvdb_hip_search_batch_masked(self.h, queries.ctypes.data, nq, k, mo.ctypes.data if mo is not None else None,
                                                        ids.ctypes.data, scores.ctypes.data, counts.ctypes.data,
                                                        C.byref(t) if want_timing else None))
        return (ids, scores, counts, t) if want_timing else (ids, scores, counts)

    def search_partitions_anyk(self, queries, k, probe, mask_of=None, masked=None, want_timing=False):
        queries, nq, ids, scores, counts = self._probe_outputs(queries, k)
        probe = np.ascontiguousarray(probe, dtype=np.uint32).reshape(nq, -1)
        mo = _mask_of_arg(mask_of, nq)
        masked = (mo is not None) if masked is None else bool(masked)
        t = Timing()
        self._chk(self.lib.nvdb_hip_search_partitions_anyk(self.h, queries.ctypes.data, nq, k, probe.ctypes.data, probe.shape[1],
                                                           mo.ctypes.data if mo is not None else None, 1 if masked else 0, ids.ctypes.data,
                                                           scores.ctypes.data, counts.ctypes.data, C.byref(t) if want_timing else None))
        return (ids, scores, counts, t) if want_timing else (ids, scores, counts)

    def search_ivf_anyk(self, queries, k, nprobe, mask_of=None, masked=None, want_probe=False):
        queries, nq, ids, scores, counts = self._probe_outputs(queries, k)
        probe = np.full((nq, nprobe), 0xFFFFFFFF, dtype=np.uint32)
        mo = _mask_of_arg(mask_of, nq)
        masked = (mo is not None) if masked is None else bool(masked)
        self._chk(self.lib.nvdb_hip_search_ivf_anyk(self.h, queries.ctypes.data, nq, k, nprobe, mo.ctypes.data if mo is not None else None,
                                                    1 if masked else 0, ids.ctypes.data, scores.ctypes.data, counts.ctypes.data,
                                                    probe.ctypes.data if want_probe else None, None))
        return (ids, scores, counts, probe) if want_probe else (ids, scores, counts)

    def _range(self, call, queries, radius, mask_of, masked):
        return _range_call(self, lambda: self.lib.nvdb_hip_last_error(self.h).decode(),
                           lambda i, s: self.lib.nvdb_hip_range_results(self.h, i, s), call, queries, radius, mask_of, masked)

    def range_search_partitions(self, queries, radius, probe, mask_of=None, masked=None):
        def call(q, nq, r, mo, masked_, lims):
            pr = np.ascontiguousarray(probe, dtype=np.uint32).reshape(nq, -1)
            return self.lib.nvdb_hip_range_search_partitions(self.h, q.ctypes.data, nq, r.ctypes.data, pr.ctypes.data, pr.shape[1], mo, masked_,
                                                             lims.ctypes.data, None)
        return self._range(call, queries, radius, mask_of, masked)

    def range_search_ivf(self, queries, radius, nprobe, mask_of=None, masked=None, want_probe=False):
# ... 279 lines not shown
```

Before: 161,100.

## Quantise i8 shadow with one common scale and use a scalar-threshold filter kernel

```diff
diff --git a/include/nvdb_hip.h b/include/nvdb_hip.h
--- a/include/nvdb_hip.h
+++ b/include/nvdb_hip.h
@@ -93,6 +93,8 @@
 
 nvdb_status nvdb_hip_shadow_info(const nvdb_hip_ctx* ctx, uint64_t* out4);
 
+nvdb_status nvdb_hip_shadow_scale_info(const nvdb_hip_ctx* ctx, double* out4);
+
 nvdb_status nvdb_hip_merge_topk_dev(nvdb_hip_ctx* ctx, const uint64_t* dev_ids, const float* dev_scores,
                                     uint32_t nshards, uint32_t nq, uint32_t k, uint64_t* dev_out_ids,
                                     float* dev_out_scores, void* hip_stream);
diff --git a/nano-vectordb_amd/csrc/kernels_corpus.h b/nano-vectordb_amd/csrc/kernels_corpus.h
--- a/nano-vectordb_amd/csrc/kernels_corpus.h
+++ b/nano-vectordb_amd/csrc/kernels_corpus.h
@@ -67,9 +67,9 @@
 
 template <typename SrcT>
 __global__ __launch_bounds__(256) void shadow_q8_kernel(const SrcT* __restrict__ src, signed char* __restrict__ dst, float* __restrict__ dst_scales,
-                                                        uint64_t n, uint32_t dim, uint32_t sdim, uint32_t* __restrict__ out_bits) {
+                                                        uint64_t n, uint32_t dim, uint32_t sdim, float common_scale, uint32_t* __restrict__ out_bits) {
   const int lane = threadIdx.x & 63;
-  float wres = 0.f;
+  float wres = 0.f, wscale = 0.f;
   bool bad = false;
   for (uint64_t r = static_cast<uint64_t>(blockIdx.x) * 4 + (threadIdx.x >> 6); r < n; r += static_cast<uint64_t>(gridDim.x) * 4) {
     const SrcT* row = src + r * dim;
@@ -77,23 +77,24 @@
     for (uint32_t c = lane; c < dim; c += 64) mx = fmaxf(mx, fabsf(static_cast<float>(row[c])));
     for (int o = 32; o > 0; o >>= 1) mx = fmaxf(mx, __shfl_xor(mx, o));
     if (!(mx < 3.0e38f)) bad = true;
-    const float scale = mx > 0.f ? mx / 127.f : 1.f;
+    wscale = fmaxf(wscale, mx / 127.f);
+    const float scale = common_scale > 0.f ? common_scale : mx > 0.f ? mx / 127.f : 1.f;
     const float inv = 1.0f / scale;
     float ss = 0.f;
-    signed char* out = dst + r * sdim;
     for (uint32_t c = lane; c < sdim; c += 64) {
       float qv = 0.f, x = 0.f;
       if (c < dim) { x = static_cast<float>(row[c]); qv = fminf(fmaxf(rintf(x * inv), -127.f), 127.f); }
-      out[c] = static_cast<signed char>(static_cast<int>(qv));
+      if (dst) dst[r * sdim + c] = static_cast<signed char>(static_cast<int>(qv));
       const float d = x - qv * scale;
       ss = __builtin_fmaf(d, d, ss);
     }
     for (int o = 32; o > 0; o >>= 1) ss += __shfl_xor(ss, o);
     if (!(ss == ss)) bad = true;
-    if (lane == 0) dst_scales[r] = scale;
+    if (dst && lane == 0) dst_scales[r] = scale;
     wres = fmaxf(wres, sqrtf(ss) * 1.0001f);
   }
   if (lane == 0 && wres > 0.f) atomicMax(out_bits, __builtin_bit_cast(uint32_t, wres));
+  if (lane == 0 && wscale > 0.f && wscale < 3.0e38f) atomicMax(out_bits + 2, __builtin_bit_cast(uint32_t, wscale));
   if (lane == 0 && (bad || !(wres < 3.0e38f))) out_bits[1] = 1u;
 }
 
diff --git a/nano-vectordb_amd/csrc/kernels_filter_i8s.h b/nano-vectordb_amd/csrc/kernels_filter_i8s.h
--- a/nano-vectordb_amd/csrc/kernels_filter_i8s.h
+++ b/nano-vectordb_amd/csrc/kernels_filter_i8s.h
@@ -1,5 +1,6 @@
 #pragma once
 #include "kernels_filter.h"
+#include "shadow_scale_plan.h"
 
 namespace nvdbhip {
 
@@ -279,4 +280,247 @@
   verify_and_scatter_i8<DIM>(mylog, wcnt, sa, lane, rows, qlo, thr, qscale, qinv);
 }
 
+static_assert(SHADOW_CS_ACC_BIAS == I8_ACC_BIAS && SHADOW_CS_H_MAX == 128 * static_cast<int>(I8_HI_L1_MAX), "shadow_scale_plan.h restates the accumulator bias and the range of H");
+template <int DIM, bool SYNC = false, int RING = 6, int WPB = 4>
+__global__ __launch_bounds__(64 * WPB, 1) void shadow_i8c_kernel(
+    const signed char* __restrict__ rows, const float* __restrict__ scales, uint32_t row_lo, uint32_t row_hi,
+    const signed char* __restrict__ qhi, const signed char* __restrict__ qlo, uint32_t nq, uint32_t QT,
+    const float* __restrict__ thr, const float* __restrict__ qscale, const float* __restrict__ qinv,
+    const float* __restrict__ qdelta, Hit* __restrict__ hitlog, ScatterArgs sa, uint32_t* __restrict__ prog,
+    uint32_t sync_mask, uint32_t sync_lead, uint32_t* __restrict__ stage_counts) {
+  static_assert(WPB == 4 || WPB == 8, "4 waves x 64 queries or 8 waves x 32 queries");
+  constexpr int NB = 16 / WPB, MB = 2;
+  constexpr int NV = 8 * NB;
+  constexpr int KS = DIM / 64;
+  constexpr int ROW_BYTES = DIM;
+  constexpr int TROWS = FILTER_ROWS * MB;
+  constexpr int NSTAGE = 3;
+  constexpr int DATA_BYTES = TROWS * ROW_BYTES;
+  constexpr int STAGE_BYTES = DATA_BYTES + WPB * 256;
+  constexpr int PIECES = DATA_BYTES / 1024, PPW = PIECES / WPB;
+  constexpr int CHUNKS_PER_ROW = ROW_BYTES / 16;
+  constexpr int NSLOT = 2 * NB * KS;
+  constexpr int NFRAG = 2 * KS;
+  constexpr int NISSUE = PPW;
+  static_assert(DIM % 128 == 0 && DIM <= 768, "row stride multiple of 128 bytes (swz_chunk); 64 queries x DIM bytes = 192 AGPRs at most");
+  static_assert(PIECES % WPB == 0 && PPW % 2 == 0 && NSTAGE * STAGE_BYTES <= 160 * 1024 && NISSUE < 64 && NFRAG >= RING, "shape / LDS / vmcnt range");
+  static_assert(NSTAGE * STAGE_BYTES == filter_i8s_lds_bytes<DIM, WPB>(), "the launchers size the dynamic LDS with filter_i8s_lds_bytes");
+
+  extern __shared__ __attribute__((aligned(16))) char smem[];
+  const int tid = threadIdx.x, lane = tid & 63, wave = __builtin_amdgcn_readfirstlane(tid >> 6);
+  const int x15 = lane & 15, g4 = lane >> 4;
+  const uint32_t wave_gid = blockIdx.x * WPB + wave;
+
+  const uint32_t nwg = gridDim.x, b = blockIdx.x;
+  const uint32_t S = nwg / QT;
+  uint32_t stream, qt;
+  if (xcd_aware_grid(QT, nwg)) { const uint32_t xcd = b & 7u, i = b >> 3; qt = i % QT; stream = (i / QT) * 8u + xcd; }
+  else { qt = b % QT; stream = b / QT; }
+  const uint32_t tiles_total = (row_hi - row_lo) / TROWS;
+  const bool xcd_map = xcd_aware_grid(QT, nwg);
+  uint32_t t_lo, t_hi;
+  stream_tile_range(tiles_total, S, stream, xcd_map, sa.xcdw, t_lo, t_hi);
+  const uint32_t NT = t_hi - t_lo;
+  if (NT == 0) return;
+
+  const uint32_t qbase = qt * 256u + wave * (16u * NB);
+  float4_t bq[NB * KS];
+#pragma unroll
+  for (int f = 0; f < NB * KS; ++f) {
+    const int nb = f / KS, s = f % KS;
+    bq[f] = *reinterpret_cast<const float4_t*>(qhi + static_cast<uint64_t>(qbase + nb * 16 + x15) * DIM + 64 * s + 16 * g4);
+  }
+#pragma unroll
+  for (int f = 0; f < NB * KS; ++f) asm volatile("" ::"a"(bq[f]));
+  intx4_t bias0;
+#pragma unroll
+  for (int r = 0; r < 4; ++r) bias0[r] = I8_ACC_BIAS;
+  asm volatile("" : "+v"(bias0));
+  uint32_t qid[NB];
+  float t1q[NB];
+  const float lo_unit = __builtin_bit_cast(float, (127u - sa.lo_bits) << 23);
+#pragma unroll
+  for (int nb = 0; nb < NB; ++nb) {
+    qid[nb] = qbase + nb * 16 + x15;
+    const bool real = qid[nb] < nq;
+    const float T = real ? thr[qid[nb]] * qscale[qid[nb]] : __builtin_huge_valf();
+    t1q[nb] = real ? i8_stage1_bar(T, qdelta[qid[nb]], lo_unit) : __builtin_huge_valf();
+    asm volatile("" ::"v"(t1q[nb]));
+  }
+  float s_c, bbar[NB];
+  {
+    s_c = __builtin_bit_cast(float, __builtin_amdgcn_readfirstlane(__builtin_bit_cast(int, scales[row_lo])));
+#pragma unroll
+    for (int nb = 0; nb < NB; ++nb) { bbar[nb] = qid[nb] < nq ? shadow_cs_bits_bar(t1q[nb], s_c) : __builtin_huge_valf(); asm volatile("" ::"v"(bbar[nb])); }
+  }
+  const bool wave_has_queries = qbase < nq;
+
+  uint32_t src_off[PPW];
+#pragma unroll
+  for (int i = 0; i < PPW; ++i) {
+    const uint32_t P = static_cast<uint32_t>((wave * PPW + i) * 64 + lane);
+    const uint32_t r = P / CHUNKS_PER_ROW, cpos = P % CHUNKS_PER_ROW;
+    src_off[i] = r * ROW_BYTES + (swz_chunk<ROW_BYTES>(cpos, r) << 4);
+  }
+  const uint32_t a16 = static_cast<uint32_t>(x15) * ROW_BYTES + (swz_chunk<ROW_BYTES>(static_cast<uint32_t>(g4), static_cast<uint32_t>(x15)) << 4);
+
+  const char* gbase = reinterpret_cast<const char*>(rows);
+  const uint32_t lds_base = static_cast<uint32_t>(reinterpret_cast<uintptr_t>(NVDB_LPTR(smem)));
+  const uint32_t g_lo = row_lo / TROWS + t_lo;
+  auto tile_row0 = [&](uint32_t t_rel) -> uint32_t { return perm_tile(g_lo + (t_rel < NT ? t_rel : NT - 1), sa) * TROWS; };
+  auto issue_piece = [&](uint32_t row0, uint32_t buf, int i) {
+    glds16(src_off[i], gbase + static_cast<uint64_t>(row0) * ROW_BYTES, lds_base + buf * STAGE_BYTES + (wave * PPW + i) * 1024);
+  };
+#pragma unroll
+  for (int st = 0; st < NSTAGE - 1; ++st) {
+#pragma unroll
+    for (int i = 0; i < PPW; ++i) issue_piece(tile_row0(st), st, i);
+  }
+
+  uint32_t wcnt = 0, n_stage1 = 0;
+  Hit* mylog = hitlog + static_cast<uint64_t>(wave_gid) * FILTER_LOGCAP;
+
+  intx4_t acc0[2][NB], acc1[2][NB];
+#pragma unroll
+  for (int h = 0; h < 2; ++h)
+#pragma unroll
+    for (int nb = 0; nb < NB; ++nb) acc1[h][nb] = bias0;
+  float mx[NB][2];
+  float4_t ar[RING];
+
+  auto read_a = [&](const char* stage, int u, int mb) -> float4_t {
+    const int s = u >> 1, h = u & 1;
+    const uint32_t off = swz16<ROW_BYTES>() ? (a16 ^ ((s & 3) << 6)) + (s >> 2) * 256 : (a16 ^ ((s & 1) << 6)) + (s >> 1) * 128;
+    return *reinterpret_cast<const float4_t*>(stage + off + (2 * mb + h) * 16 * ROW_BYTES);
+  };
+  constexpr int SW0 = NSLOT >= 64 ? 8 : 4;
+  constexpr int W0 = SW0 + 10;
+  constexpr int SPU = (NSLOT - W0 - 4) / NV >= 2 ? 2 : 1;
+  static_assert(W0 + NV * SPU + 2 <= NSLOT, "the test ends before the half's last MFMA");
+  auto test_step = [&](const intx4_t (&a)[2][NB], int w) {
+    const int rel = w - W0;
+    if (rel < 0 || rel % SPU != 0) return;
+    const int v = rel / SPU;
+    if (v < NV && (v & 1)) {
+      const int nb = v >> 3, h = (v >> 2) & 1, j = v & 3;
+      const int b0 = a[h][nb][j - 1], b1 = a[h][nb][j];
+      mx[nb][h] = vmax3(mx[nb][h], __builtin_bit_cast(float, b0), __builtin_bit_cast(float, b1));
+    }
+  };
+  auto reset_max = [&]() {
+#pragma unroll
+    for (int nb = 0; nb < NB; ++nb) { mx[nb][0] = -__builtin_huge_valf(); mx[nb][1] = -__builtin_huge_valf(); }
+  };
+  float flagv = -1.f;
+  auto combine_flags = [&]() {
+    float m[NB];
+#pragma unroll
+    for (int nb = 0; nb < NB; ++nb) m[nb] = vmax3(mx[nb][0], mx[nb][1], mx[nb][1]) - bbar[nb];
+    flagv = NB == 4 ? vmax3(vmax3(m[0], m[1], m[NB / 2]), m[NB - 1], m[NB - 1]) : vmax3(m[0], m[NB - 1], m[NB - 1]);
+  };
+  auto any_flag = [&]() -> bool { return __builtin_amdgcn_ballot_w64(flagv >= 0.f) != 0; };
+  auto rare_log = [&](const intx4_t (&a)[2][NB], uint32_t row0, int mb) {
+    ++n_stage1;
+#pragma unroll
+    for (int nb = 0; nb < NB; ++nb)
+#pragma unroll
+      for (int h = 0; h < 2; ++h) {
+        if (!__builtin_amdgcn_ballot_w64(mx[nb][h] >= bbar[nb])) continue;
+#pragma unroll
+        for (int j = 0; j < 4; ++j) {
+          const int H = a[h][nb][j] - I8_ACC_BIAS;
+          const bool hit = static_cast<float>(H) * s_c >= t1q[nb];
+          const unsigned long long m = __builtin_amdgcn_ballot_w64(hit);
+          if (m) {
+            const uint32_t idx = wcnt + static_cast<uint32_t>(__builtin_popcountll(m & ((1ull << lane) - 1ull)));
+            if (hit && idx < FILTER_LOGCAP)
+              mylog[idx] = Hit{s_c, row0 + 32u * mb + 16u * h + 4u * g4 + j, qid[nb], static_cast<uint32_t>(H)};
+            wcnt += static_cast<uint32_t>(__builtin_popcountll(m));
+          }
+        }
+      }
+  };
+
+  uint32_t sync_strikes = 0;
+  const uint32_t xw_t0 = static_cast<uint32_t>(__builtin_amdgcn_s_memrealtime());
+  constexpr int HP = PPW / 2, HP0 = HP < 3 ? HP : 3;
+  constexpr int D1 = (HP - HP0) > 0 ? (HP - HP0) : 1;
+  constexpr int EV1 = NFRAG / D1, EV2 = NFRAG / (PPW - HP);
+  static_assert((HP == HP0 || NFRAG % (HP - HP0) == 0) && NFRAG % (PPW - HP) == 0, "pieces spread evenly over the A fragments of both halves");
+  for (uint32_t t = 0; t < NT; ++t) {
+    if constexpr (SYNC) {
+      if (wave == 0 && (t & sync_mask) == 0) sibling_rendezvous(prog + static_cast<uint64_t>(stream) * 8, qt, t, sync_lead, sync_strikes, lane);
+    }
+    asm volatile("s_waitcnt vmcnt(%0)" ::"n"(NISSUE) : "memory");
+    __builtin_amdgcn_s_barrier();
+    const uint32_t next_row0 = tile_row0(t + 2), next_buf = (t + 2) % NSTAGE;
+    const char* stage = smem + (t % NSTAGE) * STAGE_BYTES;
+    if (!wave_has_queries) {
+#pragma unroll
+      for (int i = 0; i < PPW; ++i) issue_piece(next_row0, next_buf, i);
+      continue;
+    }
+    reset_max();
+#pragma unroll
+    for (int u = 0; u < RING - 1; ++u) ar[u] = read_a(stage, u, 0);
+#pragma unroll
+    for (int i = 0; i < HP0; ++i) issue_piece(next_row0, next_buf, i);
+    __builtin_amdgcn_sched_barrier(0);
+#pragma unroll
+    for (int u = 0; u < NFRAG; ++u) {
+      if (u + RING - 1 < NFRAG) ar[(u + RING - 1) % RING] = read_a(stage, u + RING - 1, 0);
+      else ar[(u + RING - 1) % RING] = read_a(stage, u + RING - 1 - NFRAG, 1);
+      const float4_t av = ar[u % RING];
+      const int s = u >> 1, h = u & 1;
+#pragma unroll
+      for (int nb = 0; nb < NB; ++nb) {
+        if (s == 0) NVDB_MFMA_I8S_FROM(acc0[h][nb], av, bq[nb * KS], bias0);
+        else NVDB_MFMA_I8S_ACC(acc0[h][nb], av, bq[nb * KS + s]);
+        const int w = NB * u + nb;
+        test_step(acc1, w);
+        if (w == NSLOT - 1) combine_flags();
+        __builtin_amdgcn_sched_barrier(0);
+      }
+      if constexpr (HP > HP0) {
+        if (u % EV1 == EV1 - 1) issue_piece(next_row0, next_buf, HP0 + u / EV1);
+        __builtin_amdgcn_sched_barrier(0);
+      }
+    }
+    if (t > 0 && any_flag()) rare_log(acc1, tile_row0(t - 1), 1);
+    reset_max();
+    constexpr int R0 = NFRAG % RING;
+#pragma unroll
+    for (int u = 0; u < NFRAG; ++u) {
+      if (u + RING - 1 < NFRAG) ar[(R0 + u + RING - 1) % RING] = read_a(stage, u + RING - 1, 1);
+      const float4_t av = ar[(R0 + u) % RING];
+      const int s = u >> 1, h = u & 1;
+#pragma unroll
+      for (int nb = 0; nb < NB; ++nb) {
+        if (s == 0) NVDB_MFMA_I8S_FROM(acc1[h][nb], av, bq[nb * KS], bias0);
+        else NVDB_MFMA_I8S_ACC(acc1[h][nb], av, bq[nb * KS + s]);
+        const int w = NB * u + nb;
+        test_step(acc0, w);
+        if (w == NSLOT - 1) combine_flags();
+        __builtin_amdgcn_sched_barrier(0);
+      }
+      if (u % EV2 == EV2 - 1) issue_piece(next_row0, next_buf, HP + u / EV2);
+      __builtin_amdgcn_sched_barrier(0);
+    }
+    if (any_flag()) rare_log(acc0, tile_row0(t), 0);
+  }
+  if (wave_has_queries) {
+    asm volatile("s_nop 15\n\ts_nop 15" ::: "memory");
+    reset_max();
+#pragma unroll
+    for (int w = W0; w < W0 + (NV + 1) * SPU; ++w) test_step(acc1, w);
+    combine_flags();
+    if (any_flag()) rare_log(acc1, tile_row0(NT - 1), 1);
+  }
+  if constexpr (SYNC) { if (wave == 0 && lane == 0) __hip_atomic_store(prog + static_cast<uint64_t>(stream) * 8 + qt, 0xFFFFFFFFu, __ATOMIC_RELAXED, __HIP_MEMORY_SCOPE_AGENT); }
+  if (stage_counts && lane == 0 && n_stage1) atomicAdd(stage_counts, n_stage1);
+  if (wave == 0 && lane == 0) record_xcd_speed(sa.xcdw, xcd_map, stream & 7u, NT, static_cast<uint32_t>(__builtin_amdgcn_s_memrealtime()) - xw_t0);
+  verify_and_scatter_i8<DIM>(mylog, wcnt, sa, lane, rows, qlo, thr, qscale, qinv);
 }
+
+
+}
diff --git a/nano-vectordb_amd/csrc/nvdb_corpus.cpp b/nano-vectordb_amd/csrc/nvdb_corpus.cpp
--- a/nano-vectordb_amd/csrc/nvdb_corpus.cpp
+++ b/nano-vectordb_amd/csrc/nvdb_corpus.cpp
@@ -17,7 +17,7 @@
   if (c->shadow8_scales) { (void)hipFree(c->shadow8_scales); c->shadow8_scales = nullptr; }
   c->rows = nullptr; c->scales = nullptr; c->owned = false; c->n = 0; c->cap_rows = 0; c->dim = 0; c->fdim = 0; c->dtype = 0; c->max_norm = 0.f;
   c->cap_hint = 0;
-  c->q8shadow = false; c->resid_max = 0.f; c->filter_max_norm = 0.f;
+  c->q8shadow = false; c->resid_max = 0.f; c->filter_max_norm = 0.f; c->shadow_cs = ShadowScaleFact{};
   c->shadow_demoted = false; c->last_filter_kind = FILTER_NONE;
   c->range_valid = false; c->range_total = 0;
   parts_drop(c);
@@ -44,7 +44,7 @@
   c->i8_scales_signed = hb[1] != 0;
   c->fdim = c->dim;
   c->filter_max_norm = c->max_norm;
-  c->q8shadow = false; c->resid_max = 0.f;
+  c->q8shadow = false; c->resid_max = 0.f; c->shadow_cs = ShadowScaleFact{};
   size_t free_hbm = 0, total_hbm = 0;
   const bool automatic = c->opt_q8_shadow < 0;
   if (automatic && hipMemGetInfo(&free_hbm, &total_hbm) != hipSuccess) { (void)hipGetLastError(); free_hbm = 0; }
@@ -67,14 +67,33 @@
     const size_t n_pad = (static_cast<size_t>(c->n) + PAD_ROWS - 1) / PAD_ROWS * PAD_ROWS + PAD_ROWS;
     HIPCHK(c, hipMemsetAsync(c->shadow8 + count, 0, pad, c->stream));
     HIPCHK(c, hipMemsetAsync(c->shadow8_scales, 0, n_pad * 4, c->stream));
-    HIPCHK(c, hipMemsetAsync(bits, 0, 8, c->stream));
-    if (c->dtype == NVDB_DTYPE_F32) shadow_q8_kernel<float><<<grid, 256, 0, c->stream>>>(static_cast<const float*>(c->rows), c->shadow8, c->shadow8_scales, c->n, c->dim, sdim, bits);
-    else shadow_q8_kernel<_Float16><<<grid, 256, 0, c->stream>>>(static_cast<const _Float16*>(c->rows), c->shadow8, c->shadow8_scales, c->n, c->dim, sdim, bits);
-    HIPCHK(c, hipGetLastError());
-    HIPCHK(c, hipMemcpyAsync(hb, bits, 8, hipMemcpyDeviceToHost, c->stream));
-    HIPCHK(c, hipStreamSynchronize(c->stream));
+    uint32_t hb4[4] = {0, 0, 0, 0};
+    auto pass = [&](bool write, float common) -> nvdb_status {
+      HIPCHK(c, hipMemsetAsync(bits, 0, 16, c->stream));
+      signed char* dst = write ? c->shadow8 : nullptr;
+      if (c->dtype == NVDB_DTYPE_F32) shadow_q8_kernel<float><<<grid, 256, 0, c->stream>>>(static_cast<const float*>(c->rows), dst, c->shadow8_scales, c->n, c->dim, sdim, common, bits);
+      else shadow_q8_kernel<_Float16><<<grid, 256, 0, c->stream>>>(static_cast<const _Float16*>(c->rows), dst, c->shadow8_scales, c->n, c->dim, sdim, common, bits);
+      HIPCHK(c, hipGetLastError());
+      HIPCHK(c, hipMemcpyAsync(hb4, bits, 16, hipMemcpyDeviceToHost, c->stream));
+      HIPCHK(c, hipStreamSynchronize(c->stream));
+      return NVDB_OK;
+    };
+    ShadowScaleFact fact;
+    if (c->opt_shadow_common_scale != 0) {
+      if ((st = pass(false, 0.f))) return st;
+      std::memcpy(&fact.resid_row, &hb4[0], 4);
+      std::memcpy(&fact.s_c, &hb4[2], 4);
+      if (shadow_cs_try(c->opt_shadow_common_scale, hb4[1] != 0, fact.s_c)) {
+        if ((st = pass(true, fact.s_c))) return st;
+        std::memcpy(&fact.resid_common, &hb4[0], 4);
+        fact.common = shadow_cs_keep(fact.resid_row, fact.resid_common, hb4[1] != 0);
+      }
+    }
+    if (!fact.common && (st = pass(true, 0.f))) return st;
+    hb[0] = hb4[0]; hb[1] = hb4[1];
     if (hb[1] == 0) {
       std::memcpy(&c->resid_max, &hb[0], 4);
+      c->shadow_cs = fact;
       HIPCHK(c, hipMemsetAsync(bits, 0, 8, c->stream));
       row_norm_max_kernel<DT_I8><<<grid, 256, 0, c->stream>>>(c->shadow8, c->shadow8_scales, c->n, sdim, bits);
       HIPCHK(c, hipGetLastError());
@@ -387,6 +406,7 @@
   else if (k == "sibling_sync") { c->opt_sibling_sync = value ? 1 : 0; }
   else if (k == "f32_shadow") { c->opt_f32_shadow = value ? 1 : 0; }
   else if (k == "q8_shadow") { c->opt_q8_shadow = value < 0 ? -1 : value ? 1 : 0; }
+  else if (k == "shadow_common_scale") { c->opt_shadow_common_scale = value == 0 ? 0 : -1; }
   else if (k == "q8_auto_min_rows") { if (value < 1) return fail(c, NVDB_ERR_INVALID, "q8_auto_min_rows must be >= 1"); c->opt_q8_auto_min_rows = value; }
   else if (k == "q8_auto_max_mb") { if (value < 0 || value > (int64_t(1) << 30)) return fail(c, NVDB_ERR_INVALID, "q8_auto_max_mb out of range"); c->opt_q8_auto_max_mb = value; }
 #ifdef NVDB_HIP_DEV
@@ -445,6 +465,16 @@
   return NVDB_OK;
 }
 
+nvdb_status nvdb_hip_shadow_scale_info(const nvdb_hip_ctx* c, double* out4) {
+  if (!c || !out4) return NVDB_ERR_INVALID;
+  const bool on = c->q8shadow;
+  out4[0] = on && c->shadow_cs.common ? 1.0 : 0.0;
+  out4[1] = on ? c->shadow_cs.s_c : 0.0;
+  out4[2] = on ? c->shadow_cs.resid_row : 0.0;
+  out4[3] = on ? c->shadow_cs.resid_common : 0.0;
+  return NVDB_OK;
+}
+
 nvdb_status nvdb_hip_get_stats(nvdb_hip_ctx* c, nvdb_hip_scan_stats* stats) {
   if (!c || !stats) return NVDB_ERR_INVALID;
   if (c->stats_lazy) {
diff --git a/nano-vectordb_amd/csrc/nvdb_ctx.h b/nano-vectordb_amd/csrc/nvdb_ctx.h
--- a/nano-vectordb_amd/csrc/nvdb_ctx.h
+++ b/nano-vectordb_amd/csrc/nvdb_ctx.h
@@ -25,6 +25,7 @@
 #include "kernels_exact.h"
 #include "kernels_filter.h"
 #include "nvdb_common.h"
+#include "shadow_scale_plan.h"
 
 using namespace nvdbhip;
 
@@ -70,6 +71,8 @@
   bool shadow_demoted = false;
   float filter_max_norm = 0.f;
   float resid_max = 0.f;
+  ShadowScaleFact shadow_cs;
+  int64_t opt_shadow_common_scale = -1;
   int64_t opt_q8_shadow = -1;
   int64_t opt_q8_auto_min_rows = 1 << 20;
   int64_t opt_q8_auto_max_mb = 16384;
diff --git a/nano-vectordb_amd/csrc/nvdb_insert.cpp b/nano-vectordb_amd/csrc/nvdb_insert.cpp
--- a/nano-vectordb_amd/csrc/nvdb_insert.cpp
+++ b/nano-vectordb_amd/csrc/nvdb_insert.cpp
@@ -208,15 +208,24 @@
   float new_filter_norm = 0.f, new_resid = 0.f;
   bool shadow_bad = false;
   DevTmp sh8, sh8s, sh16;
+  ShadowScaleFact cs = c->shadow_cs;
   const void* staged_sh8s = nullptr;
   if (c->q8shadow) {
     if ((st = tmp_alloc(c, sh8, m * c->dim)) || (st = tmp_alloc(c, sh8s, m * 4))) return st;
-    HIPCHK(c, hipMemsetAsync(bits, 0, 8, s));
     const unsigned grid = static_cast<unsigned>(std::min<uint64_t>((m + 3) / 4, 4096));
-    if (c->dtype == NVDB_DTYPE_F32) shadow_q8_kernel<float><<<grid, 256, 0, s>>>(static_cast<const float*>(stage.rows), static_cast<signed char*>(sh8.p), static_cast<float*>(sh8s.p), m, c->dim, c->dim, bits);
-    else shadow_q8_kernel<_Float16><<<grid, 256, 0, s>>>(static_cast<const _Float16*>(stage.rows), static_cast<signed char*>(sh8.p), static_cast<float*>(sh8s.p), m, c->dim, c->dim, bits);
-    HIPCHK(c, hipGetLastError());
-    if ((st = read_bits(c, s, bits, hb))) return st;
+    uint32_t hb4[4] = {0, 0, 0, 0};
+    auto quantise = [&](float common) -> nvdb_status {
+      HIPCHK(c, hipMemsetAsync(bits, 0, 16, s));
+      if (c->dtype == NVDB_DTYPE_F32) shadow_q8_kernel<float><<<grid, 256, 0, s>>>(static_cast<const float*>(stage.rows), static_cast<signed char*>(sh8.p), static_cast<float*>(sh8s.p), m, c->dim, c->dim, common, bits);
+      else shadow_q8_kernel<_Float16><<<grid, 256, 0, s>>>(static_cast<const _Float16*>(stage.rows), static_cast<signed char*>(sh8.p), static_cast<float*>(sh8s.p), m, c->dim, c->dim, common, bits);
+      HIPCHK(c, hipGetLastError());
+      HIPCHK(c, hipMemcpyAsync(hb4, bits, 16, hipMemcpyDeviceToHost, s));
+      HIPCHK(c, hipStreamSynchronize(s));
+      return NVDB_OK;
+    };
+    if ((st = quantise(cs.common ? cs.s_c : 0.f))) return st;
+    if (cs.common && !shadow_cs_after_write(cs, as_float(hb4[2])) && (st = quantise(0.f))) return st;
+    hb[0] = hb4[0]; hb[1] = hb4[1];
     new_resid = as_float(hb[0]);
     shadow_bad = hb[1] != 0;
     if (!shadow_bad) {
@@ -298,6 +307,7 @@
     if (c->q8shadow) {
       c->filter_max_norm = std::max(c->filter_max_norm, new_filter_norm);
       c->resid_max = std::max(c->resid_max, new_resid);
+      c->shadow_cs = cs;
     } else {
       c->filter_max_norm = c->max_norm;
       c->i8_scales_signed = c->i8_scales_signed || new_signed;
diff --git a/nano-vectordb_amd/csrc/nvdb_ivf.cpp b/nano-vectordb_amd/csrc/nvdb_ivf.cpp
--- a/nano-vectordb_amd/csrc/nvdb_ivf.cpp
+++ b/nano-vectordb_amd/csrc/nvdb_ivf.cpp
@@ -346,6 +346,7 @@
   nvdb_hip_ctx* c = ix->ctx;
   auto ctx_fail = [&](nvdb_status s_) { return bail(s_, "ivf_build: " + c->err); };
   c->opt_f32_shadow = src->opt_f32_shadow;
+  c->opt_shadow_common_scale = src->opt_shadow_common_scale;
   c->opt_q8_shadow = src->opt_q8_shadow > 0 ? 1 : 0;
   void* rows = nullptr;
   float* scales = nullptr;
diff --git a/nano-vectordb_amd/csrc/nvdb_launch_i8.cpp b/nano-vectordb_amd/csrc/nvdb_launch_i8.cpp
--- a/nano-vectordb_amd/csrc/nvdb_launch_i8.cpp
+++ b/nano-vectordb_amd/csrc/nvdb_launch_i8.cpp
@@ -28,6 +28,7 @@
 template <int DIM, int NB, int MB> auto i8w_build(bool sync) { return sync ? filter_i8w_kernel<DIM, NB, 6, true, MB> : filter_i8w_kernel<DIM, NB, 6, false, MB>; }
 template <int DIM, int WPB, bool DEFER> auto i8p_build(bool sync) { return sync ? filter_i8p_kernel<DIM, true, false, 6, WPB, DEFER> : filter_i8p_kernel<DIM, false, false, 6, WPB, DEFER>; }
 template <int DIM, int WPB> auto i8s_build(bool sync) { return sync ? filter_i8s_kernel<DIM, true, false, 6, WPB> : filter_i8s_kernel<DIM, false, false, 6, WPB>; }
+template <int DIM, int WPB> auto i8c_build(bool sync) { return sync ? shadow_i8c_kernel<DIM, true, 6, WPB> : shadow_i8c_kernel<DIM, false, 6, WPB>; }
 
 template <int DIM, int NB>
 nvdb_status launch_filter_i8w_dim(nvdb_hip_ctx* c, FilterRun& run, RowRange rows) {
@@ -60,6 +61,14 @@
     if (c->opt_i8_small8 && !defer && run.QT == 1 && run.nq > 64)
       return launch(filter_i8s_kernel<DIM, false, false, 6, 4>, 4, filter_i8s_lds_bytes<DIM, 4>());
   if (logs && c->opt_i8_mfma16) {
+    const bool common = run.kind == FILTER_SHADOW8 && c->q8shadow && c->shadow_cs.common && c->opt_shadow_common_scale != 0;
+    if constexpr (DIM == 768) {
+      if (common) {
+        if (w8 || c->opt_i8_dense8) return launch(i8c_build<DIM, 8>(sync), 8, filter_i8s_lds_bytes<DIM, 8>());
+        return launch(i8c_build<DIM, 4>(sync), 4, filter_i8s_lds_bytes<DIM, 4>());
+      }
+    }
+    (void)common;
     if constexpr (DIM == 768 || (DEV_I8S8_512 && DIM == 512))
       if ((w8 || c->opt_i8_dense8) && DIM == 768) return launch(i8s_build<DIM, 8>(sync), 8, filter_i8s_lds_bytes<DIM, 8>());
     if constexpr (DIM >= 384)
diff --git a/nano-vectordb_amd/csrc/shadow_scale_plan.h b/nano-vectordb_amd/csrc/shadow_scale_plan.h
--- /dev/null
+++ b/nano-vectordb_amd/csrc/shadow_scale_plan.h
@@ -0,0 +1,44 @@
+#pragma once
+#include <cstdint>
+
+#if defined(__HIPCC__)
+#define NVDB_CS_HD __host__ __device__
+#else
+#define NVDB_CS_HD
+#endif
+
+namespace nvdbhip {
+
+constexpr int SHADOW_CS_ACC_BIAS = 0x4B000000;
+constexpr int SHADOW_CS_H_MAX = 8384000;
+
+constexpr float SHADOW_CS_MARGIN = 0.25f;
+
+inline bool shadow_cs_scale_ok(float s_c) { return s_c >= 1e-30f && s_c <= 1e30f; }
+
+struct ShadowScaleFact {
+  bool common = false;
+  float s_c = 0.f;
+  float resid_row = 0.f, resid_common = 0.f;
+};
+
+inline bool shadow_cs_try(int64_t opt, bool bad, float s_c) { return opt != 0 && !bad && shadow_cs_scale_ok(s_c); }
+
+inline bool shadow_cs_keep(float resid_row, float resid_common, bool bad_common) {
+  return !bad_common && resid_row >= 0.f && resid_common <= resid_row * (1.0f + SHADOW_CS_MARGIN);
+}
+
+inline bool shadow_cs_after_write(ShadowScaleFact& f, float new_scale_max) {
+  if (f.common && !(new_scale_max <= f.s_c)) f.common = false;
+  return f.common;
+}
+
+NVDB_CS_HD inline float shadow_cs_bits_bar(float t1q, float s_c) {
+  const double r = static_cast<double>(t1q) / static_cast<double>(s_c);
+  const double hb = __builtin_floor(r * (r > 0.0 ? 1.0 - 0x1p-22 : 1.0 + 0x1p-22)) - 1.0;
+  if (hb > static_cast<double>(SHADOW_CS_H_MAX)) return __builtin_huge_valf();
+  const int Hb = hb >= -static_cast<double>(SHADOW_CS_H_MAX) - 1.0 ? static_cast<int>(hb) : -SHADOW_CS_H_MAX - 1;
+  return __builtin_bit_cast(float, SHADOW_CS_ACC_BIAS + Hb);
+}
+
+}
diff --git a/nano-vectordb_amd/nvdb_amd/__init__.py b/nano-vectordb_amd/nvdb_amd/__init__.py
--- a/nano-vectordb_amd/nvdb_amd/__init__.py
+++ b/nano-vectordb_amd/nvdb_amd/__init__.py
@@ -15,7 +15,7 @@
     "nvdb_hip_abi_version", "nvdb_hip_device_count", "nvdb_hip_create", "nvdb_hip_destroy", "nvdb_hip_last_error",
     "nvdb_hip_upload_corpus", "nvdb_hip_adopt_corpus", "nvdb_hip_generate_corpus", "nvdb_hip_corpus_info",
     "nvdb_hip_download_rows", "nvdb_hip_search_batch", "nvdb_hip_search_batch_dev", "nvdb_hip_search_check",
-    "nvdb_hip_get_stats", "nvdb_hip_range_search", "nvdb_hip_range_results", "nvdb_hip_shadow_info", "nvdb_hip_collect_kernel_times", "nvdb_hip_merge_topk_dev", "nvdb_hip_merge_topk_strided_dev", "nvdb_merge_topk_host", "nvdb_hip_set_option",
+    "nvdb_hip_get_stats", "nvdb_hip_range_search", "nvdb_hip_range_results", "nvdb_hip_shadow_info", "nvdb_hip_shadow_scale_info", "nvdb_hip_collect_kernel_times", "nvdb_hip_merge_topk_dev", "nvdb_hip_merge_topk_strided_dev", "nvdb_merge_topk_host", "nvdb_hip_set_option",
     "nvdb_hip_refine_l2_topk", "nvdb_hip_refine_l2_topk_dev", "nvdb_synth_rows_f32", "nvdb_f32_to_f16",
     "nvdb_quantize_i8_rows",
     "nvdb_hip_group_create", "nvdb_hip_group_destroy", "nvdb_hip_group_last_error", "nvdb_hip_group_size", "nvdb_hip_group_ctx",
@@ -133,6 +133,7 @@
     L.nvdb_hip_range_search.argtypes = [vp, vp, u32, vp, vp, C.POINTER(Timing)]
     L.nvdb_hip_range_results.argtypes = [vp, vp, vp]
     L.nvdb_hip_shadow_info.argtypes = [vp, C.POINTER(u64)]
+    L.nvdb_hip_shadow_scale_info.argtypes = [vp, C.POINTER(C.c_double)]
     L.nvdb_hip_collect_kernel_times.argtypes = [vp, C.POINTER(u32), C.POINTER(C.c_double), C.POINTER(C.c_double),
                                                 C.POINTER(C.c_double)]
     L.nvdb_hip_merge_topk_dev.argtypes = [vp, vp, vp, u32, u32, u32, vp, vp, vp]
@@ -458,6 +459,11 @@
         self._chk(self.lib.nvdb_hip_shadow_info(self.h, out))
         return dict(resident=bool(out[0]), bytes=int(out[1]), demoted=bool(out[2]), last_filter=(None, "f16", "shadow", "i8")[out[3]])
 
+    def shadow_scale_info(self):
+        out = (C.c_double * 4)()
+        self._chk(self.lib.nvdb_hip_shadow_scale_info(self.h, out))
+        return dict(common=bool(out[0]), scale=float(out[1]), resid_row=float(out[2]), resid_common=float(out[3]))
+
     def collect_kernel_times(self):
         n, ms, fl, by = C.c_uint32(), C.c_double(), C.c_double(), C.c_double()
         self._chk(self.lib.nvdb_hip_collect_kernel_times(self.h, C.byref(n), C.byref(ms), C.byref(fl), C.byref(by)))
```

Result: faster. 167,600, median of 6 (+4.0%).
